# MichaelWoodhams/IQ-TREE

Hardware: AMD Instinct MI355X
Metric: million pattern-node partial-likelihood updates/sec (higher is better)
Workload: dtype f64; 1 GPU; DNA 50 taxa x 100000 patterns/GPU, GTR+G4, fixed tree: clearAllPartialLH + full traversal + root-branch lnL; ntaxa=50, patterns_per_gpu=100000, patterns_total=100000, nstates=4, ncat=4, parallelism=patterns sharded over 1 GPU(s), 1 RCCL all-reduce/step

## Files before the change

### include/iqhip.h

```cpp
#ifndef IQHIP_H_
#define IQHIP_H_

#include <stddef.h>
#include <stdint.h>

#ifdef __cplusplus
extern "C" {
#endif

#define IQHIP_ABI_VERSION 2

enum {
    IQHIP_OK = 0,
    IQHIP_ERR_NO_DEVICE = 1,
    IQHIP_ERR_INVALID = 2,
    IQHIP_ERR_UNSUPPORTED = 3,
    IQHIP_ERR_HIP = 4,
    IQHIP_ERR_NOMEM = 5
};

typedef struct iqhip_engine iqhip_engine;

typedef struct iqhip_node_op {
    uint64_t dst_key;
// ... 185 lines not shown
int iqhip_debug_ufboot_timing(iqhip_engine *e, double *ms , int64_t *launches);

int iqhip_pair_counts(iqhip_engine *e, const int32_t *pairs , int npairs, double *counts);
int iqhip_pair_distances(iqhip_engine *e, const double *init, double x1, double x2, double xacc, int max_steps,
                         double *dist, double *d2l, int32_t *nsteps);
int iqhip_debug_pair_timing(iqhip_engine *e, double *counts_ms, double *solve_ms);

typedef struct iqhip_quartet_result {
    double  logl[3];
    double  len[3][5];
    int32_t nsweeps[3], neval[3], status[3], _pad;
} iqhip_quartet_result;
int iqhip_quartet_cells(iqhip_engine *e, const int32_t *quartets , int nq,
                        double *cells , int32_t *nother );
int iqhip_quartet_likelihoods(iqhip_engine *e, const int32_t *quartets, int nq,
                              const double *const_invar ,
                              double x1, double x2, double xacc, int max_steps, double diverge_frac,
                              int iterations, double tolerance, iqhip_quartet_result *results);
int iqhip_debug_quartet_timing(iqhip_engine *e, double *cells_ms, double *solve_ms);

typedef struct iqhip_bionj_step { int32_t a, b; double la, lb, lambda; } iqhip_bionj_step;
int iqhip_bionj(iqhip_engine *e, int n, const double *dist , const double *var ,
                iqhip_bionj_step *steps , int32_t *last , double *last_len );
int iqhip_debug_bionj_timing(iqhip_engine *e, double *ms, int64_t *launches);

typedef struct iqhip_pars_op { int32_t dst, left, right, _pad; } iqhip_pars_op;
int iqhip_pars_init(iqhip_engine *e, const uint8_t *informative , int nvectors, int64_t *nsites);
int iqhip_pars_update(iqhip_engine *e, const iqhip_pars_op *ops, int nops);
int iqhip_pars_branch_scores(iqhip_engine *e, const int32_t *ends , int nbranch, int32_t *score,
                             int32_t *subst );
int iqhip_pars_insert_scores(iqhip_engine *e, const int32_t *ends, int nbranch, int32_t taxon,
                             int32_t *score , int32_t *best, int32_t *best_score);
int iqhip_pars_shape(iqhip_engine *e, int64_t *nsites, int64_t *nwords, int *nvectors);
int iqhip_pars_fetch(iqhip_engine *e, int32_t slot, uint32_t *out );
int iqhip_debug_pars_levels(int ntaxa, int nvectors, const uint8_t *valid , const iqhip_pars_op *ops,
                            int nops, int32_t *level);
int iqhip_debug_pars_timing(iqhip_engine *e, double *ms , int64_t *counts , int reset);
int iqhip_pars_insert_scores_batch(iqhip_engine *e, const int32_t *ends ,
                                   const int32_t *seg_start , int nseg,
                                   const int32_t *taxon , int32_t *score ,
                                   int32_t *best , int32_t *best_score );
int iqhip_debug_pars_batch_timing(iqhip_engine *e, double *ms , int64_t *counts ,
                                  int reset);

enum { IQHIP_PARS_SPR_NO_SCORE = 1 };
#define IQHIP_PARS_SPR_MAX_RADIUS 10
typedef struct iqhip_pars_spr_step { int32_t parent, side, target, flags; } iqhip_pars_spr_step;
typedef struct iqhip_pars_spr_job { int32_t subtree, first_step, nsteps, _pad; } iqhip_pars_spr_job;
int iqhip_pars_spr_scan(iqhip_engine *e, const iqhip_pars_spr_job *jobs, int njobs, const iqhip_pars_spr_step *steps,
                        int nsteps, int32_t *score , int32_t *best_step ,
                        int32_t *best_score , int32_t *best_job);
int iqhip_debug_pars_spr_check(int ntaxa, int nvectors, const uint8_t *valid ,
                               const iqhip_pars_spr_job *jobs, int njobs, const iqhip_pars_spr_step *steps, int nsteps,
                               int32_t *depth );
int iqhip_debug_pars_spr_timing(iqhip_engine *e, double *ms , int64_t *counts , int reset);

int iqhip_upload_partial(iqhip_engine *e, uint64_t key, const double *partial_lh,
                         const int16_t *scale_num);

int iqhip_timing_enable(iqhip_engine *e, int on);
int iqhip_timing_read(iqhip_engine *e, double *avg_ms, int64_t *launches, int reset);
int iqhip_timing_plan_bytes(iqhip_engine *e, double *stored, double *loaded);
int iqhip_timing_collective_read(iqhip_engine *e, double *avg_us, int64_t *count, int reset);

int iqhip_debug_cherry_tables(iqhip_engine *e, int64_t *tables_built, int64_t *ops_from_tables);

#define IQHIP_PATH_NEWTON_ONE_LAUNCH 0
#define IQHIP_PATH_NEWTON_CHAIN 1
#define IQHIP_PATH_SWEEP_PERSISTENT 2
#define IQHIP_PATH_SWEEP_PER_STEP 3
#define IQHIP_PATH_SWEEP_SEQUENTIAL 4
#define IQHIP_PATH_NEWTON_FALLBACK 5
#define IQHIP_PATH_NSLOTS 6
int iqhip_debug_path_counts(iqhip_engine *e, int64_t *out, int n);

int iqhip_debug_create_planner(iqhip_engine **out, int nstates , int ncat, int64_t nptn, int ntaxa,
                               int num_cus, int state_unknown, int nclass);
int iqhip_debug_plan(iqhip_engine *e, const iqhip_node_op *ops, int nops);
#define IQHIP_PLAN_SHAPE_NSLOTS 28
int iqhip_debug_plan_shape(iqhip_engine *e, int64_t *out, int n);
#define IQHIP_PLAN_LAYOUT_NSLOTS 8
int iqhip_debug_plan_layout(iqhip_engine *e, int32_t *out, int nops);

void iqhip_debug_memory(int64_t *device_bytes, int64_t *host_bytes);
void iqhip_debug_fail_alloc(int nth);

typedef struct iqhip_partition iqhip_partition;
int iqhip_partition_create(iqhip_partition **out, iqhip_engine *const *members, int nparts);
void iqhip_partition_destroy(iqhip_partition *g);
int iqhip_partition_set_rates(iqhip_partition *g, const double *rate );
int iqhip_partition_newton_branch(iqhip_partition *g, double xguess, double x1, double x2, double xacc, int max_steps,
                                  double *optx, double *d2l, int *nsteps, double *part_lnl );
int iqhip_partition_lnl_from_theta(iqhip_partition *g, double x, double *part_lnl );
int iqhip_partition_traverse_lnl(iqhip_partition *g, const iqhip_node_op *ops, int nops, iqhip_branch_end a,
                                 iqhip_branch_end b, double len, const double *scale ,
                                 double *part_lnl );
int iqhip_partition_optimize_branch_batch(iqhip_partition *g, const iqhip_branch_task *tasks, int ntasks,
                                          iqhip_branch_result *results,
                                          double *part_lnl );
int iqhip_debug_partition_timing(iqhip_partition *g, double *ms ,
                                 int64_t *launches);

int iqhip_partition_ptnlh_reserve(iqhip_partition *g, int nrows);
int iqhip_partition_optimize_branch_batch_rows(iqhip_partition *g, const iqhip_branch_task *tasks, int ntasks,
                                               iqhip_branch_result *results,
                                               double *part_lnl ,
                                               const int32_t *rows );
int iqhip_partition_ptnlh_rell(iqhip_partition *g, const int32_t *rows, int nrows, int nsamples,
                               double *out );
int iqhip_partition_ufboot_init(iqhip_partition *g, int nsamples);
int iqhip_partition_ufboot_update(iqhip_partition *g, const iqhip_ufboot_tree *trees, int ntrees, double epsilon,
                                  double logl_cutoff, int64_t *counts , double *min_orig_logl );
int iqhip_partition_ufboot_fetch(iqhip_partition *g, double *boot_logl, double *boot_orig_logl, int32_t *boot_counts,
                                 int64_t *boot_tree);
int iqhip_debug_partition_ufboot_timing(iqhip_partition *g, double *ms , int64_t *launches);

int iqhip_partition_pair_distances(iqhip_partition *g, const double *init, double x1, double x2, double xacc, int max_steps,
                                   double *dist, double *d2l, int32_t *nsteps);
int iqhip_debug_partition_pair_timing(iqhip_partition *g, double *counts_ms, double *solve_ms);

#ifdef __cplusplus
}
#endif
#endif
```

### iq-tree_amd/__init__.py

```python
import ctypes as C
import os

import numpy as np

_HERE = os.path.dirname(os.path.abspath(__file__))
LIB_DIR = os.environ.get("IQHIP_LIB_DIR") or os.path.join(_HERE, "lib")
REPO_ROOT = os.path.dirname(_HERE)

IQHIP_SYMBOLS = [
    "iqhip_last_error", "iqhip_abi_version", "iqhip_device_count", "iqhip_create", "iqhip_destroy",
    "iqhip_set_stream", "iqhip_reserve", "iqhip_release", "iqhip_rekey", "iqhip_set_alignment",
    "iqhip_set_ptn_freq", "iqhip_set_ptn_invar", "iqhip_set_ascertainment", "iqhip_set_model", "iqhip_update_partials",
    "iqhip_branch_lnl", "iqhip_traverse_lnl", "iqhip_compute_theta", "iqhip_derv",
    "iqhip_lnl_from_theta", "iqhip_newton_branch", "iqhip_optimize_branch", "iqhip_bind_result_buffer", "iqhip_result_device_ptr",
    "iqhip_result_capacity", "iqhip_traverse_lnl_async", "iqhip_derv_async", "iqhip_result_read",
    "iqhip_synchronize", "iqhip_fetch_scale_num", "iqhip_fetch_pattern_lh", "iqhip_fetch_partial",
    "iqhip_fetch_theta", "iqhip_upload_partial", "iqhip_timing_enable", "iqhip_timing_read",
    "iqhip_fetch_pattern_lh_scaled", "iqhip_set_boot_samples", "iqhip_rell", "iqhip_rell_async",
    "iqhip_set_mixture_model", "iqhip_pattern_lh_cat", "iqhip_optimize_branch_batch",
    "iqhip_em_posteriors", "iqhip_em_fetch_posteriors", "iqhip_em_site_rates", "iqhip_em_objective", "iqhip_debug_em_timing",
    "iqhip_mix_class_lh", "iqhip_mix_weights_em", "iqhip_mix_posteriors", "iqhip_debug_mix_timing",
    "iqhip_class_lnl", "iqhip_debug_class_lnl_timing",
    "iqhip_create_sharded", "iqhip_num_shards", "iqhip_shard_range", "iqhip_comm_unique_id", "iqhip_comm_init_rank",
    "iqhip_comm_size", "iqhip_update_partials_async", "iqhip_lnl_from_theta_async",
    "iqhip_newton_host_init", "iqhip_newton_host_update", "iqhip_newton_host_result",
    "iqhip_debug_create_planner", "iqhip_debug_plan", "iqhip_timing_plan_bytes", "iqhip_timing_collective_read", "iqhip_optimize_sweep", "iqhip_debug_cherry_tables",
    "iqhip_debug_path_counts", "iqhip_debug_plan_shape", "iqhip_debug_plan_layout", "iqhip_debug_memory", "iqhip_debug_fail_alloc",
    "iqhip_ptnlh_reserve", "iqhip_ptnlh_put_current", "iqhip_ptnlh_fetch", "iqhip_optimize_branch_batch_rows",
    "iqhip_branch_tests", "iqhip_ptnlh_rell",
    "iqhip_ptnlh_upload", "iqhip_gen_boot_samples", "iqhip_ptnlh_diff_variance", "iqhip_tree_tests", "iqhip_multiscale_bp",
    "iqhip_pair_counts", "iqhip_pair_distances", "iqhip_debug_pair_timing",
    "iqhip_quartet_cells", "iqhip_quartet_likelihoods", "iqhip_debug_quartet_timing",
    "iqhip_pars_init", "iqhip_pars_update", "iqhip_pars_branch_scores", "iqhip_pars_insert_scores", "iqhip_pars_fetch", "iqhip_pars_shape",
    "iqhip_debug_pars_levels", "iqhip_debug_pars_timing",
    "iqhip_pars_insert_scores_batch", "iqhip_debug_pars_batch_timing",
    "iqhip_pars_spr_scan", "iqhip_debug_pars_spr_check", "iqhip_debug_pars_spr_timing",
    "iqhip_bionj", "iqhip_debug_bionj_timing",
    "iqhip_ufboot_init", "iqhip_ufboot_update", "iqhip_ufboot_fetch", "iqhip_debug_ufboot_timing",
    "iqhip_partition_create", "iqhip_partition_destroy", "iqhip_partition_set_rates", "iqhip_partition_newton_branch",
    "iqhip_partition_lnl_from_theta", "iqhip_partition_traverse_lnl", "iqhip_debug_partition_timing",
    "iqhip_partition_optimize_branch_batch",
    "iqhip_partition_ptnlh_reserve", "iqhip_partition_optimize_branch_batch_rows", "iqhip_partition_ptnlh_rell",
    "iqhip_partition_ufboot_init", "iqhip_partition_ufboot_update", "iqhip_partition_ufboot_fetch",
    "iqhip_partition_pair_distances", "iqhip_debug_partition_pair_timing",
    "iqhip_debug_partition_ufboot_timing",
]

_LAUNCH_SLOTS = ("variant", "tab", "nfull", "ngroups", "grid", "lds_bytes", "hold_off")
PLAN_SHAPE_SLOTS = (("lds_budget", "lds_doubles", "state_slots", "nhold", "chunks", "stages") +
                    tuple("stage_units_%d" % s for s in range(8)) +
                    tuple("top_" + f for f in _LAUNCH_SLOTS) + tuple("unit_" + f for f in _LAUNCH_SLOTS))
PATH_SLOTS = ("newton_one_launch", "newton_chain", "sweep_persistent", "sweep_per_step", "sweep_sequential",
              "newton_fallback")


class NodeOp(C.Structure):
    _fields_ = [("dst_key", C.c_uint64), ("left_key", C.c_uint64), ("right_key", C.c_uint64),
                ("left_leaf", C.c_int32), ("right_leaf", C.c_int32),
                ("left_len", C.c_double), ("right_len", C.c_double), ("flags", C.c_uint32), ("_pad", C.c_uint32)]


class BranchEnd(C.Structure):
    _fields_ = [("key", C.c_uint64), ("leaf", C.c_int32), ("_pad", C.c_int32)]


class ParsOp(C.Structure):
    _fields_ = [("dst", C.c_int32), ("left", C.c_int32), ("right", C.c_int32), ("_pad", C.c_int32)]


class BranchSupport(C.Structure):
    _fields_ = [("sh_alrt", C.c_double), ("lbp", C.c_double), ("abayes", C.c_double), ("alrt_stat", C.c_double)]


class TreeTest(C.Structure):
    _fields_ = [("rell_bp", C.c_double), ("kh_pvalue", C.c_double), ("sh_pvalue", C.c_double), ("wkh_pvalue", C.c_double),
                ("wsh_pvalue", C.c_double), ("elw_value", C.c_double), ("rell_confident", C.c_int32),
                ("elw_confident", C.c_int32)]


class UFBootTree(C.Structure):
    _fields_ = [("row", C.c_int32), ("_pad", C.c_int32), ("tree_id", C.c_int64), ("logl", C.c_double), ("rand", C.c_double)]


class BranchTask(C.Structure):
    _fields_ = [("ops", C.c_void_p), ("nops", C.c_int32), ("max_steps", C.c_int32), ("a", BranchEnd), ("b", BranchEnd),
                ("xguess", C.c_double), ("x1", C.c_double), ("x2", C.c_double), ("xacc", C.c_double)]


class BranchResult(C.Structure):
    _fields_ = [("optx", C.c_double), ("d2l", C.c_double), ("lnl", C.c_double), ("nsteps", C.c_int32), ("status", C.c_int32)]


TREE_TEST_DTYPE = np.dtype([("logl", np.float64), ("rell_bp", np.float64), ("kh_pvalue", np.float64),
                            ("sh_pvalue", np.float64), ("wkh_pvalue", np.float64), ("wsh_pvalue", np.float64),
                            ("elw_value", np.float64), ("rell_confident", np.bool_), ("elw_confident", np.bool_)])
AU_SCALES = (0.5, 0.6, 0.7, 0.8, 0.9, 1.0, 1.1, 1.2, 1.3, 1.4)
BIONJ_STEP_DTYPE = np.dtype([("a", np.int32), ("b", np.int32), ("la", np.float64), ("lb", np.float64), ("lambda", np.float64)])
SUPPORT_DTYPE = np.dtype([("node1", np.int32), ("node2", np.int32), ("lh", np.float64, (3,)), ("sh_alrt", np.float64),
                          ("lbp", np.float64), ("abayes", np.float64), ("alrt_stat", np.float64)])


def leaf_end(leaf):
    return BranchEnd(0, int(leaf), 0)


def key_end(key):
    return BranchEnd(int(key), -1, 0)


ALLREDUCE_HOOK = C.CFUNCTYPE(None, C.c_void_p, C.c_int, C.c_void_p)
# ... 2713 lines not shown
```

### iq-tree_amd/csrc/engine.hip

```cpp
#include <math.h>
#include <stdio.h>
#include <stdlib.h>
#include <string.h>

#include <algorithm>
#include <cmath>
#include <atomic>

#include "iqhip_internal.h"

using namespace iqhip;

static thread_local std::string g_err;
namespace iqhip {
int set_error(int code, const std::string &msg) {
    g_err = msg;
    return code;
}
double debug_build_us = 0.0;
}

extern "C" void iqhip_debug_memory(int64_t *device_bytes, int64_t *host_bytes) {
    if (device_bytes) *device_bytes = g_mem_bytes[0].load();
    if (host_bytes) *host_bytes = g_mem_bytes[1].load();
// ... 138 lines not shown
                    hipHostGetDevicePointer((void **)&e->d_done, (void *)e->h_done.p, 0) == hipSuccess &&
                    hipEventCreateWithFlags(&e->staging_free, hipEventDisableTiming) == hipSuccess &&
                    e->dummy.plh.ensure(e, P * e->block) == hipSuccess && e->dummy.sc.ensure(e, P) == hipSuccess &&
                    e->d_newton_partials.ensure(e, (size_t)4 * e->num_cus) == hipSuccess &&
                    e->d_newton_barrier.ensure(e, 2) == hipSuccess && e->d_fold_ticket.ensure(e, 4) == hipSuccess &&
                    e->d_newton_posts.ensure(e, nposts) == hipSuccess &&
                    e->d_fold_flags.ensure(e, (size_t)e->result_cap) == hipSuccess;
    if (!ok) {
        iqhip_destroy(e);
        return fail(IQHIP_ERR_NOMEM, "iqhip_create: device allocation failed");
    }
    hipMemsetAsync(e->dummy.plh.p, 0, P * e->block * sizeof(double), e->stream);
    hipMemsetAsync(e->dummy.sc.p, 0, P * sizeof(int16_t), e->stream);
    hipMemsetAsync(e->d_newton_barrier.p, 0, 2 * sizeof(unsigned int), e->stream);
    hipMemsetAsync(e->d_newton_posts.p, 0xFF, nposts * sizeof(double), e->stream);
    hipMemsetAsync(e->d_fold_ticket.p, 0, 4 * sizeof(unsigned int), e->stream);
    hipMemsetAsync(e->d_fold_flags.p, 0, (size_t)e->result_cap * sizeof(int), e->stream);
    e->d_result = e->d_result_own;
    hipMemsetAsync(e->d_theta.p, 0, P * e->block * sizeof(double), e->stream);
    hipMemsetAsync(e->d_pattern_lh.p, 0, P * sizeof(double), e->stream);
    memset(e->h_result.p, 0, e->result_cap * sizeof(double));
    *e->h_done.p = 0;
    hipStreamSynchronize(e->stream);
    *out = e;
    return IQHIP_OK;
}

extern "C" void iqhip_destroy(iqhip_engine *e) {
    if (!e) return;
    if (!e->shards.empty()) sharded::destroy(e);
    use_device(e);
    if (e->stream) hipStreamSynchronize(e->stream);
    if (e->pair) iqhip_destroy(e->pair);
    e->pair = nullptr;
    comm_destroy(e);
    if (e->stream) hipStreamSynchronize(e->stream);
    if (e->staging_free) hipEventDestroy(e->staging_free);
    for (auto &p : e->tev) {
        hipEventDestroy(p.first);
        hipEventDestroy(p.second);
    }
    for (auto &p : e->cev) {
        hipEventDestroy(p.first);
        hipEventDestroy(p.second);
    }
    if (e->own_stream && e->stream) hipStreamDestroy(e->stream);
    delete e;
}

extern "C" int iqhip_set_stream(iqhip_engine *e, void *hip_stream) {
    if (!e) return fail(IQHIP_ERR_INVALID, "null engine");
    if (!e->shards.empty()) return fail(IQHIP_ERR_UNSUPPORTED, "a sharded engine runs on its shards' own streams");
    HIPCHK(use_device(e));
    HIPCHK(hipStreamSynchronize(e->stream));
    if (e->own_stream) hipStreamDestroy(e->stream);
    e->stream = (hipStream_t)hip_stream;
    e->own_stream = false;
    if (e->pair) return iqhip_set_stream(e->pair, hip_stream);
    return IQHIP_OK;
}

static int new_slab(iqhip_engine *e, int *idx) {
    if (!e->free_slabs.empty()) {
        *idx = e->free_slabs.back();
        e->free_slabs.pop_back();
        return IQHIP_OK;
    }
    Slab s;
    const size_t P = (size_t)e->nptn_pad;
    if (s.plh.ensure(e, P * e->block) != hipSuccess || s.sc.ensure(e, P) != hipSuccess) return fail(IQHIP_ERR_NOMEM, "slab alloc");
    if (!e->planner) {
        hipMemsetAsync(s.plh.p, 0, P * e->block * sizeof(double), e->stream);
        hipMemsetAsync(s.sc.p, 0, P * sizeof(int16_t), e->stream);
    }
    e->slabs.push_back(std::move(s));
    *idx = (int)e->slabs.size() - 1;
    return IQHIP_OK;
}

int iqhip::slab_for_key(iqhip_engine *e, uint64_t key, bool create, int *idx) {
    auto it = e->key2slab.find(key);
    if (it != e->key2slab.end()) {
        *idx = it->second;
        return IQHIP_OK;
    }
    if (!create) return fail(IQHIP_ERR_INVALID, "unknown partial_lh key (vector never computed)");
    int rc = new_slab(e, idx);
    if (rc) return rc;
    e->key2slab[key] = *idx;
    e->keymap_version++;
    return IQHIP_OK;
}

extern "C" int iqhip_reserve(iqhip_engine *e, int nvectors) {
    if (!e) return fail(IQHIP_ERR_INVALID, "null engine");
    if (!e->shards.empty()) return sharded::reserve(e, nvectors);
    HIPCHK(use_device(e));
    int have = (int)e->slabs.size();
    for (int i = have; i < nvectors; i++) {
        int idx;
        std::vector<int> keep;
        keep.swap(e->free_slabs);
        int rc = new_slab(e, &idx);
        keep.swap(e->free_slabs);
        if (rc) return rc;
        e->free_slabs.push_back(idx);
    }
    return IQHIP_OK;
}

extern "C" int iqhip_release(iqhip_engine *e, uint64_t key) {
    if (!e) return fail(IQHIP_ERR_INVALID, "null engine");
    if (!e->shards.empty()) return sharded::release(e, key);
    auto it = e->key2slab.find(key);
    if (it == e->key2slab.end()) return IQHIP_OK;
    e->free_slabs.push_back(it->second);
    e->key2slab.erase(it);
    e->keymap_version++;
    return IQHIP_OK;
}

extern "C" int iqhip_rekey(iqhip_engine *e, uint64_t old_key, uint64_t new_key) {
    if (!e) return fail(IQHIP_ERR_INVALID, "null engine");
    if (!e->shards.empty()) return sharded::rekey(e, old_key, new_key);
    auto it = e->key2slab.find(old_key);
    if (it == e->key2slab.end()) return fail(IQHIP_ERR_INVALID, "iqhip_rekey: unknown key");
    if (old_key == new_key) return IQHIP_OK;
    if (e->key2slab.count(new_key)) iqhip_release(e, new_key);
    int idx = it->second;
    e->key2slab.erase(it);
    e->key2slab[new_key] = idx;
    e->keymap_version++;
    return IQHIP_OK;
}

extern "C" int iqhip_set_ptn_freq(iqhip_engine *e, const double *ptn_freq) {
    if (!e || !ptn_freq) return fail(IQHIP_ERR_INVALID, "null argument");
    if (!e->shards.empty()) return sharded::set_ptn_array(e, ptn_freq, false);
    HIPCHK(use_device(e));
    std::vector<double> tmp((size_t)e->nptn_pad, 0.0);
    memcpy(tmp.data(), ptn_freq, sizeof(double) * (size_t)e->nptn);
    HIPCHK(hipMemcpyAsync(e->d_freq.p, tmp.data(), tmp.size() * sizeof(double), hipMemcpyHostToDevice,
                          e->stream));
    HIPCHK(hipStreamSynchronize(e->stream));
    e->freq_prefix_valid = false;
    e->h_freq.assign(ptn_freq, ptn_freq + e->nptn);
    e->pars_ready = false;
    return IQHIP_OK;
}

extern "C" int iqhip_set_ptn_invar(iqhip_engine *e, const double *ptn_invar) {
    if (!e || !ptn_invar) return fail(IQHIP_ERR_INVALID, "null argument");
    if (!e->shards.empty()) return sharded::set_ptn_array(e, ptn_invar, true);
    HIPCHK(use_device(e));
    std::vector<double> tmp((size_t)e->nptn_pad, 0.0);
    memcpy(tmp.data(), ptn_invar, sizeof(double) * (size_t)e->nptn);
    HIPCHK(hipMemcpyAsync(e->d_invar.p, tmp.data(), tmp.size() * sizeof(double),
                          hipMemcpyHostToDevice, e->stream));
    HIPCHK(hipStreamSynchronize(e->stream));
    return IQHIP_OK;
}

extern "C" int iqhip_set_alignment(iqhip_engine *e, const uint8_t *states, const double *ptn_freq,
                                   const double *ptn_invar) {
    if (!e || !states || !ptn_freq || !ptn_invar) return fail(IQHIP_ERR_INVALID, "null argument");
    if (!e->shards.empty()) return sharded::set_alignment(e, states, ptn_freq, ptn_invar);
    if (!e->model_set)
        return fail(IQHIP_ERR_INVALID,
                    "iqhip_set_alignment: call iqhip_set_model first (needs state_unknown)");
    HIPCHK(use_device(e));
    const size_t P = (size_t)e->nptn_pad, N = (size_t)e->nptn;
    std::vector<uint8_t> tmp((size_t)e->ntaxa * P, (uint8_t)(e->embed2 ? e->n : e->state_unknown));
    for (int t = 0; t < e->ntaxa; t++) {
        const uint8_t *src = states + (size_t)t * N;
        if (e->embed2) {
            uint8_t *dst = tmp.data() + (size_t)t * P;
            for (size_t p = 0; p < N; p++) {
                if (src[p] > e->n_user) return fail(IQHIP_ERR_INVALID, "iqhip_set_alignment: state > STATE_UNKNOWN");
                dst[p] = src[p] == e->n_user ? (uint8_t)e->n : src[p];
            }
            continue;
        }
        for (size_t p = 0; p < N; p++)
            if (src[p] > e->state_unknown)
                return fail(IQHIP_ERR_INVALID, "iqhip_set_alignment: state > STATE_UNKNOWN");
        memcpy(tmp.data() + (size_t)t * P, src, N);
    }
    HIPCHK(hipMemcpyAsync(e->d_states.p, tmp.data(), tmp.size(), hipMemcpyHostToDevice, e->stream));
    HIPCHK(hipStreamSynchronize(e->stream));
    e->pars_ready = false;
    int rc = iqhip_set_ptn_freq(e, ptn_freq);
    if (rc) return rc;
    rc = iqhip_set_ptn_invar(e, ptn_invar);
    if (rc) return rc;
    e->aln_set = true;
    return IQHIP_OK;
}

extern "C" int iqhip_set_ascertainment(iqhip_engine *e, int64_t n_unobserved, double nsites) {
    if (!e) return fail(IQHIP_ERR_INVALID, "null engine");
    if (n_unobserved < 0 || n_unobserved >= e->nptn || (n_unobserved > 0 && !(nsites > 0.0)))
        return fail(IQHIP_ERR_INVALID, "iqhip_set_ascertainment: bad pattern count / site count");
    if (!e->shards.empty()) return sharded::set_ascertainment(e, n_unobserved, nsites);
    e->n_unobs = n_unobserved;
    e->asc_nsites = nsites;
    e->asc_active = n_unobserved > 0 || (e->comm && nsites > 0.0);
    e->pattern_lh_shift = 0.0;
    return IQHIP_OK;
}

static int set_model_common(iqhip_engine *e, int nclass, const int32_t *cat_class, const double *eval,
                            const double *evec, const double *inv_evec, const double *rates, const double *props,
                            int state_unknown, const double *tip ) {
    if (!e || !eval || !evec || !inv_evec || !rates || !props || !tip)
        return fail(IQHIP_ERR_INVALID, "null argument");
    if (!e->shards.empty())
        return sharded::set_model(e, nclass, cat_class, eval, evec, inv_evec, rates, props, state_unknown, tip);
    if (state_unknown < e->n || state_unknown > (e->mfma ? 255 : 31))
        return fail(IQHIP_ERR_INVALID, "iqhip_set_model: state_unknown out of range");
    if (e->aln_set && state_unknown != e->state_unknown)
        return fail(IQHIP_ERR_INVALID, "iqhip_set_model: state_unknown changed after set_alignment");
    if (nclass < 1 || nclass > e->ncat) return fail(IQHIP_ERR_INVALID, "bad number of mixture classes");
    if (e->n == 4 && !e->wide4) {
        const bool want_mfma = nclass > 1;
        if (want_mfma != e->mfma) {
            HIPCHK(use_device(e));
            HIPCHK(hipStreamSynchronize(e->stream));
            e->mfma = want_mfma;
            if (want_mfma) { e->lane_split_valu = e->lane_split; e->lane_split = 1; }
            else e->lane_split = e->lane_split_valu;
            e->tile = want_mfma ? 16 : 64;
            e->ntiles = e->nptn_pad / e->tile;
            e->plan_cache.invalidate();
            e->theta_valid = false;
            HIPCHK(hipMemsetAsync(e->d_newton_posts.p, 0xFF, (size_t)2 * kNewtonPostEpochs * (2 * e->num_cus) * 2 * sizeof(double), e->stream));
            e->newton_post_launches = 0;
        }
    }
    std::vector<int> cls(e->ncat, 0);
    if (nclass > 1) {
        if (!cat_class) return fail(IQHIP_ERR_INVALID, "null argument");
        for (int c = 0; c < e->ncat; c++) {
            if (cat_class[c] < 0 || cat_class[c] >= nclass) return fail(IQHIP_ERR_INVALID, "category class out of range");
            cls[c] = cat_class[c];
        }
    }
    HIPCHK(use_device(e));
    const int n = e->n, C = e->ncat;
    HIPCHK(hipStreamSynchronize(e->stream));
    const size_t nst = (size_t)state_unknown + 1;
    const size_t o_eval = 0, o_evec = o_eval + n, o_ievec = o_evec + (size_t)n * n, o_rates = o_ievec + (size_t)n * n,
                 o_props = o_rates + C, o_tip = o_props + C, o_evalc = o_tip + nst * n, o_tipc = o_evalc + (size_t)C * n,
                 o_cls = o_tipc + nst * C * n;
    const int a_mt = n / 16, a_ks = n / 4;
    const bool a_tail = (n % 16) == 4;
    const size_t aimg_doubles = (n == 20 || n == 64) ? (size_t)2 * a_mt * a_ks * 64 + (a_tail ? (size_t)2 * a_ks * 64 : 0) : 0;
    const size_t o_aimg = (o_cls + ((size_t)C + 1) / 2 + 1) / 2 * 2;
    const size_t total = o_aimg + aimg_doubles;
    std::vector<double> blk(total, 0.0);
    memcpy(&blk[o_eval], eval, sizeof(double) * n);
    memcpy(&blk[o_evec], evec, sizeof(double) * n * n);
    memcpy(&blk[o_ievec], inv_evec, sizeof(double) * n * n);
    memcpy(&blk[o_rates], rates, sizeof(double) * C);
    memcpy(&blk[o_props], props, sizeof(double) * C);
    for (size_t s = 0; s < nst; s++) memcpy(&blk[o_tip + s * n], &tip[(s * nclass) * n], sizeof(double) * n);
    for (int c = 0; c < C; c++) memcpy(&blk[o_evalc + (size_t)c * n], &eval[(size_t)cls[c] * n], sizeof(double) * n);
    for (size_t s = 0; s < nst; s++)
        for (int c = 0; c < C; c++)
            memcpy(&blk[o_tipc + (s * C + c) * n], &tip[(s * nclass + cls[c]) * n], sizeof(double) * n);
    memcpy(&blk[o_cls], cls.data(), sizeof(int) * C);
    e->h_evec0.assign(evec, evec + (size_t)n * n);
    e->h_tip0.assign(&blk[o_tip], &blk[o_tip] + nst * n);
    if (aimg_doubles) {
        double *U = &blk[o_aimg], *Ui = U + (size_t)a_mt * a_ks * 64, *U4 = Ui + (size_t)a_mt * a_ks * 64, *Ui4 = U4 + (size_t)a_ks * 64;
        for (int m = 0; m < a_mt; m++)
            for (int ks = 0; ks < a_ks; ks++)
                for (int l = 0; l < 64; l++) {
                    const int row = 16 * m + (l & 15), k = 4 * ks + (l >> 4);
                    U[((size_t)m * a_ks + ks) * 64 + l] = evec[(size_t)row * n + k];
                    Ui[((size_t)m * a_ks + ks) * 64 + l] = inv_evec[(size_t)row * n + k];
                }
        if (a_tail)
            for (int ks = 0; ks < a_ks; ks++)
                for (int l = 0; l < 64; l++) {
                    const int row = 16 * a_mt + (l & 3), k = 4 * ks + (l >> 4);
                    U4[(size_t)ks * 64 + l] = evec[(size_t)row * n + k];
                    Ui4[(size_t)ks * 64 + l] = inv_evec[(size_t)row * n + k];
                }
    }
    HIPCHK(e->d_model.ensure(e, total));
    double *const d_model = e->d_model.p;
    HIPCHK(hipMemcpy(d_model, blk.data(), sizeof(double) * total, hipMemcpyHostToDevice));
    e->d_eval = d_model + o_eval;
    e->d_evec = d_model + o_evec;
    e->d_inv_evec = d_model + o_ievec;
    e->d_rates = d_model + o_rates;
    e->d_props = d_model + o_props;
    e->d_tip = d_model + o_tip;
    e->d_evalc = d_model + o_evalc;
    e->d_tipc = d_model + o_tipc;
    e->d_cls = reinterpret_cast<int *>(d_model + o_cls);
    e->d_aimg = aimg_doubles ? d_model + o_aimg : nullptr;
    e->aimg_doubles = (int)aimg_doubles;
    if (nclass > 1 || (e->n == 20 && !e->mfma_pipelined_ok) || e->wide4) {
        const int MT = (n + 15) / 16, KS = n / 4;
// ... 151 lines not shown

int iqhip::require(iqhip_engine *e, const char *what, unsigned needs) {
    const auto no = [what](int code, const char *why) { return fail(code, std::string(what) + ": " + why); };
    if (!e) return no(IQHIP_ERR_INVALID, "null engine");
    if (e->planner) return no(IQHIP_ERR_INVALID, "not available on a planning-only engine");
    if ((needs & REQ_SINGLE_DEVICE) && (!e->shards.empty() || e->comm))
        return no(IQHIP_ERR_UNSUPPORTED, "not available on pattern-sharded engines");
    if ((needs & REQ_NO_ASC) && (e->asc_active || e->n_unobs > 0))
        return no(IQHIP_ERR_UNSUPPORTED, "not available with ascertainment bias correction (+ASC)");
    const bool only4 = needs & REQ_STATES_4;
    if ((needs & REQ_PLAIN_STATES) && (e->embed2 || e->n_user != e->n))
        return no(IQHIP_ERR_UNSUPPORTED, only4 ? "not available for embedded state counts (4 states only)"
                                               : "not available for embedded state counts (4, 20 or 64 states only)");
    if ((needs & REQ_STATES_4_20_64) && e->n != 4 && e->n != 20 && e->n != 64) return no(IQHIP_ERR_UNSUPPORTED, "4, 20 or 64 states only");
    if (only4 && e->n != 4) return no(IQHIP_ERR_UNSUPPORTED, "4 states only");
    if ((needs & REQ_NO_MIXTURE) && e->nclass > 1) return no(IQHIP_ERR_UNSUPPORTED, "not available for mixture models");
    if ((needs & REQ_MIXTURE) && e->nclass < 2) return no(IQHIP_ERR_UNSUPPORTED, "the model is no mixture (one class)");
    if ((needs & REQ_MODEL_ALN) && (!e->model_set || !e->aln_set))
        return no(IQHIP_ERR_INVALID, "needs iqhip_set_model and iqhip_set_alignment first");
    if ((needs & REQ_THETA) && !e->theta_valid) return no(IQHIP_ERR_INVALID, "needs iqhip_compute_theta first");
    return IQHIP_OK;
}

static void timing_begin(iqhip_engine *e) {
    if (!e->timing) return;
    if (e->tev_used == e->tev.size()) {
        hipEvent_t a, b;
        hipEventCreate(&a);
        hipEventCreate(&b);
        e->tev.emplace_back(a, b);
    }
    hipEventRecord(e->tev[e->tev_used].first, e->stream);
}
static void timing_end(iqhip_engine *e) {
    if (!e->timing) return;
    hipEventRecord(e->tev[e->tev_used].second, e->stream);
    e->tev_used++;
}

static int build_cherry_tables(iqhip_engine *e) {
    iqhip_engine *p = e->pair;
    const int n = (int)e->plan.cherry_jobs.size();
    std::vector<iqhip_node_op> ops((size_t)n);
    const std::vector<int> segs((size_t)n, 1);
    for (int i = 0; i < n; i++) {
        const iqhip_engine::CherrySlot &cs = e->cherry_slots[e->plan.cherry_jobs[i]];
        iqhip_node_op &o = ops[i];
        memset(&o, 0, sizeof o);
        o.dst_key = (uint64_t)e->plan.cherry_jobs[i] + 1;
        o.left_leaf = 0;
        o.right_leaf = 1;
        o.left_len = cs.len_l;
        o.right_len = cs.len_r;
    }
    iqhip_branch_end none = {0, -1, 0};
    int rc = submit_traverse(p, ops.data(), n, false, none, none, 0.0, true, &segs, nullptr);
    if (rc) return rc;
    std::vector<const double *> src((size_t)n);
    std::vector<double *> dst((size_t)n);
    const size_t per = (size_t)e->cherry_npairs * e->block;
    for (int i = 0; i < n; i++) {
        int idx;
        rc = slab_for_key(p, ops[i].dst_key, false, &idx);
        if (rc) return rc;
        src[i] = p->slabs[idx].plh.p;
        dst[i] = e->d_cherry_tab.p + (size_t)e->plan.cherry_jobs[i] * per;
    }
    HIPCHK(launch_cherry_transpose(e, src.data(), dst.data(), n, e->cherry_npairs));
    for (int i = 0; i < n; i++) e->cherry_slots[e->plan.cherry_jobs[i]].model_version = e->model_version;
    e->cherry_built_total += n;
    e->plan.cherry_jobs.clear();
    return IQHIP_OK;
}

int iqhip::submit_traverse(iqhip_engine *e, const iqhip_node_op *ops, int nops, bool has_root,
                           iqhip_branch_end a, iqhip_branch_end b, double len, bool skip_reduce,
                           const std::vector<int> *explicit_segs, const double *const *len_ptrs) {
    int rc = check_ready(e);
    if (rc) return rc;
    if (nops < 0 || (nops > 0 && !ops)) return fail(IQHIP_ERR_INVALID, "bad ops array");
    int last_dst = -1;
    Stopwatch watch;
    if (e->debug_sweep) watch.start();
    rc = build_plan(e, ops, nops, &last_dst, explicit_segs, len_ptrs);
    if (rc) return rc;
    if (e->debug_sweep) debug_build_us += watch.us();
    DevBranch br;
    if (has_root) {
        rc = build_branch(e, a, b, len, last_dst, &br);
        if (rc) return rc;
    }
    rc = ensure_slab_rows(e, 2 + nops);
    if (rc) return rc;
    const int nwaves = (int)e->ntiles * e->lane_split;
    if (e->plan.nleaf_tabs > 0) {
        const int njobs = leaf_tables_follow_model(e) ? e->plan.nleaf_tabs : e->plan.tab_dirty;
        if (njobs > 0)
            HIPCHK(launch_leaf_tables(e, reinterpret_cast<const TabJob *>(e->d_ops.p + e->plan.jobs_off), njobs));
        e->plan.tab_dirty = 0;
    }
    if (!e->plan.cherry_jobs.empty()) {
        rc = build_cherry_tables(e);
        if (rc) return rc;
    }
    if (e->plan.uses_cherry)
        for (int k = 0; k < nops; k++) e->cherry_ops_total += e->h_ops.p[k].cherry != nullptr;
    timing_begin(e);
    const int *table = reinterpret_cast<const int *>(e->d_ops.p + e->plan.table_off);
    {
        int off = 2;
        for (int n : e->plan.stage_units) {
            if (e->mfma) HIPCHK(launch_traverse_mfma(e, table + off, n, nwaves));
            else HIPCHK(launch_traverse4(e, table + off, n, e->plan.units_have_load, nullptr, nwaves));
            off += 2 * n;
        }
    }
    const bool empty_top = e->plan.nunits > 0 && !has_root && e->plan.top_nops == 0;
    const bool fold4 = e->fold_reduce && !e->mfma && !empty_top && !skip_reduce;
    const bool foldm = e->fold_reduce && e->mfma && has_root && e->n_unobs == 0;
    if (empty_top) {
    } else if (e->mfma) HIPCHK(launch_traverse_mfma(e, table, nops > 0 ? 1 : 0, nwaves, true));
    else HIPCHK(launch_traverse4(e, table, 1, e->plan.has_load, has_root ? &br : nullptr, nwaves, fold4 ? nops : -1));
    timing_end(e);
    if (e->timing) e->tev_launches += (int)e->plan.stage_units.size() + (empty_top ? 0 : 1);
    if (e->mfma && has_root) HIPCHK(launch_stream_mfma(e, 0, &br, br.len, nwaves, nullptr, foldm ? nops : -1));
    if (fold4 || foldm) {
    } else if (has_root) HIPCHK(launch_reduce(e, 0, 2 + nops, nwaves));
    else if (!skip_reduce) HIPCHK(launch_reduce(e, 2, nops, nwaves));
    e->last_nops = nops;
    e->last_has_root = has_root;
    e->last_root_loads_b = has_root && br.b_kind != CHILD_PREV;
    return IQHIP_OK;
}

int iqhip::read_result(iqhip_engine *e, int ndoubles) {
    if (e->d_result != e->d_result_own)
        HIPCHK(hipMemcpyAsync(e->h_result.p, e->d_result, sizeof(double) * ndoubles, hipMemcpyDeviceToHost,
                              e->stream));
    else if (e->poll_pending) {
        e->poll_pending = false;
        const unsigned long long want = e->result_seq;
        for (int spin = 0; spin < 200000; spin++) {
            if (*e->h_done.p == want) {
                std::atomic_thread_fence(std::memory_order_acquire);
                e->staging_busy = false;
                if (e->folded_rows >= 0) {
                    if (e->h_result.p[2 + e->folded_rows] == 0.0)
                        for (int k = 0; k < e->folded_rows; k++) e->h_result.p[2 + k] = 0.0;
                    e->folded_rows = -1;
                }
                return IQHIP_OK;
            }
            __builtin_ia32_pause();
        }
    }
    e->poll_pending = false;
    HIPCHK(hipStreamSynchronize(e->stream));
    e->staging_busy = false;
    if (e->folded_rows >= 0) {
        if (e->h_result.p[2 + e->folded_rows] == 0.0)
            for (int k = 0; k < e->folded_rows; k++) e->h_result.p[2 + k] = 0.0;
        e->folded_rows = -1;
    }
    return IQHIP_OK;
}

void iqhip::result_arrived(iqhip_engine *e) {
// ... 95 lines not shown
    return iqhip_traverse_lnl(e, nullptr, 0, a, b, len, nullptr, lnl);
}

extern "C" int iqhip_traverse_lnl_async(iqhip_engine *e, const iqhip_node_op *ops, int nops,
                                        iqhip_branch_end a, iqhip_branch_end b, double len) {
    if (e && !e->shards.empty())
        return fail(IQHIP_ERR_UNSUPPORTED, "a sharded engine reduces its results itself: use the synchronous calls");
    return submit_traverse(e, ops, nops, true, a, b, len);
}

extern "C" int iqhip_update_partials_async(iqhip_engine *e, const iqhip_node_op *ops, int nops) {
    if (e && !e->shards.empty())
        return fail(IQHIP_ERR_UNSUPPORTED, "a sharded engine reduces its results itself: use the synchronous calls");
    iqhip_branch_end none = {0, -1, 0};
    return submit_traverse(e, ops, nops, false, none, none, 0.0);
}

void iqhip::set_theta_branch(iqhip_engine *e, const DevBranch &br, iqhip_branch_end a, iqhip_branch_end b) {
    e->theta_valid = true;
    e->theta_a_sc = br.a_sc;
    e->theta_b_sc = br.b_sc;
    if (b.leaf >= 0) std::swap(a, b);
    e->theta_end[0] = a;
    e->theta_end[1] = b;
}

extern "C" int iqhip_compute_theta(iqhip_engine *e, iqhip_branch_end a, iqhip_branch_end b) {
    if (e && !e->shards.empty()) return sharded::compute_theta(e, a, b);
    int rc = check_ready(e);
    if (rc) return rc;
    DevBranch br;
    rc = build_branch(e, a, b, 0.0, -1, &br);
    if (rc) return rc;
    if (e->mfma) HIPCHK(launch_stream_mfma(e, 1, &br, 0.0, (int)e->ntiles));
    else HIPCHK(launch_theta4(e, br));
    set_theta_branch(e, br, a, b);
    return IQHIP_OK;
}

extern "C" int iqhip_derv_async(iqhip_engine *e, double len) {
    if (e && !e->shards.empty())
        return fail(IQHIP_ERR_UNSUPPORTED, "a sharded engine reduces its results itself: use the synchronous calls");
    int rc = check_ready(e);
    if (rc) return rc;
    if (!e->theta_valid) return fail(IQHIP_ERR_INVALID, "iqhip_derv: theta not computed");
    if (!(len >= 0.0)) return fail(IQHIP_ERR_INVALID, "negative or NaN branch length");
    const int nrows = e->n_unobs > 0 ? 5 : 2;
    if (e->asc_active && e->n_unobs == 0) {
        if (e->d_result == e->d_result_own) e->h_result.p[2] = e->h_result.p[3] = e->h_result.p[4] = 0.0;
        else HIPCHK(hipMemsetAsync(e->d_result + 2, 0, 3 * sizeof(double), e->stream));
    }
    rc = ensure_slab_rows(e, nrows);
    if (rc) return rc;
    const int nwaves = (int)e->ntiles;
    if (e->mfma) HIPCHK(launch_stream_mfma(e, 2, nullptr, len, nwaves));
    else HIPCHK(launch_derv4(e, len, nwaves));
    HIPCHK(launch_reduce(e, 0, nrows, nwaves));
    return IQHIP_OK;
}

extern "C" int iqhip_derv(iqhip_engine *e, double len, double *df, double *ddf) {
    if (e && !e->shards.empty()) return sharded::derv(e, len, df, ddf);
    int rc = iqhip_derv_async(e, len);
    if (rc) return rc;
    rc = comm_allreduce(e, e->asc_active ? 5 : 2);
    if (rc) return rc;
    rc = read_result(e, e->asc_active ? 5 : 2);
    if (rc) return rc;
    double a = e->h_result.p[0], b = e->h_result.p[1];
    newton_repair(a, b);
    if (e->asc_active) asc_derv_correct(e->h_result.p + 2, e->asc_nsites, a, b);
    if (df) *df = a;
    if (ddf) *ddf = b;
    return IQHIP_OK;
}

extern "C" int iqhip_debug_cherry_tables(iqhip_engine *e, int64_t *tables_built, int64_t *ops_from_tables) {
    if (!e) return fail(IQHIP_ERR_INVALID, "null engine");
    if (tables_built) *tables_built = e->cherry_built_total;
    if (ops_from_tables) *ops_from_tables = e->cherry_ops_total;
    return IQHIP_OK;
}

extern "C" int iqhip_debug_path_counts(iqhip_engine *e, int64_t *out, int n) {
    if (!e) return fail(IQHIP_ERR_INVALID, "null engine");
    if (!out && n > 0) return fail(IQHIP_ERR_INVALID, "null argument");
    for (int k = 0; k < n && k < IQHIP_PATH_NSLOTS; k++) out[k] = e->path_counts[k];
    return IQHIP_OK;
}

extern "C" int iqhip_lnl_from_theta_async(iqhip_engine *e, double len) {
    if (e && !e->shards.empty())
        return fail(IQHIP_ERR_UNSUPPORTED, "a sharded engine reduces its results itself: use the synchronous calls");
    int rc = check_ready(e);
    if (rc) return rc;
    if (!e->theta_valid) return fail(IQHIP_ERR_INVALID, "iqhip_lnl_from_theta: theta not computed");
    if (!(len >= 0.0)) return fail(IQHIP_ERR_INVALID, "negative or NaN branch length");
    rc = ensure_slab_rows(e, 2);
    if (rc) return rc;
    const int nwaves = (int)e->ntiles;
    if (e->mfma) HIPCHK(launch_stream_mfma(e, 3, nullptr, len, nwaves));
    else HIPCHK(launch_lnl_theta4(e, len, nwaves));
    HIPCHK(launch_reduce(e, 0, 2, nwaves));
    return IQHIP_OK;
}

extern "C" int iqhip_lnl_from_theta(iqhip_engine *e, double len, double *lnl) {
    if (e && !e->shards.empty()) return sharded::lnl_from_theta(e, len, lnl);
    int rc = iqhip_lnl_from_theta_async(e, len);
    if (rc) return rc;
    rc = comm_allreduce(e, e->asc_active ? 2 : 1);
    if (rc) return rc;
    rc = read_result(e, 2);
    if (rc) return rc;
    double v = e->h_result.p[0];
    if (isnan(v) || isinf(v)) {
        rc = repair_lnl_comm(e, &v);
        if (rc) return rc;
    }
    rc = asc_finish_lnl(e, &v);
    if (rc) return rc;
    if (lnl) *lnl = v;
    return IQHIP_OK;
}

extern "C" int iqhip_bind_result_buffer(iqhip_engine *e, void *device_ptr, int capacity_doubles) {
    if (!e) return fail(IQHIP_ERR_INVALID, "null engine");
    if (!e->shards.empty() || e->comm)
        return fail(IQHIP_ERR_UNSUPPORTED, "an engine with a communicator reduces in its own device result vector");
    HIPCHK(use_device(e));
    HIPCHK(hipStreamSynchronize(e->stream));
    if (!device_ptr) {
        e->d_result = e->d_result_own;
        e->result_cap = 8 + 16384;
        return IQHIP_OK;
    }
    if (capacity_doubles < 2) return fail(IQHIP_ERR_INVALID, "result buffer too small");
    e->d_result = (double *)device_ptr;
    e->result_cap = std::min(capacity_doubles, 8 + 16384);
    return IQHIP_OK;
}
extern "C" void *iqhip_result_device_ptr(iqhip_engine *e) { return (e && e->shards.empty()) ? (void *)e->d_result : nullptr; }
extern "C" int iqhip_result_capacity(iqhip_engine *e) { return e ? e->result_cap : 0; }

extern "C" int iqhip_result_read(iqhip_engine *e, double *out, int ndoubles) {
    if (e && !e->shards.empty())
        return fail(IQHIP_ERR_UNSUPPORTED, "a sharded engine reduces its results itself: use the synchronous calls");
    if (!e || !out || ndoubles < 0 || ndoubles > e->result_cap)
        return fail(IQHIP_ERR_INVALID, "iqhip_result_read: bad arguments");
    HIPCHK(use_device(e));
    int rc = read_result(e, ndoubles);
    if (rc) return rc;
    memcpy(out, e->h_result.p, sizeof(double) * ndoubles);
    return IQHIP_OK;
}

extern "C" int iqhip_synchronize(iqhip_engine *e) {
    if (!e) return fail(IQHIP_ERR_INVALID, "null engine");
    if (!e->shards.empty()) return sharded::synchronize(e);
    HIPCHK(use_device(e));
    HIPCHK(hipStreamSynchronize(e->stream));
    e->staging_busy = false;
    return IQHIP_OK;
}

static inline size_t dev_index(const iqhip_engine *e, int64_t p, int k) {
// ... 54 lines not shown
    HIPCHK(hipMemcpy(e->slabs[idx].sc.p, sc.data(), sc.size() * sizeof(int16_t), hipMemcpyHostToDevice));
    return IQHIP_OK;
}

extern "C" int iqhip_fetch_theta(iqhip_engine *e, double *out) {
    if (!e || !out) return fail(IQHIP_ERR_INVALID, "null argument");
    if (!e->shards.empty()) return sharded::fetch_vec(e, 0, true, out);
    HIPCHK(use_device(e));
    return fetch_vec(e, e->d_theta.p, out);
}

extern "C" int iqhip_fetch_scale_num(iqhip_engine *e, uint64_t key, int16_t *out) {
    if (!e || !out) return fail(IQHIP_ERR_INVALID, "null argument");
    if (!e->shards.empty()) return sharded::fetch_scale_num(e, key, out);
    HIPCHK(use_device(e));
    int idx;
    int rc = slab_for_key(e, key, false, &idx);
    if (rc) return rc;
    HIPCHK(hipStreamSynchronize(e->stream));
    HIPCHK(hipMemcpy(out, e->slabs[idx].sc.p, sizeof(int16_t) * (size_t)e->nptn, hipMemcpyDeviceToHost));
    return IQHIP_OK;
}

extern "C" int iqhip_fetch_pattern_lh(iqhip_engine *e, double *out) {
    if (!e || !out) return fail(IQHIP_ERR_INVALID, "null argument");
    if (!e->shards.empty()) return sharded::fetch_pattern_lh(e, out, 0, iqhip_branch_end{0, -1, 0}, iqhip_branch_end{0, -1, 0});
    HIPCHK(use_device(e));
    HIPCHK(hipStreamSynchronize(e->stream));
    HIPCHK(hipMemcpy(out, e->d_pattern_lh.p, sizeof(double) * (size_t)e->nptn, hipMemcpyDeviceToHost));
    if (e->asc_active) {
        const int64_t nobs = e->nptn - e->n_unobs;
        for (int64_t p = 0; p < nobs; p++) out[p] -= e->pattern_lh_shift;
        for (int64_t p = nobs; p < e->nptn; p++) out[p] = 0.0;
    }
    return IQHIP_OK;
}

extern "C" int iqhip_timing_enable(iqhip_engine *e, int on) {
    if (!e) return fail(IQHIP_ERR_INVALID, "null engine");
    if (!e->shards.empty()) {
        for (iqhip_engine *c : e->shards) c->timing = on != 0;
        return IQHIP_OK;
    }
    e->timing = on != 0;
    return IQHIP_OK;
}

extern "C" int iqhip_timing_collective_read(iqhip_engine *e, double *avg_us, int64_t *count, int reset) {
    if (!e) return fail(IQHIP_ERR_INVALID, "null engine");
    if (!e->shards.empty()) e = e->shards[0];
    HIPCHK(use_device(e));
    HIPCHK(hipStreamSynchronize(e->stream));
    double total = 0.0;
    for (size_t i = 0; i < e->cev_used; i++) {
        float ms = 0.f;
        HIPCHK(hipEventElapsedTime(&ms, e->cev[i].first, e->cev[i].second));
        total += ms;
    }
    if (avg_us) *avg_us = e->cev_used ? total * 1e3 / (double)e->cev_used : 0.0;
    if (count) *count = (int64_t)e->cev_used;
    if (reset) e->cev_used = 0;
    return IQHIP_OK;
}

extern "C" int iqhip_timing_plan_bytes(iqhip_engine *e, double *stored, double *loaded) {
    if (!e) return fail(IQHIP_ERR_INVALID, "null engine");
    double st = 0.0, ld = 0.0;
    if (!e->shards.empty()) {
        for (iqhip_engine *c : e->shards) {
            double a = 0.0, b = 0.0;
            int rc = iqhip_timing_plan_bytes(c, &a, &b);
            if (rc) return rc;
            st += a; ld += b;
        }
    } else {
        const double P = (double)e->nptn_pad, V = (double)e->block * 8.0;
        const bool hands_over = e->wide4 && !e->wide4_generic && e->h_ops.p && e->last_nops > 0;
        std::vector<char> seg_first(hands_over ? (size_t)e->last_nops : 0, 0);
        if (hands_over) {
            const int *tab = reinterpret_cast<const int *>(e->h_ops.p + e->plan.table_off);
            for (int u = 0; u <= e->plan.nunits; u++)
                if (tab[2 * u + 1] > 0 && tab[2 * u] >= 0 && tab[2 * u] < e->last_nops) seg_first[tab[2 * u]] = 1;
        }
        for (int k = 0; k < e->last_nops && e->h_ops.p; k++) {
            const DevOp &d = e->h_ops.p[k];
            st += P * (V + 2.0);
            const double *held = (hands_over && k > 0 && !seg_first[k]) ? e->h_ops.p[k - 1].dst : nullptr;
            if (d.left_kind == CHILD_LEAF) ld += P;
            else if ((d.left_kind == CHILD_PF || d.left_kind == CHILD_LOAD) && d.pf != held) ld += P * (V + 2.0);
            if (d.right_kind == CHILD_LEAF) ld += P; else if (d.right_kind == CHILD_LOAD && d.ld != held) ld += P * (V + 2.0);
        }
        if (e->last_has_root) {
            st += P * 8.0;
            ld += P * 16.0 + (e->last_root_loads_b ? P * V : 0.0) + P;
        }
    }
    if (stored) *stored = st;
    if (loaded) *loaded = ld;
    return IQHIP_OK;
}

extern "C" int iqhip_timing_read(iqhip_engine *e, double *avg_ms, int64_t *launches, int reset) {
    if (!e) return fail(IQHIP_ERR_INVALID, "null engine");
    if (!e->shards.empty()) {
        double worst = 0.0;
        int64_t n0 = 0;
        for (size_t g = 0; g < e->shards.size(); g++) {
            double a = 0.0;
            int64_t n = 0;
            int rc = iqhip_timing_read(e->shards[g], &a, &n, reset);
            if (rc) return rc;
            if (a > worst) worst = a;
            if (g == 0) n0 = n;
        }
        if (avg_ms) *avg_ms = worst;
        if (launches) *launches = n0;
        return IQHIP_OK;
    }
    HIPCHK(use_device(e));
    HIPCHK(hipStreamSynchronize(e->stream));
    double total = 0.0;
    for (size_t i = 0; i < e->tev_used; i++) {
        float ms = 0.f;
        HIPCHK(hipEventElapsedTime(&ms, e->tev[i].first, e->tev[i].second));
        total += ms;
    }
    if (avg_ms) *avg_ms = e->tev_launches ? total / (double)e->tev_launches : 0.0;
    if (launches) *launches = e->tev_launches;
    if (reset) { e->tev_used = 0; e->tev_launches = 0; }
    return IQHIP_OK;
}

extern "C" int iqhip_debug_create_planner(iqhip_engine **out, int nstates, int ncat, int64_t nptn, int ntaxa, int num_cus,
                                          int state_unknown, int nclass) {
    if (!out) return fail(IQHIP_ERR_INVALID, "iqhip_debug_create_planner: out == NULL");
    *out = nullptr;
    if (nptn <= 0 || ntaxa < 2 || ncat < 1 || num_cus < 1 || nclass < 1 || nclass > ncat)
        return fail(IQHIP_ERR_INVALID, "iqhip_debug_create_planner: bad shape");
    if (nstates != 4 && nstates != 20 && nstates != 64)
        return fail(IQHIP_ERR_UNSUPPORTED, "iqhip_debug_create_planner: nstates must be 4, 20 or 64");
    if (state_unknown < nstates || state_unknown > 255) return fail(IQHIP_ERR_INVALID, "state_unknown out of range");
    {
        const int rc = check_shape4("iqhip_debug_create_planner", nstates, nstates, ncat);
        if (rc) return rc;
    }
    iqhip_engine *e = new iqhip_engine();
    e->planner = true;
    e->check_plans = true;
    e->num_cus = num_cus;
    configure_engine(e, -1, nstates, nstates, ncat, nptn, ntaxa);
    const size_t P = (size_t)e->nptn_pad;
    e->d_states.ensure(e, (size_t)ntaxa * P);
    e->dummy.plh.ensure(e, P * e->block);
    e->dummy.sc.ensure(e, P);
    e->result_cap = 8 + 16384;
    e->state_unknown = state_unknown;
    e->nclass = nclass;
    if (nclass > 1 && nstates == 4 && !e->wide4) {
        e->mfma = true;
        e->lane_split = 1;
        e->tile = 16;
        e->ntiles = e->nptn_pad / 16;
    }
    e->mfma_pipelined = e->mfma_pipelined_ok && nclass == 1;
    e->model_set = e->aln_set = true;
    {
        const int s2 = state_unknown + 1;
        if (cherry_candidate(e) && nclass == 1 && s2 * s2 <= 4356 && (int64_t)4 * s2 * s2 <= e->nptn_pad) {
            e->cherry_s2 = s2;
// ... 61 lines not shown
```

### iq-tree_amd/csrc/iqhip_internal.h

```cpp
#pragma once
#include <hip/hip_runtime.h>
#include <stdint.h>
#include <stdlib.h>
#include <time.h>
#include <algorithm>
#include <atomic>
#include <string>
#include <type_traits>
#include <unordered_map>
#include <vector>
#include "../../include/iqhip.h"
#include "trav_lds.h"

namespace iqhip {

constexpr int kSmallPlanOps = 4;
constexpr int kNewtonPostEpochs = 128;
constexpr int kMixEmTile = 256;
constexpr int kMixEmRegClasses = 8;
constexpr int kMixEmBatch = 16;
constexpr int kMixEmUpdateThreads = 1024;
constexpr double kScalingThreshold = 0x1p-256;
constexpr double kScalingThresholdInv = 0x1p256;
constexpr double kLogScalingThreshold = -177.44567822334599;

enum ChildKind : int32_t { CHILD_LEAF = 0, CHILD_LOAD = 1, CHILD_PREV = 2, CHILD_PF = 3, CHILD_HOLD = 4 };

struct __attribute__((aligned(16))) DevOp {
    double *dst;
    int16_t *dst_sc;
    const double *pf;
    const int16_t *pf_sc;
    const uint8_t *sl;
    const uint8_t *sr;
    const double *ld;
    const int16_t *ld_sc;
    int32_t left_kind;
    int32_t right_kind;
    double left_len;
    double right_len;
    int32_t lds_left;
    int32_t lds_right;
    int32_t chunk_nops;
    int32_t real_mask;
    int32_t sl_slot;
    int32_t sr_slot;
    int32_t push_hold;
    int32_t out_row;
    int32_t no_scale;
    const double *tabL;
    const double *tabR;
    const double *left_len_p;
    const double *right_len_p;
    const double *cherry;
    int32_t chunk_slots;
    int32_t _pad_slots;
};

#if defined(__HIPCC__)
__device__ __forceinline__ double wave_sum64(double v) {
    unsigned lo = __double2loint(v), hi = __double2hiint(v);
    auto a = __builtin_amdgcn_permlane32_swap(lo, lo, false, false);
    auto b = __builtin_amdgcn_permlane32_swap(hi, hi, false, false);
    v = __hiloint2double(b[0], a[0]) + __hiloint2double(b[1], a[1]);
    lo = __double2loint(v);
    hi = __double2hiint(v);
    auto c = __builtin_amdgcn_permlane16_swap(lo, lo, false, false);
    auto d = __builtin_amdgcn_permlane16_swap(hi, hi, false, false);
    v = __hiloint2double(d[0], c[0]) + __hiloint2double(d[1], c[1]);
#define IQHIP_DPP_STEP(ctrl)                                                                                  \
    v += __hiloint2double(__builtin_amdgcn_mov_dpp(__double2hiint(v), ctrl, 0xF, 0xF, true),                  \
                          __builtin_amdgcn_mov_dpp(__double2loint(v), ctrl, 0xF, 0xF, true));
    IQHIP_DPP_STEP(0x128)
    IQHIP_DPP_STEP(0x124)
    IQHIP_DPP_STEP(0x4E)
    IQHIP_DPP_STEP(0xB1)
#undef IQHIP_DPP_STEP
    return v;
}

__device__ __forceinline__ double group_sum(double v) {
    unsigned lo = __double2loint(v), hi = __double2hiint(v);
    auto a = __builtin_amdgcn_permlane16_swap(lo, lo, false, false);
    auto b = __builtin_amdgcn_permlane16_swap(hi, hi, false, false);
    v = __hiloint2double(b[0], a[0]) + __hiloint2double(b[1], a[1]);
    lo = __double2loint(v);
    hi = __double2hiint(v);
    auto c = __builtin_amdgcn_permlane32_swap(lo, lo, false, false);
    auto d = __builtin_amdgcn_permlane32_swap(hi, hi, false, false);
    return __hiloint2double(d[0], c[0]) + __hiloint2double(d[1], c[1]);
}

constexpr unsigned kScalingThresholdHi = 0x2FF00000u;
__device__ __forceinline__ unsigned amax_hi(unsigned m, double v) {
    const unsigned h = (unsigned)__double2hiint(v) & 0x7fffffffu;
    return m > h ? m : h;
}
__device__ __forceinline__ unsigned nonzero_bits(double v) {
    return ((unsigned)__double2hiint(v) & 0x7fffffffu) | (unsigned)__double2loint(v);
}
__device__ __forceinline__ unsigned group_max_u(unsigned v) {
    auto a = __builtin_amdgcn_permlane32_swap(v, v, false, false);
    v = a[0] > a[1] ? a[0] : a[1];
    auto b = __builtin_amdgcn_permlane16_swap(v, v, false, false);
    return b[0] > b[1] ? b[0] : b[1];
}

template <typename OpRef>
__device__ __forceinline__ double op_child_len(const OpRef &d, int child) {
    const double *p = child ? d.right_len_p : d.left_len_p;
    return p ? *p : (child ? d.right_len : d.left_len);
}
#endif

struct __attribute__((aligned(16))) DevBranch {
    const double *a;
    const uint8_t *a_states;
    const double *b;
    const int16_t *a_sc;
    const int16_t *b_sc;
    int32_t a_kind;
    int32_t b_kind;
    double len;
};

struct __attribute__((aligned(16))) SweepOp {
    double *dst;
    int16_t *dst_sc;
    const double *lv, *rv;
    const int16_t *lsc, *rsc;
    const uint8_t *ls, *rs;
    double llen, rlen;
    int32_t llen_step, rlen_step;
    int32_t no_scale;
    int32_t row;
};
struct __attribute__((aligned(16))) SweepStep {
    DevBranch br;
    double xguess;
    int32_t op_begin, nops;
};

struct __attribute__((aligned(16))) PairTile {
    int32_t ra[4], rb[4];
    int32_t out[16];
};

struct __attribute__((aligned(16))) TabJob {
    double len;
    double *tab;
    const double *len_p;
    double _pad;
};

struct Plan {
    int lds_doubles = 0;
    int state_slots = 1;
    bool has_load = false;
    bool units_have_load = false;
    bool small = false;
    int small_nops = 0;
    int nunits = 0, top_nops = 0;
    std::vector<int> stage_units;
    int table_off = 0, jobs_off = 0;
    int nhold = 0;
    int nleaf_tabs = 0;
    std::vector<TabJob> tab_jobs;
    int tab_dirty = 0;
    std::vector<int> cherry_jobs;
    bool uses_cherry = false;
    uint64_t cherry_model = 0;
};

struct PlanCache {
    std::vector<char> ops_in;
    std::vector<int> segs;
    uint64_t version = 0;
    int dst = -1;
    std::vector<char> uploaded;
    void invalidate() { version = 0; uploaded.clear(); }
};

struct __attribute__((aligned(16))) NewtonState {
    double x1, x2, xacc;
    double rts, rts_old, xl, xh, dx, f, df, d2l, result;
    int32_t max_steps, j, neval, status;
    int32_t done, _pad[3];
};

__host__ __device__ inline void newton_init(NewtonState &s, double xguess, double x1, double x2, double xacc,
                                            int max_steps) {
    s.x1 = x1; s.x2 = x2; s.xacc = xacc;
    s.rts = xguess;
    if (s.rts < x1) s.rts = x1;
    if (s.rts > x2) s.rts = x2;
    s.rts_old = s.rts; s.xl = x1; s.xh = x2; s.dx = 0.0; s.f = s.df = s.d2l = 0.0;
    s.result = s.rts;
    s.max_steps = max_steps; s.j = 0; s.neval = 0; s.status = 0; s.done = 0;
    s._pad[0] = s._pad[1] = s._pad[2] = 0;
}

__host__ __device__ inline bool newton_finite(double v) { return v == v && v - v == 0.0; }

__host__ __device__ inline void newton_repair(double &pdf, double &pddf) {
    if (!newton_finite(pdf)) { pdf = 0.0; pddf = 0.0; }
}

__host__ __device__ inline void asc_derv_correct(const double *c, double asc_nsites, double &df, double &ddf) {
    const double prob_const = 1.0 - c[0];
    const double df_frac = c[1] / prob_const, ddf_frac = c[2] / prob_const;
    df += asc_nsites * df_frac;
    ddf += asc_nsites * (ddf_frac + df_frac * df_frac);
}

__host__ __device__ inline void newton_advance(NewtonState &s, double f, double df) {
    if (s.done) return;
    s.f = f; s.df = df;
    s.neval++;
    if (s.neval == 1) {
        s.d2l = df;
        if (!newton_finite(f) || !newton_finite(df)) { s.status = 2; s.result = s.rts; s.done = 1; return; }
        if (df >= 0.0 && fabs(f) < s.xacc) { s.result = s.rts; s.done = 1; return; }
        if (f < 0.0) { s.xl = s.rts; s.xh = s.x2; } else { s.xh = s.rts; s.xl = s.x1; }
        s.dx = fabs(s.xh - s.xl);
        s.j = 1;
    } else {
        if (!newton_finite(f) || !newton_finite(df)) { s.status = 2; s.result = s.rts_old; s.done = 1; return; }
        if (df > 0.0 && fabs(f) < s.xacc) { s.d2l = df; s.result = s.rts; s.done = 1; return; }
        if (f < 0.0) s.xl = s.rts; else s.xh = s.rts;
        s.j++;
        if (s.j > s.max_steps) { s.status = 3; s.result = s.rts; s.done = 1; return; }
    }
    s.rts_old = s.rts;
    if ((df <= 0.0) || (((s.rts - s.xh) * df - f) * ((s.rts - s.xl) * df - f) >= 0.0)) {
        s.dx = 0.5 * (s.xh - s.xl);
        s.rts = s.xl + s.dx;
        s.d2l = df;
        if (s.xl == s.rts) { s.result = s.rts; s.done = 1; return; }
    } else {
        s.dx = f / df;
        const double temp = s.rts;
        s.rts -= s.dx;
        s.d2l = df;
        if (temp == s.rts) { s.result = s.rts; s.done = 1; return; }
    }
    if (fabs(s.dx) < s.xacc || s.j == s.max_steps) { s.result = s.rts_old; s.done = 1; return; }
}

__host__ __device__ inline void newton_update(NewtonState &s, double pdf, double pddf) {
    if (s.done) return;
    newton_repair(pdf, pddf);
    newton_advance(s, -pdf, -pddf);
}

enum MemKind : int { MEM_DEVICE = 0, MEM_PINNED, MEM_PINNED_MAPPED, MEM_HOST };
inline std::atomic<int64_t> g_mem_bytes[2];
inline std::atomic<int> g_fail_alloc_in{0};
inline hipError_t mem_alloc(void **p, size_t bytes, MemKind kind) {
    *p = nullptr;
    if (g_fail_alloc_in.load() > 0 && g_fail_alloc_in.fetch_sub(1) == 1) return hipErrorOutOfMemory;
    hipError_t s;
    if (kind == MEM_DEVICE) s = hipMalloc(p, bytes);
    else if (kind == MEM_HOST) s = (*p = calloc(1, bytes)) ? hipSuccess : hipErrorOutOfMemory;
    else s = hipHostMalloc(p, bytes, kind == MEM_PINNED_MAPPED ? hipHostMallocMapped : hipHostMallocDefault);
    if (s == hipSuccess) g_mem_bytes[kind != MEM_DEVICE] += (int64_t)bytes;
    return s;
}
inline void mem_free(void *p, size_t bytes, MemKind kind) {
    if (kind == MEM_DEVICE) hipFree(p);
    else if (kind == MEM_HOST) free(p);
    else hipHostFree(p);
    g_mem_bytes[kind != MEM_DEVICE] -= (int64_t)bytes;
}

template <typename T>
struct OwnedBuf {
    T *p = nullptr; size_t cap = 0;
    OwnedBuf() = default;
    OwnedBuf(OwnedBuf &&o) noexcept { swap(o); }
    OwnedBuf &operator=(OwnedBuf &&o) noexcept { swap(o); return *this; }
    ~OwnedBuf() { reset(); }
    void swap(OwnedBuf &o) { std::swap(p, o.p); std::swap(cap, o.cap); std::swap(bytes, o.bytes); std::swap(kind, o.kind); }
    void reset() {
        if (bytes) mem_free(const_cast<std::remove_cv_t<T> *>(p), bytes, kind);
        p = nullptr; cap = 0; bytes = 0;
    }
protected:
    hipError_t replace(hipStream_t s, size_t count, MemKind k) {
        if (k != MEM_HOST) {
            const hipError_t rc = hipStreamSynchronize(s);
            if (rc != hipSuccess) return rc;
        }
        reset();
        void *q = nullptr;
        const hipError_t rc = mem_alloc(&q, count * sizeof(T), k);
        if (rc != hipSuccess) return rc;
        p = static_cast<T *>(q); cap = count; bytes = count * sizeof(T); kind = k;
        return hipSuccess;
    }
    size_t bytes = 0;
    MemKind kind = MEM_DEVICE;
};

template <typename T>
struct DevBuf : OwnedBuf<T> {
    hipError_t ensure(hipStream_t s, size_t count) { return count <= this->cap ? hipSuccess : this->replace(s, count, MEM_DEVICE); }
    hipError_t ensure(iqhip_engine *e, size_t count);
};
template <typename T>
struct PinBuf : OwnedBuf<T> {
    hipError_t ensure(hipStream_t s, size_t count, bool mapped = false) {
        return count <= this->cap ? hipSuccess : this->replace(s, count, mapped ? MEM_PINNED_MAPPED : MEM_PINNED);
    }
    hipError_t ensure(iqhip_engine *e, size_t count, bool mapped = false);
};
template <typename T>
struct PairBuf {
    DevBuf<T> d; PinBuf<T> h;
    template <typename Where>
    hipError_t ensure(Where w, size_t count) {
        const hipError_t rc = d.ensure(w, count);
        return rc != hipSuccess ? rc : h.ensure(w, count);
    }
};

struct Slab {
    DevBuf<double> plh;
    DevBuf<int16_t> sc;
};

}

struct iqhip_engine {
    int device = 0;
    bool planner = false;
    uint64_t fake_next = 0x100000000000ull;
    bool check_plans = false;
    int n = 0, ncat = 0, ntaxa = 0;
    bool embed2 = false;
    bool scalar_rule_all = false;
    int n_user = 0;
    int64_t nptn = 0;
    int64_t nptn_pad = 0;
    int64_t ntiles = 0;
    int tile = 64;
    bool mfma = false;
    bool mfma_pipelined = false;
    bool row_split = false;
    bool cat_split = false;
    bool top_cs2 = false;
    int lane_split = 1;
    bool wide4 = false, wide4_generic = false;
    int lane_split_valu = 1;
    bool mix_split = false;
    bool mixed_top = true;
    bool hold_lds = true;
    int lds_budget_bytes = 64 * 1024;
    bool small_plans = true;
    int split_target = -1;
    int max_levels = 3;
    int mfma_lds_kb = -1;
    bool debug_plan = false;
    bool debug_sweep = false;
    std::string debug_break_plan;
    iqhip::Plan plan;
    iqhip::Slab dummy;
    int block = 0;
    int state_unknown = -1;
    bool model_set = false, aln_set = false, theta_valid = false;
    int64_t n_unobs = 0;
    bool asc_active = false;
    double asc_nsites = 0.0;
    double pattern_lh_shift = 0.0;
    const int16_t *theta_a_sc = nullptr;
    const int16_t *theta_b_sc = nullptr;
    iqhip_branch_end theta_end[2] = {{0, -1, 0}, {0, -1, 0}};

    hipStream_t stream = nullptr;
    bool own_stream = false;

    iqhip::DevBuf<uint8_t> d_states;
    iqhip::DevBuf<double> d_freq, d_invar;
    double *d_eval = nullptr, *d_evec = nullptr, *d_inv_evec = nullptr;
    double *d_rates = nullptr, *d_props = nullptr, *d_tip = nullptr;
    std::vector<double> h_eval, h_rates, h_props;
    std::vector<int> h_cls;
    iqhip::DevBuf<iqhip::DevOp> d_ops;
    iqhip::DevBuf<double> d_slab;
    iqhip::DevBuf<unsigned int> d_fold_ticket;
    iqhip::DevBuf<int> d_fold_flags;
    bool fold_reduce = false;
    bool poll_result = true, poll_pending = false;
    unsigned long long result_seq = 0;
    iqhip::PinBuf<volatile unsigned long long> h_done;
    unsigned long long *d_done = nullptr;
    iqhip::DevBuf<double> d_theta, d_pattern_lh;
    iqhip::DevBuf<double> d_leaf_tab;
    std::vector<double> tab_len;
    uint64_t model_version = 1, tab_model_version = 0;
    struct CherrySlot {
        double len_l = -1.0, len_r = -1.0;
        uint64_t model_version = 0;
        uint64_t stamp = 0;
    };
    bool cherry_on = true;
    iqhip_engine *pair = nullptr;
    int cherry_s2 = 0, cherry_npairs = 0;
    iqhip::DevBuf<double> d_cherry_tab;
    std::unordered_map<uint64_t, int> cherry_slot_of;
    std::vector<CherrySlot> cherry_slots;
    uint64_t cherry_stamp = 0;
// ... 58 lines not shown
    } mix;
    struct {
        iqhip::DevBuf<double> cw, inv, part, out;
        iqhip::DevBuf<int32_t> list;
        double ms = 0.0;
    } cl;
    bool mixture_api = false;
    struct {
        iqhip::DevBuf<iqhip::PairTile> tiles;
        iqhip::DevBuf<double> counts, coef, init, out;
        double ms[2] = {0.0, 0.0};
    } pd;
    struct {
        iqhip::DevBuf<int32_t> quartets, nother, other;
        iqhip::DevBuf<double> cells;
        iqhip::DevBuf<iqhip_quartet_result> out;
        double ms[2] = {0.0, 0.0};
    } qt;
    struct {
        double ms = 0.0;
        int64_t launches = 0;
    } bj;
    std::vector<double> h_freq, h_evec0, h_tip0;
    bool pars_ready = false;
    int pars_nvec = 0;
    int64_t pars_nsites = 0, pars_nwords = 0;
    std::vector<uint8_t> pars_valid;
    struct {
        iqhip::DevBuf<uint32_t> vec, score;
        iqhip::DevBuf<int32_t> ints;
        iqhip::DevBuf<int32_t> out;
        iqhip::DevBuf<uint64_t> masks;
    } pars;
    iqhip::PinBuf<int32_t> h_pars_ops, h_pars_ends, h_pars_out;
    double pars_ms[2] = {0.0, 0.0};
    int64_t pars_counts[4] = {0, 0, 0, 0};
    double pars_spr_ms = 0.0;
    int64_t pars_spr_counts[2] = {0, 0};
    double pars_batch_ms = 0.0;
    int64_t pars_batch_counts[3] = {0, 0, 0};
    iqhip::DevBuf<int32_t> d_batch_rows;
    double *d_result_own = nullptr, *d_result = nullptr;
    iqhip::DevBuf<double> d_newton_partials;
    iqhip::DevBuf<unsigned int> d_newton_barrier;
    unsigned int newton_launches = 0;
    iqhip::DevBuf<double> d_newton_posts;
    unsigned int newton_post_launches = 0;
    bool newton_posts = true;
    iqhip::DevBuf<double> d_batch_posts;
    size_t batch_posts_used[2] = {0, 0};
    unsigned int batch_post_launches = 0;
    iqhip::DevBuf<double> d_theta_batch, d_batch_partials, d_batch_out;
    iqhip::DevBuf<unsigned int> d_batch_barriers;
    iqhip::DevBuf<char> d_batch_tasks;
    int batch_cap = 0;
    unsigned int batch_launches = 0;
    iqhip::DevBuf<double> d_sweep_len;
    iqhip::PinBuf<char> h_sweep_desc;
    iqhip::DevBuf<char> d_sweep_desc;
    iqhip::DevBuf<unsigned long long> d_sweep_prof;
    iqhip::DevBuf<double> d_sweep_posts;
    int num_cus = 256;
    int result_cap = 0;
    void *comm = nullptr;
    int comm_nranks = 1, comm_rank = 0;
    iqhip::DevBuf<double> d_result_dev;
    iqhip::DevBuf<iqhip::NewtonState> d_nstate;
    iqhip::PinBuf<iqhip::NewtonState> h_nstate;
    iqhip::DevBuf<iqhip::NewtonState> d_bstates;
    iqhip::DevBuf<const int16_t *> d_bsc;
    std::vector<iqhip_engine *> shards;
    std::vector<int64_t> shard_first;
    int reduce_mode = 0;
    iqhip::PinBuf<iqhip::DevOp> h_ops;
    iqhip::PinBuf<double> h_result;
    iqhip::PlanCache plan_cache;
    iqhip::PinBuf<char> h_plan_arena;
    size_t plan_arena_used = 0;
    bool plan_arena_on = false;
    uint64_t keymap_version = 1;
    hipEvent_t staging_free = nullptr;
    bool staging_busy = false;

    std::unordered_map<uint64_t, int> key2slab;
    std::vector<iqhip::Slab> slabs;
    std::vector<int> free_slabs;

    bool timing = false;
    std::vector<std::pair<hipEvent_t, hipEvent_t>> tev;
    size_t tev_used = 0;
    std::vector<std::pair<hipEvent_t, hipEvent_t>> cev;
    size_t cev_used = 0;
    int64_t tev_launches = 0;
    int last_nops = 0;
    bool last_has_root = false, last_root_loads_b = false;
    int folded_rows = -1;
};

namespace iqhip {

struct FoldArgs {
    double *slab;
    double *result;
    unsigned int *ticket;
    int *flags;
    int nwaves;
    int nrows_scale;
    int root_rows;
    int enabled;
    volatile unsigned long long *done;
    unsigned long long seq;
};

#if defined(__HIPCC__)
__device__ __forceinline__ void fold_store(double *p, double v) {
    __hip_atomic_store(p, v, __ATOMIC_RELAXED, __HIP_MEMORY_SCOPE_AGENT);
}
__device__ __forceinline__ void fold_flag(const FoldArgs &F, int row) {
    __hip_atomic_fetch_or(&F.flags[row], 1, __ATOMIC_RELAXED, __HIP_MEMORY_SCOPE_AGENT);
}

__device__ inline void fold_tail(const FoldArgs &F) {
    __shared__ double s_f[256];
    __shared__ int s_last;
    asm volatile("s_waitcnt vmcnt(0)" ::: "memory");
    __syncthreads();
    if (threadIdx.x == 0) {
        const unsigned int t = __hip_atomic_fetch_add(F.ticket, 1u, __ATOMIC_RELAXED, __HIP_MEMORY_SCOPE_AGENT);
        s_last = (t == gridDim.x - 1) ? 1 : 0;
    }
    __syncthreads();
    if (!s_last) return;
    __shared__ int s_rows[256];
    __shared__ int s_n;
    const int nrows = 2 + F.nrows_scale;
    auto sum_row = [&](int row) {
        const double *r = F.slab + (size_t)row * F.nwaves;
        if (threadIdx.x < 64) {
            double acc[4] = {0.0, 0.0, 0.0, 0.0};
            for (int base = 0; base < F.nwaves; base += 8 * 256) {
                double v[4][8];
#pragma unroll
                for (int j = 0; j < 4; j++)
#pragma unroll
                    for (int q = 0; q < 8; q++) {
                        const int i = base + q * 256 + (int)threadIdx.x + 64 * j;
                        v[j][q] = i < F.nwaves ? __hip_atomic_load(&r[i], __ATOMIC_RELAXED, __HIP_MEMORY_SCOPE_AGENT) : 0.0;
                    }
#pragma unroll
                for (int j = 0; j < 4; j++)
#pragma unroll
                    for (int q = 0; q < 8; q++) {
                        const int i = base + q * 256 + (int)threadIdx.x + 64 * j;
                        if (i < F.nwaves) acc[j] += v[j][q];
                    }
            }
#pragma unroll
            for (int j = 0; j < 4; j++) s_f[(int)threadIdx.x + 64 * j] = acc[j];
        }
        __syncthreads();
#pragma unroll
        for (int o = 128; o > 0; o >>= 1) {
            if (threadIdx.x < 64)
                for (int v = (int)threadIdx.x; v < o; v += 64) s_f[v] += s_f[v + o];
            __syncthreads();
        }
// ... 38 lines not shown
                }
        }
        for (int q = 0; q < n; q++) sum_row(s_rows[q]);
    }
    if (F.done && threadIdx.x == 0) F.result[nrows] = (double)nflagged;
    if (threadIdx.x == 0) {
        __hip_atomic_store(F.ticket, 0u, __ATOMIC_RELAXED, __HIP_MEMORY_SCOPE_AGENT);
        if (F.done) {
            __threadfence_system();
            *F.done = F.seq;
        }
    }
}
#endif

int set_error(int code, const std::string &msg);
inline int fail(int code, const std::string &msg) { return set_error(code, msg); }
#define HIPCHK(call)                                                                                           \
    do {                                                                                                       \
        hipError_t _s = (call);                                                                                \
        if (_s != hipSuccess)                                                                                  \
            return iqhip::set_error(IQHIP_ERR_HIP, std::string(#call) + ": " + hipGetErrorString(_s));        \
    } while (0)

template <typename T>
T *fake_alloc(iqhip_engine *e, size_t count) {
    const uint64_t a = e->fake_next;
    e->fake_next += (count * sizeof(T) + 255) / 256 * 256 + 256;
    return reinterpret_cast<T *>(a);
}
template <typename T>
hipError_t DevBuf<T>::ensure(iqhip_engine *e, size_t count) {
    if (!e->planner) return ensure(e->stream, count);
    if (count > this->cap) {
        this->p = fake_alloc<T>(e, count);
        this->cap = count;
    }
    return hipSuccess;
}
template <typename T>
hipError_t PinBuf<T>::ensure(iqhip_engine *e, size_t count, bool mapped) {
    if (!e->planner) return ensure(e->stream, count, mapped);
    return count <= this->cap ? hipSuccess : this->replace(nullptr, count, MEM_HOST);
}
constexpr unsigned kLdsCeilingDevices = 64;
template <auto Kernel>
hipError_t raise_lds_ceiling(const iqhip_engine *e, int bytes) {
    static std::atomic<bool> raised[kLdsCeilingDevices];
    const unsigned dev = (unsigned)e->device;
    if (dev < kLdsCeilingDevices && raised[dev].load(std::memory_order_relaxed)) return hipSuccess;
    const hipError_t s = hipFuncSetAttribute(reinterpret_cast<const void *>(Kernel), hipFuncAttributeMaxDynamicSharedMemorySize, bytes);
    if (s == hipSuccess && dev < kLdsCeilingDevices) raised[dev].store(true, std::memory_order_relaxed);
    return s;
}
struct PhaseTimer {
    PhaseTimer(iqhip_engine *e_, int nphases_) : e(e_), nphases(nphases_), ok(e_->timing) {}
    PhaseTimer(const PhaseTimer &) = delete; PhaseTimer &operator=(const PhaseTimer &) = delete;
    void mark() {
        hipEvent_t x = nullptr;
        if (!ok || !(ok = hipEventCreate(&x) == hipSuccess)) return;
        ev.push_back(x);
        ok = hipEventRecord(x, e->stream) == hipSuccess;
    }
    bool read(double *ms) {
        const size_t round = (size_t)nphases + 1;
        if (!ok || ev.empty() || ev.size() % round || hipEventSynchronize(ev.back()) != hipSuccess) return false;
        std::vector<double> sum((size_t)nphases, 0.0);
        for (size_t k = 0; k < ev.size(); k += round)
            for (int h = 0; h < nphases; h++) {
                float t = 0.0f;
                if (hipEventElapsedTime(&t, ev[k + h], ev[k + h + 1]) != hipSuccess) return false;
                sum[(size_t)h] += t;
            }
        std::copy(sum.begin(), sum.end(), ms);
        return true;
    }
    ~PhaseTimer() { for (hipEvent_t x : ev) hipEventDestroy(x); }
    iqhip_engine *e;
    int nphases;
    bool ok;
    std::vector<hipEvent_t> ev;
};
int slab_for_key(iqhip_engine *e, uint64_t key, bool create, int *idx);
bool cherry_candidate(const iqhip_engine *e);

int build_plan(iqhip_engine *e, const iqhip_node_op *ops, int nops, int *last_dst,
               const std::vector<int> *explicit_segs = nullptr, const double *const *len_ptrs = nullptr);
int build_branch(iqhip_engine *e, iqhip_branch_end a, iqhip_branch_end b, double len, int prev_dst, DevBranch *br);
int resolve_child(iqhip_engine *e, uint64_t key, int32_t leaf, int prev_dst, const double **plh, const int16_t **sc,
                  const uint8_t **states, int32_t *kind);
bool leaf_tables_follow_model(iqhip_engine *e);
int lds_budget(const iqhip_engine *e);

enum TravVariant : int {
    TRAV_NONE = 0,
    TRAV_GENERIC,
    TRAV_MIX20,
    TRAV_MIX20_SPLIT,
    TRAV_M2,
    TRAV_M2_CAT_SPLIT,
    TRAV_M2_TOP_CS2,
    TRAV_TOP20,
    TRAV_ROWS64,
    TRAV_TOP64,
    TRAV_WIDE4,
};
struct TravLaunch {
    TravVariant variant;
    bool tab;
    int nfull;
    int ngroups;
    int grid;
    size_t lds_bytes;
    int hold_off;
};
TravLaunch choose_traverse_mfma(const iqhip_engine *e, bool top_stage, int nsegs);
inline bool top_stage_may_share_tiles(const iqhip_engine *e) { return e->top_cs2; }
inline bool top_stage_may_mix_roles64(const iqhip_engine *e) { return e->n == 64 && e->mixed_top; }
inline int trav4_ngroups(const iqhip_engine *e) {
    const int wpb = kTravWg / 64;
    return (int)((e->ntiles * e->lane_split + wpb - 1) / wpb);
}
inline bool kernel_takes_small_plan(const iqhip_engine *e) {
    return !e->mfma || (e->mfma_pipelined && e->n == 20 && !e->leaf_tables && e->plan.nleaf_tabs == 0);
}

int comm_allreduce(iqhip_engine *e, int n);
int comm_group_allreduce(const std::vector<iqhip_engine *> &shards, int n);
int comm_init_all(const std::vector<iqhip_engine *> &shards);
void comm_destroy(iqhip_engine *e);
int comm_use_device_result(iqhip_engine *e);

hipError_t use_device(const iqhip_engine *e);
enum : unsigned {
    REQ_SINGLE_DEVICE = 1u << 0,
    REQ_NO_ASC = 1u << 1,
    REQ_PLAIN_STATES = 1u << 2,
    REQ_STATES_4_20_64 = 1u << 3,
    REQ_STATES_4 = 1u << 4,
    REQ_NO_MIXTURE = 1u << 5,
    REQ_MIXTURE = 1u << 6,
    REQ_MODEL_ALN = 1u << 7,
    REQ_THETA = 1u << 8,
};
int require(iqhip_engine *e, const char *what, unsigned needs);
int check_ready(iqhip_engine *e);
int branch_scale_counters(iqhip_engine *e, iqhip_branch_end a, iqhip_branch_end b, const int16_t *sc[2]);
int ensure_slab_rows(iqhip_engine *e, int nrows);
int submit_traverse(iqhip_engine *e, const iqhip_node_op *ops, int nops, bool has_root, iqhip_branch_end a,
                    iqhip_branch_end b, double len, bool skip_reduce = false, const std::vector<int> *explicit_segs = nullptr,
                    const double *const *len_ptrs = nullptr);
int read_result(iqhip_engine *e, int ndoubles);
void set_theta_branch(iqhip_engine *e, const DevBranch &br, iqhip_branch_end a, iqhip_branch_end b);
void result_arrived(iqhip_engine *e);
int eng_repair_lnl(iqhip_engine *e, double *lnl);
extern double debug_build_us;

struct Stopwatch {
    timespec t0;
    void start() { clock_gettime(CLOCK_MONOTONIC, &t0); }
    double us() const {
        timespec t1;
        clock_gettime(CLOCK_MONOTONIC, &t1);
        return (t1.tv_sec - t0.tv_sec) * 1e6 + (t1.tv_nsec - t0.tv_nsec) * 1e-3;
    }
};
// ... 310 lines not shown
```

### iq-tree_amd/csrc/kernels_valu4.hip

```cpp
#include "iqhip_internal.h"
#include "trav_phases.h"

namespace iqhip {

#define CONST_AS __attribute__((address_space(4)))
template <typename T>
__device__ __forceinline__ const CONST_AS T *as_const(const T *p) {
    return (const CONST_AS T *)(p);
}

__device__ __forceinline__ double wave_sum(double v) { return wave_sum64(v); }

template <int C>
__device__ __forceinline__ void load_vec4(const double *__restrict__ base, int64_t tile, int lane,
                                          double (&v)[4 * C]) {
    const double2 *p = reinterpret_cast<const double2 *>(base + tile * (64 * 4 * C)) + lane;
#pragma unroll
    for (int j = 0; j < 2 * C; j++) {
        double2 t = p[j * 64];
        v[2 * j] = t.x;
        v[2 * j + 1] = t.y;
    }
}
template <int C>
__device__ __forceinline__ void store_vec4(double *__restrict__ base, int64_t tile, int lane,
                                           const double (&v)[4 * C]) {
    double2 *p = reinterpret_cast<double2 *>(base + tile * (64 * 4 * C)) + lane;
#pragma unroll
    for (int j = 0; j < 2 * C; j++) p[j * 64] = make_double2(v[2 * j], v[2 * j + 1]);
}

struct Trav4Args {
    const DevOp *ops;
    const double *evec;
    const double *inv_evec;
    const double *tip;
    const double *freq;
    const double *invar;
    const double *eval;
    const double *rates;
    const double *props;
    double *pattern_lh;
    double *slab;
    int64_t ntiles;
    int64_t nptn;
    int64_t nobs;
    const int *segs;
    int ngroups;
    int nwaves;
    int state_unknown;
    int has_root;
    int lds_reg_doubles;
    int state_slots;
    int nsegs_launch;
    int has_load;
    FoldArgs fold;
    DevBranch root;
    int small_plan;
    int small_segs[2];
    DevOp small_ops[kSmallPlanOps];
};

template <int CF>
__device__ __forceinline__ void leaf_cat4(const double *reg , const double *s_tip,
                                          const CONST_AS double *U, int s, int row, bool slow,
                                          int state_unknown, int c, double (&a)[4]) {
    constexpr int B = 4 * CF;
    if (__builtin_expect(slow, 0)) {
        double l[4];
#pragma unroll
        for (int i = 0; i < 4; i++) l[i] = reg[c * 4 + i] * s_tip[s * 4 + i];
#pragma unroll
        for (int x = 0; x < 4; x++) {
            double v = U[x * 4] * l[0];
            v = fma(U[x * 4 + 1], l[1], v);
            v = fma(U[x * 4 + 2], l[2], v);
            v = fma(U[x * 4 + 3], l[3], v);
            a[x] = (s == state_unknown) ? 1.0 : v;
        }
    } else {
        const double2 *tab = reinterpret_cast<const double2 *>(reg + B + row * B + c * 4);
        const double2 v0 = tab[0], v1 = tab[1];
        a[0] = v0.x; a[1] = v0.y; a[2] = v1.x; a[3] = v1.y;
    }
}

template <int C, int CF>
__device__ __forceinline__ double node_update4(bool leafL, bool holdL, bool leafR, const double *regL,
                                               const double *regR, const double *s_tip,
                                               const CONST_AS double *U, const CONST_AS double *uinv,
                                               int sL, int sR, int state_unknown, const char *nx_pf,
                                               char *dst, int coff, double (&PF)[4 * C],
                                               const double (&HOLD)[4 * C], double (&prev)[4 * C]) {
    bool slowL = false, slowR = false;
    int rowL = 0, rowR = 0;
    if (leafL) {
        slowL = __any((sL >= 4) && (sL != state_unknown));
        rowL = sL < 4 ? sL : 4;
    }
    if (leafR) {
        slowR = __any((sR >= 4) && (sR != state_unknown));
        rowR = sR < 4 ? sR : 4;
    }
    double lh_max = 0.0;
#pragma unroll
    for (int c = 0; c < C; c++) {
        double a[4], b[4], tmp[4];
        if (leafL) {
            leaf_cat4<CF>(regL, s_tip, U, sL, rowL, slowL, state_unknown, coff + c, a);
        } else {
            double l[4];
            if (holdL) {
#pragma unroll
                for (int i = 0; i < 4; i++) l[i] = regL[(coff + c) * 4 + i] * HOLD[c * 4 + i];
            } else {
#pragma unroll
                for (int i = 0; i < 4; i++) l[i] = regL[(coff + c) * 4 + i] * PF[c * 4 + i];
            }
#pragma unroll
            for (int x = 0; x < 4; x++) {
                double v = U[x * 4] * l[0];
                v = fma(U[x * 4 + 1], l[1], v);
                v = fma(U[x * 4 + 2], l[2], v);
                a[x] = fma(U[x * 4 + 3], l[3], v);
            }
        }
        if (nx_pf != nullptr) {
            const double2 t0 = *reinterpret_cast<const double2 *>(nx_pf + (2 * c) * 1024);
            const double2 t1 = *reinterpret_cast<const double2 *>(nx_pf + (2 * c + 1) * 1024);
            PF[c * 4] = t0.x; PF[c * 4 + 1] = t0.y; PF[c * 4 + 2] = t1.x; PF[c * 4 + 3] = t1.y;
        }
        if (leafR) {
            leaf_cat4<CF>(regR, s_tip, U, sR, rowR, slowR, state_unknown, coff + c, b);
        } else {
            double r[4];
#pragma unroll
            for (int i = 0; i < 4; i++) r[i] = regR[(coff + c) * 4 + i] * prev[c * 4 + i];
#pragma unroll
            for (int x = 0; x < 4; x++) {
                double v = U[x * 4] * r[0];
                v = fma(U[x * 4 + 1], r[1], v);
                v = fma(U[x * 4 + 2], r[2], v);
                b[x] = fma(U[x * 4 + 3], r[3], v);
            }
        }
#pragma unroll
        for (int x = 0; x < 4; x++) tmp[x] = a[x] * b[x];
#pragma unroll
        for (int i = 0; i < 4; i++) {
            double o = uinv[i * 4] * tmp[0];
            o = fma(uinv[i * 4 + 1], tmp[1], o);
            o = fma(uinv[i * 4 + 2], tmp[2], o);
            o = fma(uinv[i * 4 + 3], tmp[3], o);
            prev[c * 4 + i] = o;
            lh_max = fmax(lh_max, fabs(o));
        }
#ifndef IQHIP_ABLATE_NOSTORE
        *reinterpret_cast<double2 *>(dst + (2 * c) * 1024) = make_double2(prev[c * 4], prev[c * 4 + 1]);
        *reinterpret_cast<double2 *>(dst + (2 * c + 1) * 1024) = make_double2(prev[c * 4 + 2], prev[c * 4 + 3]);
#endif
    }
    return (leafL && leafR) ? 0.0 : lh_max;
}

template <int C>
__device__ __forceinline__ void load_vec4_off(const double *base, uint32_t voff, double (&v)[4 * C]) {
    const char *p = reinterpret_cast<const char *>(base) + voff;
#pragma unroll
    for (int j = 0; j < 2 * C; j++) {
        const double2 t = *reinterpret_cast<const double2 *>(p + j * 1024);
        v[2 * j] = t.x;
        v[2 * j + 1] = t.y;
    }
}
template <int C>
__device__ __forceinline__ void store_vec4_off(double *base, uint32_t voff, const double (&v)[4 * C]) {
    char *p = reinterpret_cast<char *>(base) + voff;
#pragma unroll
    for (int j = 0; j < 2 * C; j++)
        *reinterpret_cast<double2 *>(p + j * 1024) = make_double2(v[2 * j], v[2 * j + 1]);
}

__device__ __forceinline__ void lds_barrier() { asm volatile("s_waitcnt lgkmcnt(0)\n\ts_barrier" ::: "memory"); }
#ifdef IQHIP_T4_TRACE
__device__ unsigned long long g_t4[8];
#define T4_CLK() (t4_on ? (unsigned long long)clock64() : 0ull)
#else
#define T4_CLK() 0ull
#endif
template <int C, bool HAS_LOAD, int SP>
__global__ __launch_bounds__(kTravWg, 2) void k_traverse4(const Trav4Args A) {
    static_assert(SP == 1 || (SP == 2 && C % 2 == 0), "SP = 2 needs an even category count");
    constexpr int B = 4 * C;
    constexpr int CL = C / SP, BL = 4 * CL;
    constexpr int WPB = kTravWg / 64;
    extern __shared__ __attribute__((aligned(16))) double smem[];
    constexpr Trav4Lds L = trav4_lds(B);
    double *s_tip = smem + L.s_tip;
    double *s_val = smem + L.s_val;
    double *s_reg = smem + L.s_reg;
    uint8_t *s_states = reinterpret_cast<uint8_t *>(s_reg + A.lds_reg_doubles);

    __shared__ double s_model[32];
    __shared__ int s_opi[64][4];
    __shared__ double s_opl[64][2];
    __shared__ const uint8_t *s_row[kTrav4RowSlots];
    const int nst = A.state_unknown + 1;
    for (int t = threadIdx.x; t < nst * 4; t += kTravWg) s_tip[t] = A.tip[t];
    for (int t = threadIdx.x; t < 20 + C; t += kTravWg) s_model[t] = t < 16 ? A.evec[t] : (t < 20 ? A.eval[t - 16] : A.rates[t - 20]);
    if (A.has_root && threadIdx.x < B) {
        const int c = threadIdx.x >> 2, i = threadIdx.x & 3;
        s_val[threadIdx.x] = exp(A.eval[i] * (A.rates[c] * A.root.len)) * A.props[c];
    }

    const int lane = threadIdx.x & 63;
    const int wave = __builtin_amdgcn_readfirstlane(threadIdx.x >> 6);
    uint8_t *const w_states = s_states + wave * (A.state_slots * 64);
    const int seg = (int)blockIdx.x / A.ngroups;
    const CONST_AS char *kargs = (const CONST_AS char *)__builtin_amdgcn_kernarg_segment_ptr();
    const CONST_AS int *segs = A.small_plan ? (const CONST_AS int *)(kargs + offsetof(Trav4Args, small_segs)) : as_const(A.segs);
    const int k_begin = segs[2 * seg], k_end = k_begin + segs[2 * seg + 1];
    const int64_t wtile = (int64_t)((int)blockIdx.x - seg * A.ngroups) * WPB + wave;
    const bool active = wtile < A.ntiles * SP;
    const int64_t wt = active ? wtile : 0;
    const int gw = (int)wt;
    const int64_t tl = wt / SP;
    const int pl = (SP == 1) ? lane : (int)(wt & 1) * 32 + (lane & 31);
    const int hl = (SP == 1) ? 0 : (lane >> 5);
    const int coff = hl * CL;
    const bool lead = (hl == 0);
    const int64_t ptn = tl * 64 + pl;
    const uint32_t voff = (uint32_t)(tl * (64 * B * 8) + pl * 16 + coff * 2048);
    const uint32_t doff = (uint32_t)(lane * 16);
    const uint32_t soff = (uint32_t)(ptn * 2);
    const uint32_t poff = (uint32_t)ptn;

    const double freq = A.freq[ptn];
    const double invar = A.invar[ptn];

    const CONST_AS double *U = as_const(A.evec);
    const CONST_AS double *uinv = as_const(A.inv_evec);
    const CONST_AS DevOp *ops = A.small_plan ? (const CONST_AS DevOp *)(kargs + offsetof(Trav4Args, small_ops)) : as_const(A.ops);

    double prev[BL], PF[BL], HOLD[BL];
    int hold_sc = 0;
    int pf_sc = 0, prev_sc = 0;
#pragma unroll
    for (int e = 0; e < BL; e++) { prev[e] = 0.0; PF[e] = 0.0; }
#pragma unroll
    for (int e = 0; e < BL; e++) HOLD[e] = 0.0;

    if (active) {
        const CONST_AS DevOp *nx = ops + k_begin;
        const int nreal = nx->real_mask;
        load_vec4_off<CL>(nx->pf, (nreal & 1) ? voff : doff, PF);
        pf_sc = *reinterpret_cast<const int16_t *>(reinterpret_cast<const char *>(nx->pf_sc) +
                                                   ((nreal & 1) ? soff : (uint32_t)(lane * 2)));
    }


#ifdef IQHIP_T4_TRACE
    const bool t4_on = (blockIdx.x % 97) == 5 && threadIdx.x == 0;
    unsigned long long t4_fill = 0, t4_head = 0, t4_upd = 0, t4_tail = 0, t4_n = 0, t4_f1 = 0, t4_f2 = 0;
#endif
    int k = k_begin;
    while (k < k_end) {
        const int kn = ops[k].chunk_nops;
        const int nslots = ops[k].chunk_slots;
        [[maybe_unused]] const unsigned long long c0 = T4_CLK();
        __syncthreads();
        for (int t = threadIdx.x; t < kn; t += kTravWg) {
            const CONST_AS DevOp &d = ops[k + t];
            const int slot_l = d.sl_slot, slot_r = d.sr_slot;
            const uint8_t *const row_l = d.sl, *const row_r = d.sr;
            s_row[slot_l] = row_l;
            s_row[slot_r] = row_r;
        }
        auto request_states = [&]() {
            if constexpr (SP == 1) {
                if (active) {
                    constexpr int RB = 4;
                    const int grp = lane >> 4;
                    const int64_t roff = tl * 64 + 4 * (lane & 15);
                    for (int s0 = 1; s0 < nslots; s0 += 4 * RB) {
                        const uint8_t *row[RB];
#pragma unroll
                        for (int r = 0; r < RB; r++) {
                            const int slot = s0 + 4 * r + grp;
                            row[r] = s_row[slot < nslots ? slot : 0];
                        }
#pragma unroll
                        for (int r = 0; r < RB; r++) {
                            if (s0 + 4 * r + grp < nslots)
                                __builtin_amdgcn_global_load_lds((const __attribute__((address_space(1))) void *)(row[r] + roff),
                                                                 (__attribute__((address_space(3))) void *)(w_states + (s0 + 4 * r) * 64), 4, 0, 0);
                        }
                    }
                }
            }
        };
        lds_barrier();
        request_states();
        {
            int touched = 0;
#pragma unroll 4
            for (int o = wave; o < kn; o += WPB) {
                const CONST_AS int *w = reinterpret_cast<const CONST_AS int *>(ops + (k + o));
                touched ^= w[0] ^ w[16] ^ w[32] ^ w[sizeof(DevOp) / 4 - 1];
            }
            asm volatile("" ::"s"(touched));
        }
        [[maybe_unused]] unsigned long long c0a = T4_CLK();
        for (int o0 = 0; o0 < kn; o0 += 64) {
            const int on = kn - o0 < 64 ? kn - o0 : 64;
            if (o0 > 0) lds_barrier();
            for (int t = threadIdx.x; t < on; t += kTravWg) {
                const CONST_AS DevOp &d = ops[k + o0 + t];
                s_opi[t][0] = d.lds_left;
                s_opi[t][1] = d.lds_right;
                s_opi[t][2] = d.left_kind == CHILD_LEAF;
                s_opi[t][3] = d.right_kind == CHILD_LEAF;
                s_opl[t][0] = op_child_len(d, 0);
                s_opl[t][1] = op_child_len(d, 1);
            }
            lds_barrier();
            for (int t = threadIdx.x; t < on * 2 * B; t += kTravWg) {
                const int o = t / (2 * B), r = t - o * (2 * B), child = r / B, e = r - child * B;
                s_reg[s_opi[o][child] + e] = exp(s_model[16 + (e & 3)] * (s_model[20 + (e >> 2)] * s_opl[o][child]));
            }
            lds_barrier();
            c0a = T4_CLK();
            for (int t = threadIdx.x; t < on * 2 * B; t += kTravWg) {
                const int o = t / (2 * B), r = t - o * (2 * B), child = r / B, e = r - child * B, c = e >> 2, x = e & 3;
                if (!s_opi[o][2 + child]) continue;
                double *reg = s_reg + s_opi[o][child];
                const LeafE4 E = leaf_e4(s_model + x * 4, reg + c * 4);
#pragma unroll
                for (int row = 0; row < 4; row++) reg[B + row * B + e] = E.entry(s_tip + row * 4);
                reg[B + 4 * B + e] = 1.0;
            }
        }
        [[maybe_unused]] const unsigned long long c0b = T4_CLK();
        if constexpr (SP == 1) {
            asm volatile("s_waitcnt vmcnt(0)" ::: "memory");
        } else
        if (active) {
            for (int o0 = 0; o0 < kn; o0 += 16) {
                uint8_t vl[16], vr[16];
#pragma unroll
                for (int j = 0; j < 16; j++) {
                    const CONST_AS DevOp *d = ops + (k + (o0 + j < kn ? o0 + j : kn - 1));
                    vl[j] = *(d->sl + poff);
                    vr[j] = *(d->sr + poff);
                }
#pragma unroll
                for (int j = 0; j < 16; j++) {
                    if (o0 + j < kn) {
                        const CONST_AS DevOp *d = ops + (k + o0 + j);
                        w_states[d->sl_slot * 64 + lane] = vl[j];
                        w_states[d->sr_slot * 64 + lane] = vr[j];
                    }
                }
            }
        }
        __syncthreads();
        if (!active) { k += kn; continue; }
#ifdef IQHIP_T4_TRACE
        { const unsigned long long cz = T4_CLK(); t4_fill += cz - c0; t4_f1 += c0a - c0; t4_f2 += c0b - c0a; }
#endif

        for (int kk = 0; kk < kn; kk++, k++) {
            [[maybe_unused]] const unsigned long long c1 = T4_CLK();
            const CONST_AS DevOp *op = ops + k;
            const bool leafL = op->left_kind == CHILD_LEAF;
            const bool holdL = op->left_kind == CHILD_HOLD;
            const bool leafR = op->right_kind == CHILD_LEAF;
            int16_t *const dst_sc_p = op->dst_sc;
            const int out_row = op->out_row, rule = op->no_scale, push_hold = op->push_hold;
            int sc = 0;
            const int sL = w_states[op->sl_slot * 64 + lane];
            const int sR = w_states[op->sr_slot * 64 + lane];
            if (!leafL) sc += holdL ? hold_sc : pf_sc;
            if (HAS_LOAD && op->right_kind == CHILD_LOAD) {
                load_vec4_off<CL>(op->ld, voff, prev);
                prev_sc = *reinterpret_cast<const int16_t *>(reinterpret_cast<const char *>(op->ld_sc) + soff);
            }
            if (!leafR) sc += prev_sc;
            const CONST_AS DevOp *nx = ops + (k + 1);
            const int nreal = nx->real_mask;
            const char *nx_pf = (nreal & 1) ? reinterpret_cast<const char *>(nx->pf) + voff : nullptr;
            if (nreal & 1) pf_sc = *reinterpret_cast<const int16_t *>(reinterpret_cast<const char *>(nx->pf_sc) + soff);
            char *dstp = reinterpret_cast<char *>(op->dst) + voff;
            [[maybe_unused]] const unsigned long long c2 = T4_CLK();
            double lh_max = node_update4<CL, C>(leafL, holdL, leafR, s_reg + op->lds_left, s_reg + op->lds_right,
                                                s_tip, U, uinv, sL, sR, A.state_unknown, nx_pf, dstp, coff, PF, HOLD, prev);
            if (SP == 2) lh_max = fmax(lh_max, __shfl_xor(lh_max, 32, 64));
            [[maybe_unused]] const unsigned long long c3 = T4_CLK() + (lh_max == -1.0 ? 1 : 0);
            const ScaleChoice ch = scale_choice(rule, leafL && leafR, lh_max, invar);
            double my_scale = 0.0;
            const unsigned long long any = __ballot(ch.scale);
            if (__builtin_expect(any != 0, 0)) {
                if (ch.scale) {
                    if (ch.zero) {
#pragma unroll
                        for (int e = 0; e < BL; e++) prev[e] = s_tip[A.state_unknown * 4 + (e & 3)];
                    } else {
#pragma unroll
                        for (int e = 0; e < BL; e++) prev[e] *= kScalingThresholdInv;
                    }
                    sc += ch.events();
                    my_scale = (lead && ptn < A.nptn) ? ch.events() * (kLogScalingThreshold * freq) : 0.0;
#ifndef IQHIP_ABLATE_NOSTORE
                    store_vec4_off<CL>(op->dst, voff, prev);
#endif
                }
            }
            prev_sc = sc;
            if (push_hold) {
#pragma unroll
                for (int e = 0; e < BL; e++) HOLD[e] = prev[e];
                hold_sc = sc;
            }
#ifndef IQHIP_ABLATE_NOSTORE
            if (SP == 1 || lead) *reinterpret_cast<int16_t *>(reinterpret_cast<char *>(dst_sc_p) + soff) = (int16_t)sc;
#endif
            double ws = 0.0;
            if (any) ws = wave_sum(my_scale);
            if (lane == 0) {
                fold_store(&A.slab[(size_t)(2 + out_row) * A.nwaves + gw], ws);
                if (any) fold_flag(A.fold, 2 + out_row);
            }
#ifdef IQHIP_T4_TRACE
            { const unsigned long long c4 = T4_CLK(); t4_head += c2 - c1; t4_upd += c3 - c2; t4_tail += c4 - c3; t4_n++; }
#endif
        }
    }
#ifdef IQHIP_T4_TRACE
    if (t4_on) {
        atomicAdd(&g_t4[0], t4_fill); atomicAdd(&g_t4[1], t4_head); atomicAdd(&g_t4[2], t4_upd); atomicAdd(&g_t4[3], t4_tail);
        atomicAdd(&g_t4[4], t4_n); atomicAdd(&g_t4[5], 1ull); atomicAdd(&g_t4[6], t4_f1); atomicAdd(&g_t4[7], t4_f2);
    }
#endif
    if (k_end == k_begin) __syncthreads();
    if (!active) return;

    if (A.has_root) {
        double Bv[BL];
        const double *sv = s_val + coff * 4;
        if (A.root.b_kind == CHILD_PREV) {
#pragma unroll
            for (int e = 0; e < BL; e++) Bv[e] = prev[e];
        } else {
            load_vec4_off<CL>(A.root.b, voff, Bv);
        }
        double lh = 0.0;
        if (A.root.a_kind == CHILD_LEAF) {
            const int s = A.root.a_states[ptn];
#pragma unroll
            for (int e = 0; e < BL; e++) lh = fma(sv[e] * s_tip[s * 4 + (e & 3)], Bv[e], lh);
        } else {
            double Av[BL];
            if (A.root.a_kind == CHILD_PREV) {
#pragma unroll
                for (int e = 0; e < BL; e++) Av[e] = prev[e];
            } else {
                load_vec4_off<CL>(A.root.a, voff, Av);
            }
#pragma unroll
            for (int e = 0; e < BL; e++) lh = fma(sv[e] * Av[e], Bv[e], lh);
        }
        if (SP == 2) lh += __shfl_xor(lh, 32, 64);
        double pc = 0.0;
        if (A.nobs < A.nptn) {
            if (lead && ptn >= A.nobs && ptn < A.nptn) {
                int ssc = (A.root.b_kind == CHILD_PREV) ? prev_sc : (int)A.root.b_sc[ptn];
                if (A.root.a_kind != CHILD_LEAF) ssc += (A.root.a_kind == CHILD_PREV) ? prev_sc : (int)A.root.a_sc[ptn];
                pc = (ssc >= 1 ? lh * kScalingThreshold : lh) + invar;
            }
        }
        lh += invar;
        const double plh = log(fabs(lh));
        if (SP == 1 || lead) A.pattern_lh[ptn] = plh;
        const double acc = (lead && ptn < A.nobs) ? plh * freq : 0.0;
        const double ws = wave_sum(acc);
        const double wpc = (A.nobs < A.nptn) ? wave_sum(pc) : 0.0;
        if (lane == 0) {
            fold_store(&A.slab[gw], ws);
            fold_store(&A.slab[(size_t)A.nwaves + gw], wpc);
        }
    }
    if (A.fold.enabled) fold_tail(A.fold);
}

template <int C, bool HAS_LOAD, int SP>
static hipError_t launch_trav(iqhip_engine *e, Trav4Args &A) {
    const size_t lds = trav4_lds_bytes(4 * C, e->plan.lds_doubles, e->plan.state_slots);
    (void)raise_lds_ceiling<&k_traverse4<C, HAS_LOAD, SP>>(e, kTrav4MaxLdsBytes);
    A.ngroups = trav4_ngroups(e);
    hipLaunchKernelGGL((k_traverse4<C, HAS_LOAD, SP>), dim3((unsigned)(A.ngroups * A.nsegs_launch)), dim3(kTravWg), lds, e->stream, A);
    return hipGetLastError();
}

template <int C>
static hipError_t launch_trav_c(iqhip_engine *e, Trav4Args &A) {
    if constexpr (C % 2 == 0) {
        if (e->lane_split == 2) return A.has_load ? launch_trav<C, true, 2>(e, A) : launch_trav<C, false, 2>(e, A);
    }
    return A.has_load ? launch_trav<C, true, 1>(e, A) : launch_trav<C, false, 1>(e, A);
}

hipError_t launch_traverse4(iqhip_engine *e, const int *seg_table, int nsegs, bool has_load, const DevBranch *root, int nwaves,
                            int fold_rows) {
#ifdef IQHIP_T4_TRACE
// ... 203 lines not shown
        const double wpc = (nobs < nptn) ? wave_sum(pc) : 0.0;
        if (lane == 0) {
            slab[gw] = wa;
            slab[(size_t)nwaves + gw] = wpc;
        }
    }
}

template <int MODE>
static hipError_t launch_theta_reduce(iqhip_engine *e, double len, int nwaves, const NewtonState *st = nullptr,
                                      const BatchChain *bc = nullptr) {
    const int grid = (int)((e->ntiles + 3) / 4);
    const double *theta = bc ? bc->theta : e->d_theta.p;
    double *plh = bc ? nullptr : e->d_pattern_lh.p;
    const size_t stride = bc ? bc->theta_stride : 0;
    const int ny = bc ? bc->ntasks : 1;
    const int task_rows = (bc && MODE == 0) ? bc->derv_rows : 2;
    const int16_t *const *task_sc = bc ? bc->sc : nullptr;
#define IQ_TR(Cv)                                                                              \
    case Cv:                                                                                   \
        hipLaunchKernelGGL((k_theta_reduce4<Cv, MODE>), dim3(grid, ny), dim3(256), 0, e->stream, \
                           theta, e->d_eval, e->d_rates, e->d_props, len, e->d_freq.p,           \
                           e->d_invar.p, plh, e->d_slab.p, e->ntiles, e->nptn, nwaves,             \
                           e->nptn - e->n_unobs, e->theta_a_sc, e->theta_b_sc, st, stride,     \
                           task_rows, task_sc);                                                \
        break;
    switch (e->ncat) {
        IQ_TR(1) IQ_TR(2) IQ_TR(3) IQ_TR(4) IQ_TR(5) IQ_TR(6) IQ_TR(7) IQ_TR(8)
        default: return hipErrorInvalidValue;
    }
#undef IQ_TR
    return hipGetLastError();
}

hipError_t launch_derv4(iqhip_engine *e, double len, int nwaves, const NewtonState *st, const BatchChain *bc) {
    return launch_theta_reduce<0>(e, len, nwaves, bc ? bc->states : st, bc);
}
hipError_t launch_lnl_theta4(iqhip_engine *e, double len, int nwaves, const BatchChain *bc) {
    return launch_theta_reduce<1>(e, len, nwaves, bc ? bc->states : nullptr, bc);
}

__global__ __launch_bounds__(256) void k_reduce(const double *__restrict__ slab, int nwaves,
                                                int first_row, double *__restrict__ result, unsigned int *ticket,
                                                volatile unsigned long long *done, unsigned long long seq) {
    __shared__ double s[256];
    const double *row = slab + (size_t)(first_row + blockIdx.x) * nwaves;
    double acc = 0.0;
    for (int i = threadIdx.x; i < nwaves; i += 256) acc += row[i];
    s[threadIdx.x] = acc;
    __syncthreads();
#pragma unroll
    for (int o = 128; o > 0; o >>= 1) {
        if ((int)threadIdx.x < o) s[threadIdx.x] += s[threadIdx.x + o];
        __syncthreads();
    }
    if (threadIdx.x == 0) {
        result[first_row + blockIdx.x] = s[0];
        if (done) {
            __threadfence_system();
            const unsigned int t = __hip_atomic_fetch_add(ticket, 1u, __ATOMIC_RELAXED, __HIP_MEMORY_SCOPE_AGENT);
            if (t == gridDim.x - 1) {
                __hip_atomic_store(ticket, 0u, __ATOMIC_RELAXED, __HIP_MEMORY_SCOPE_AGENT);
                __threadfence_system();
                *done = seq;
            }
        }
    }
}

hipError_t launch_reduce(iqhip_engine *e, int first_row, int nrows, int nwaves) {
    if (nrows <= 0) return hipSuccess;
    unsigned long long *done = nullptr;
    unsigned long long seq = 0;
    if (e->poll_result && e->d_result == e->d_result_own) {
        seq = ++e->result_seq;
        done = e->d_done;
        e->poll_pending = true;
    }
    hipLaunchKernelGGL(k_reduce, dim3(nrows), dim3(256), 0, e->stream, e->d_slab.p, nwaves,
                       first_row, e->d_result, e->d_fold_ticket.p + 1, done, seq);
    return hipGetLastError();
}

}
```

### iq-tree_amd/csrc/plan.hip

```cpp
#include <math.h>
#include <stdio.h>
#include <stdlib.h>
#include <string.h>

#include <algorithm>
#include <unordered_set>

#include "iqhip_internal.h"

using namespace iqhip;

namespace {

int fail(int code, const std::string &msg) { return set_error(code, msg); }
constexpr int kSentinels = 2;

int devops_for(size_t bytes) { return (int)((bytes + sizeof(DevOp) - 1) / sizeof(DevOp)); }

struct Units {
    std::vector<int> order;
    std::vector<int> seg_of;
    std::vector<std::pair<int, int>> units;
    std::vector<int> stage_units;
    int top_begin = 0;
};

int segment_table_ops(const Units &u) { return devops_for(sizeof(int) * 2 * (1 + u.units.size())); }

int ensure_plan_capacity(iqhip_engine *e, int nops) {
    if ((size_t)nops <= std::min(e->d_ops.cap, e->h_ops.cap)) return IQHIP_OK;
    const size_t cap = (size_t)std::max(64, nops * 2);
    e->plan_cache.uploaded.clear();
    HIPCHK(e->d_ops.ensure(e, cap));
    if (e->h_ops.ensure(e, cap) != hipSuccess) return fail(IQHIP_ERR_NOMEM, "plan staging");
    return IQHIP_OK;
}

void dummy_op(const iqhip_engine *e, DevOp &d) {
    memset(&d, 0, sizeof(d));
    d.dst = e->dummy.plh.p;
    d.dst_sc = e->dummy.sc.p;
    d.pf = d.ld = e->dummy.plh.p;
    d.pf_sc = d.ld_sc = e->dummy.sc.p;
    d.sl = d.sr = e->d_states.p;
    d.tabL = d.tabR = e->d_leaf_tab.p;
}

bool plan_is_cached(const iqhip_engine *e, const iqhip_node_op *ops, int nops, const std::vector<int> *explicit_segs,
                    const double *const *len_ptrs) {
    const PlanCache &c = e->plan_cache;
    const size_t in_bytes = sizeof(iqhip_node_op) * (size_t)nops;
    return !len_ptrs && nops > 0 && c.version == e->keymap_version && c.ops_in.size() == in_bytes &&
           memcmp(c.ops_in.data(), ops, in_bytes) == 0 && !c.uploaded.empty() &&
           (explicit_segs ? c.segs == *explicit_segs : c.segs.empty()) &&
           (!e->plan.uses_cherry || e->plan.cherry_model == e->model_version);
}

int cut_explicit(const iqhip_node_op *ops, int nops, const std::vector<int> &segs, Units &u) {
    std::unordered_set<uint64_t> dsts;
    for (int k = 0; k < nops; k++)
        if (!dsts.insert(ops[k].dst_key).second)
            return fail(IQHIP_ERR_INVALID, "batched node updates must write distinct vectors");
    int pos = 0;
    for (const int n : segs) {
        if (n <= 0) continue;
        if (pos + n > nops) break;
        u.units.push_back({pos, n});
        for (int q = 0; q < n; q++) u.seg_of[pos + q] = (int)u.units.size();
        pos += n;
    }
    if (pos != nops) return fail(IQHIP_ERR_INVALID, "segment sizes do not add up to the op count");
    u.stage_units.push_back((int)u.units.size());
    u.top_begin = nops;
    return IQHIP_OK;
}

int unit_target(const iqhip_engine *e, int nops) {
    if (e->split_target >= 0) return e->split_target;
    const int64_t simds = (int64_t)e->num_cus * 4;
    int target = 0;
    if (e->mfma && e->ntiles < 6 * simds && nops >= 12)
        target = (int)std::min<int64_t>(nops / 2, std::max<int64_t>(3, ((int64_t)nops * e->ntiles + 4 * simds - 1) / (4 * simds)));
    if (!e->mfma && e->ntiles * e->lane_split <= simds && nops >= 12) target = std::max(6, nops / 4);
    return target;
}

bool producer_links(const iqhip_node_op *ops, int nops, std::vector<int> &lc, std::vector<int> &rc) {
    std::unordered_map<uint64_t, int> prod;
    std::unordered_set<uint64_t> ext_in;
    std::vector<char> consumed(nops, 0);
    lc.assign(nops, -1);
    rc.assign(nops, -1);
    for (int k = 0; k < nops; k++) {
        const iqhip_node_op &o = ops[k];
        for (int side = 0; side < 2; side++) {
            if ((side ? o.right_leaf : o.left_leaf) >= 0) continue;
            const uint64_t key = side ? o.right_key : o.left_key;
            auto it = prod.find(key);
            if (it == prod.end()) { ext_in.insert(key); continue; }
            if (consumed[it->second]++) return false;
            (side ? rc : lc)[k] = it->second;
        }
        if (!prod.emplace(o.dst_key, k).second) return false;
    }
    for (int k = 0; k < nops; k++)
        if (ext_in.count(ops[k].dst_key)) return false;
    return true;
}

void cut_subtrees(int nops, int target, int max_levels, const std::vector<int> &lc, const std::vector<int> &rc, Units &u) {
    std::vector<char> placed(nops, 0);
    std::vector<int> new_order;
    new_order.reserve(nops);
    const int min_top = std::max(2, std::min(target, 6));
    for (int level = 0; level < max_levels && nops - (int)new_order.size() > min_top; level++) {
        std::vector<int> rem;
        for (int k = 0; k < nops; k++)
            if (!placed[k]) rem.push_back(k);
        const int R = (int)rem.size();
        std::vector<int> pos_of(nops, -1), l2(R, -1), r2(R, -1), sz(R, 1);
        std::vector<char> cont(R, 1), cons(R, 0);
        for (int q = 0; q < R; q++) pos_of[rem[q]] = q;
        for (int q = 0; q < R; q++) {
            const int k = rem[q];
            if (lc[k] >= 0 && !placed[lc[k]]) { l2[q] = pos_of[lc[k]]; cons[l2[q]] = 1; sz[q] += sz[l2[q]]; }
            if (rc[k] >= 0 && !placed[rc[k]]) { r2[q] = pos_of[rc[k]]; cons[r2[q]] = 1; sz[q] += sz[r2[q]]; }
            const int a = std::max(l2[q], r2[q]), b2 = std::min(l2[q], r2[q]);
            bool c2 = true;
            if (a >= 0) c2 = (a == q - 1) && cont[a];
            if (b2 >= 0) c2 = c2 && (b2 == a - sz[a]) && cont[b2];
            cont[q] = c2;
        }
        std::vector<int> stack;
        for (int q = R - 1; q >= 0; q--)
            if (!cons[q]) stack.push_back(q);
        std::vector<std::pair<int, int>> found;
        while (!stack.empty()) {
            const int q = stack.back();
            stack.pop_back();
            if (sz[q] <= target && sz[q] >= 2 && cont[q]) {
                found.push_back({q, sz[q]});
            } else {
                if (l2[q] >= 0) stack.push_back(l2[q]);
                if (r2[q] >= 0) stack.push_back(r2[q]);
            }
        }
        if (found.size() < 2) break;
        std::stable_sort(found.begin(), found.end(),
                         [](const std::pair<int, int> &x, const std::pair<int, int> &y2) { return x.second > y2.second; });
        for (const std::pair<int, int> &f : found) {
            u.units.push_back({(int)new_order.size(), f.second});
            for (int q = f.first - f.second + 1; q <= f.first; q++) {
                u.seg_of[new_order.size()] = (int)u.units.size();
                placed[rem[q]] = 1;
                new_order.push_back(rem[q]);
            }
        }
        u.stage_units.push_back((int)found.size());
    }
    if (u.units.empty()) return;
    u.top_begin = (int)new_order.size();
    for (int k = 0; k < nops; k++)
        if (!placed[k]) { u.seg_of[new_order.size()] = 0; new_order.push_back(k); }
    u.order = std::move(new_order);
}

int cut_units(const iqhip_engine *e, const iqhip_node_op *ops, int nops, const std::vector<int> *explicit_segs, Units &u) {
    u.order.resize(nops);
    for (int k = 0; k < nops; k++) u.order[k] = k;
    u.seg_of.assign(nops, 0);
    if (explicit_segs) {
        const int rc = cut_explicit(ops, nops, *explicit_segs, u);
        if (rc) return rc;
    } else {
        const int target = unit_target(e, nops);
        std::vector<int> lc, rc;
        if (target > 0 && target < nops && nops >= 4 && producer_links(ops, nops, lc, rc))
            cut_subtrees(nops, target, e->max_levels, lc, rc, u);
    }
    if (e->debug_plan) {
        fprintf(stderr, "[iqhip] plan: %d ops, %zu stages of units (", nops, u.stage_units.size());
        size_t ui = 0;
        for (int n : u.stage_units) {
            for (int q = 0; q < n; q++) fprintf(stderr, "%d ", u.units[ui++].second);
            fprintf(stderr, "| ");
        }
        fprintf(stderr, ") top %d ops\n", nops - u.top_begin);
    }
    return IQHIP_OK;
}

int fill_descriptors(iqhip_engine *e, const iqhip_node_op *ops, int nops, const Units &u, const double *const *len_ptrs,
                     int *last_dst) {
    int prev_dst = -1;
    for (int k = 0; k < nops; k++) {
        const iqhip_node_op &o = ops[u.order[k]];
        DevOp &d = e->h_ops.p[k];
        dummy_op(e, d);
        d.out_row = u.order[k];
        d.no_scale = (o.flags & IQHIP_OP_NO_SCALE) ? 1 : (((o.flags & IQHIP_OP_SCALAR_RULE) || e->scalar_rule_all) ? 2 : 0);
        if (k > 0 && u.seg_of[k] != u.seg_of[k - 1]) prev_dst = -1;
        if (!(o.left_len >= 0.0) || !(o.right_len >= 0.0))
            return fail(IQHIP_ERR_INVALID, "negative or NaN branch length");
        const double *lp, *rp; const int16_t *lsc, *rsc;
        const uint8_t *lst, *rst; int32_t lkind, rkind;
        int rc = resolve_child(e, o.left_key, o.left_leaf, prev_dst, &lp, &lsc, &lst, &lkind);
        if (rc) return rc;
        rc = resolve_child(e, o.right_key, o.right_leaf, prev_dst, &rp, &rsc, &rst, &rkind);
        if (rc) return rc;
        int didx;
        rc = slab_for_key(e, o.dst_key, true, &didx);
        if (rc) return rc;
        if ((lkind != CHILD_LEAF && lp == e->slabs[didx].plh.p) || (rkind != CHILD_LEAF && rp == e->slabs[didx].plh.p))
            return fail(IQHIP_ERR_INVALID, "node update writes onto one of its own children");
        if (lkind == CHILD_PREV && rkind == CHILD_PREV)
            return fail(IQHIP_ERR_INVALID, "node update uses the same vector for both children");
        double llen = o.left_len, rlen = o.right_len;
        const double *llen_p = len_ptrs ? len_ptrs[2 * u.order[k]] : nullptr, *rlen_p = len_ptrs ? len_ptrs[2 * u.order[k] + 1] : nullptr;
        d.dst = e->slabs[didx].plh.p;
        d.dst_sc = e->slabs[didx].sc.p;
        if (e->mfma && !e->mfma_pipelined) {
            if (lkind != CHILD_LEAF) { lkind = CHILD_LOAD; d.pf = lp; d.pf_sc = lsc; } else d.sl = lst;
            if (rkind != CHILD_LEAF) { rkind = CHILD_LOAD; d.ld = rp; d.ld_sc = rsc; } else d.sr = rst;
        } else {
            auto swap_children = [&]() {
                std::swap(lp, rp); std::swap(lsc, rsc); std::swap(lst, rst);
                std::swap(lkind, rkind); std::swap(llen, rlen); std::swap(llen_p, rlen_p);
            };
            if (lkind == CHILD_PREV) swap_children();
            else if (lkind == CHILD_LEAF && rkind == CHILD_LOAD) swap_children();
            if (lkind == CHILD_LOAD) lkind = CHILD_PF;
            if (rkind == CHILD_LOAD) (u.seg_of[k] ? e->plan.units_have_load : e->plan.has_load) = true;
            if (lkind == CHILD_PF) { d.pf = lp; d.pf_sc = lsc; d.real_mask |= 1; }
            if (rkind == CHILD_LOAD) { d.ld = rp; d.ld_sc = rsc; }
            if (lkind == CHILD_LEAF) d.sl = lst;
            if (rkind == CHILD_LEAF) d.sr = rst;
        }
        d.left_kind = lkind; d.right_kind = rkind;
        d.left_len = llen; d.right_len = rlen;
        d.left_len_p = llen_p; d.right_len_p = rlen_p;
        prev_dst = didx;
    }
    *last_dst = prev_dst;
    return IQHIP_OK;
}

void park_operands(iqhip_engine *e, int nops, const std::vector<int> &seg_of) {
    const bool hold_regs = !e->mfma;
    const bool hold_in_lds = e->mfma && e->mfma_pipelined && e->hold_lds && e->n == 20 && !e->cat_split;
    std::unordered_map<const double *, int> producer;
    for (int k = 0; k < nops && (hold_regs || hold_in_lds); k++) {
        DevOp &d = e->h_ops.p[k];
        const auto it = d.left_kind == CHILD_PF ? producer.find(d.pf) : producer.end();
        const int j = it == producer.end() ? -1 : it->second;
        producer[d.dst] = k;
        if (j < 0) continue;
        bool ok = !e->h_ops.p[j].push_hold && seg_of[j] == seg_of[k];
        if (hold_in_lds && top_stage_may_share_tiles(e) && seg_of[k] == 0) ok = false;
        for (int q = j + 1; q < k && ok; q++) {
            const DevOp &m = e->h_ops.p[q];
            ok = m.left_kind != CHILD_PF && m.left_kind != CHILD_HOLD && m.right_kind != CHILD_LOAD && !m.push_hold;
        }
        if (!ok) continue;
        e->h_ops.p[j].push_hold = 1;
        d.left_kind = CHILD_HOLD;
        d.pf = e->dummy.plh.p;
        d.pf_sc = e->dummy.sc.p;
        d.real_mask &= ~1;
        e->plan.nhold++;
    }
    if (e->debug_plan) {
        int npf = 0;
        for (int k = 0; k < nops; k++) npf += (e->h_ops.p[k].left_kind == CHILD_PF) + (e->h_ops.p[k].right_kind == CHILD_LOAD);
        fprintf(stderr, "[iqhip] plan: %d children read back from memory, %d parked\n", npf, e->plan.nhold);
    }
}

int assign_leaf_tables(iqhip_engine *e, int nops) {
    if (!(e->mfma && e->mfma_pipelined && e->leaf_tables)) return IQHIP_OK;
    const size_t per = leaf_table_doubles(e);
    leaf_tables_follow_model(e);
    struct Use { double len; const double *len_p; int slot; };
    std::unordered_map<int, std::vector<Use>> seen;
    int noverflow = 0;
    std::vector<TabJob> dirty, clean;
    std::vector<std::pair<int, int>> uses;
    std::vector<int> use_slot;
    for (int k = 0; k < nops; k++) {
        const DevOp &d = e->h_ops.p[k];
        for (int side = 0; side < 2; side++) {
            if ((side ? d.right_kind : d.left_kind) != CHILD_LEAF) continue;
            const uint8_t *row = side ? d.sr : d.sl;
            const int taxon = (int)((row - e->d_states.p) / e->nptn_pad);
            const double *len_p = side ? d.right_len_p : d.left_len_p;
            const double len = len_p ? NAN : (side ? d.right_len : d.left_len);
            std::vector<Use> &u = seen[taxon];
            int slot = -1;
            for (const Use &x : u)
                if (x.len_p == len_p && (len_p || x.len == len)) slot = x.slot;
            if (slot < 0) {
                slot = u.empty() ? taxon : e->ntaxa + noverflow++;
                u.push_back({len, len_p, slot});
                const TabJob j = {len, reinterpret_cast<double *>((size_t)slot), len_p, 0.0};
                const bool cached = !len_p && slot < e->ntaxa && (size_t)slot < e->tab_len.size() && e->tab_len[slot] == len;
                (cached ? clean : dirty).push_back(j);
            }
            uses.push_back({k, side});
            use_slot.push_back(slot);
        }
    }
    const size_t need = (size_t)e->ntaxa + (size_t)noverflow;
    if (need > e->d_leaf_tab.cap / per) {
        HIPCHK(e->d_leaf_tab.ensure(e, (need + 16) * per));
        e->plan_cache.uploaded.clear();
        dirty.insert(dirty.end(), clean.begin(), clean.end());
        clean.clear();
        e->tab_len.assign(e->d_leaf_tab.cap / per, NAN);
    }
    if (e->tab_len.size() < e->d_leaf_tab.cap / per) e->tab_len.resize(e->d_leaf_tab.cap / per, NAN);
    for (int k = 0; k < nops; k++) e->h_ops.p[k].tabL = e->h_ops.p[k].tabR = e->d_leaf_tab.p;
    for (size_t q = 0; q < uses.size(); q++) {
        DevOp &d = e->h_ops.p[uses[q].first];
        (uses[q].second ? d.tabR : d.tabL) = e->d_leaf_tab.p + (size_t)use_slot[q] * per;
    }
    for (std::vector<TabJob> *v : {&dirty, &clean})
        for (TabJob &j : *v) {
            const size_t slot = (size_t)j.tab;
            j.tab = e->d_leaf_tab.p + slot * per;
            e->tab_len[slot] = slot < (size_t)e->ntaxa ? j.len : NAN;
            e->plan.tab_jobs.push_back(j);
        }
    e->plan.tab_dirty = (int)dirty.size();
    e->plan.nleaf_tabs = (int)e->plan.tab_jobs.size();
    return IQHIP_OK;
}

int assign_cherry_tables(iqhip_engine *e, int nops, const std::vector<int> &seg_of) {
    const bool have_pair = e->planner ? e->cherry_s2 > 0 : (e->pair && e->cherry_model_synced);
    if (!(cherry_candidate(e) && e->mfma_pipelined && have_pair && nops >= 8)) return IQHIP_OK;
    const size_t per = (size_t)e->cherry_npairs * e->block;
    const size_t want = (size_t)2 * e->ntaxa + 16;
    const bool fresh = e->d_cherry_tab.cap < want * per;
    if (fresh) HIPCHK(e->d_cherry_tab.ensure(e, want * per));
    const size_t cherry_cap = e->d_cherry_tab.cap / per;
    if (fresh || e->cherry_slots.size() + (size_t)e->ntaxa / 2 + 1 > cherry_cap) {
        e->cherry_slot_of.clear();
        e->cherry_slots.clear();
    }
    const uint64_t stamp = ++e->cherry_stamp;
    for (int k = 0; k < nops; k++) {
        DevOp &d = e->h_ops.p[k];
        if (d.left_kind != CHILD_LEAF || d.right_kind != CHILD_LEAF || d.left_len_p || d.right_len_p) continue;
        if ((top_stage_may_share_tiles(e) || top_stage_may_mix_roles64(e)) && seg_of[k] == 0) continue;
        const uint64_t tl = (uint64_t)((d.sl - e->d_states.p) / e->nptn_pad), tr = (uint64_t)((d.sr - e->d_states.p) / e->nptn_pad);
        const uint64_t key = (tl << 32) | tr;
        auto it = e->cherry_slot_of.find(key);
        int slot;
        if (it == e->cherry_slot_of.end()) {
            if (e->cherry_slots.size() >= cherry_cap) continue;
            slot = (int)e->cherry_slots.size();
            e->cherry_slots.emplace_back();
            e->cherry_slot_of[key] = slot;
        } else {
            slot = it->second;
        }
        iqhip_engine::CherrySlot &cs = e->cherry_slots[slot];
        const bool same = cs.len_l == d.left_len && cs.len_r == d.right_len;
        if (cs.stamp == stamp && !same) continue;
        if (!same || cs.model_version != e->model_version) {
            cs.len_l = d.left_len;
            cs.len_r = d.right_len;
            cs.model_version = 0;
            if (cs.stamp != stamp) e->plan.cherry_jobs.push_back(slot);
        }
        cs.stamp = stamp;
        d.cherry = e->d_cherry_tab.p + (size_t)slot * per;
        e->plan.uses_cherry = true;
    }
    return IQHIP_OK;
}

int lay_out_lds(iqhip_engine *e, int nops, const std::vector<int> &seg_of) {
    const int B = e->block, budget = lds_budget(e);
    const bool tables_in_lds = e->mfma && e->mfma_pipelined && e->n == 20 && e->plan.nleaf_tabs > 0;
    const int leaf_sz = (!e->mfma || e->wide4) ? 6 * B : (tables_in_lds ? (int)leaf_table_doubles(e) : B);
    const int slot_sz = e->mfma ? 0 : trav4_lds(B).slot_doubles;
    int chunk_start = 0, used = slot_sz, regs = 0, max_used = 0, slots = 1, max_slots = 1;
    for (int k = 0; k < nops; k++) {
        DevOp &d = e->h_ops.p[k];
        const int szl = d.left_kind == CHILD_LEAF ? leaf_sz : B;
        const int szr = d.right_kind == CHILD_LEAF ? leaf_sz : B;
        const int nleaf = (d.left_kind == CHILD_LEAF) + (d.right_kind == CHILD_LEAF);
        const int need = szl + szr + nleaf * slot_sz;
        if (need > budget) return fail(IQHIP_ERR_UNSUPPORTED, "nstates*ncat too large for the LDS plan regions");
        const bool rows_full = !e->mfma && slots + nleaf > kTrav4RowSlots;
        if ((used + need > budget || rows_full || seg_of[k] != seg_of[k - (k > 0)]) && k > chunk_start) {
            e->h_ops.p[chunk_start].chunk_nops = k - chunk_start;
            e->h_ops.p[chunk_start].chunk_slots = slots;
            chunk_start = k; used = slot_sz; regs = 0; slots = 1;
        }
        d.lds_left = regs; d.lds_right = regs + szl;
        regs += szl + szr;
        used += need;
        if (regs > max_used) max_used = regs;
        d.sl_slot = d.left_kind == CHILD_LEAF ? slots++ : 0;
        d.sr_slot = d.right_kind == CHILD_LEAF ? slots++ : 0;
        if (slots > max_slots) max_slots = slots;
    }
    if (nops > 0) {
        e->h_ops.p[chunk_start].chunk_nops = nops - chunk_start;
        e->h_ops.p[chunk_start].chunk_slots = slots;
    }
    e->plan.state_slots = max_slots;
    e->plan.lds_doubles = max_used;
    return IQHIP_OK;
}

int check_plan(iqhip_engine *e, int nops, int nsentinels) {
    std::unordered_set<const void *> vecs, scs;
    for (const Slab &sl : e->slabs) { vecs.insert(sl.plh.p); scs.insert(sl.sc.p); }
    vecs.insert(e->dummy.plh.p);
    scs.insert(e->dummy.sc.p);
    const size_t per = (e->mfma && e->mfma_pipelined) ? leaf_table_doubles(e) : 0;
    char msg[256];
    auto bad = [&](int k, const char *what) {
        snprintf(msg, sizeof msg, "plan check: op %d of %d (+%d sentinels): %s", k, nops, nsentinels, what);
        return fail(IQHIP_ERR_INVALID, msg);
    };
    auto state_row = [&](const uint8_t *p) {
        if (!p || !e->d_states.p || p < e->d_states.p) return false;
        const size_t off = (size_t)(p - e->d_states.p);
        return off % (size_t)e->nptn_pad == 0 && off / (size_t)e->nptn_pad < (size_t)e->ntaxa;
    };
    auto table = [&](const double *p) {
        if (e->plan.nleaf_tabs == 0 && !e->d_leaf_tab.p) return p == nullptr;
        if (!p || !e->d_leaf_tab.p || p < e->d_leaf_tab.p || per == 0) return false;
        const size_t off = (size_t)(p - e->d_leaf_tab.p);
        return off % per == 0 && off / per < e->d_leaf_tab.cap / per;
    };
    for (int k = 0; k < nops + nsentinels; k++) {
        const DevOp &d = e->h_ops.p[k];
        if (!vecs.count(d.dst) || d.dst == nullptr) return bad(k, "dst is not a vector slab");
        if (!scs.count(d.dst_sc)) return bad(k, "dst_sc is not a counter slab");
        if (!vecs.count(d.pf)) return bad(k, "pf (streamed child) is not a vector slab / the dummy slab");
        if (!scs.count(d.pf_sc)) return bad(k, "pf_sc is not a counter slab / the dummy");
        if (!vecs.count(d.ld)) return bad(k, "ld (second memory child) is not a vector slab / the dummy slab");
        if (!scs.count(d.ld_sc)) return bad(k, "ld_sc is not a counter slab / the dummy");
        if (!state_row(d.sl) || !state_row(d.sr)) return bad(k, "sl / sr is not a row of the state matrix");
        if (!table(d.tabL) || !table(d.tabR)) return bad(k, "tabL / tabR is not a K2 table slot");
        if (d.cherry) {
            const size_t cper = (size_t)e->cherry_npairs * e->block;
            if (!e->d_cherry_tab.p || cper == 0 || d.cherry < e->d_cherry_tab.p || (size_t)(d.cherry - e->d_cherry_tab.p) % cper != 0 ||
                (size_t)(d.cherry - e->d_cherry_tab.p) / cper >= e->d_cherry_tab.cap / cper || k >= nops || d.left_kind != CHILD_LEAF ||
                d.right_kind != CHILD_LEAF)
                return bad(k, "cherry is not a cherry-table slot of an op with two leaf children");
        }
        if (k >= nops) continue;
        if (d.dst == e->dummy.plh.p || d.dst_sc == e->dummy.sc.p) return bad(k, "a real op writes the dummy slab");
        const bool lk = d.left_kind == CHILD_LEAF || d.left_kind == CHILD_PF || d.left_kind == CHILD_HOLD ||
                        (d.left_kind == CHILD_LOAD && e->mfma && !e->mfma_pipelined);
        const bool rk = d.right_kind == CHILD_LEAF || d.right_kind == CHILD_PREV || d.right_kind == CHILD_LOAD;
        if (!lk || !rk) return bad(k, "child kinds are not in canonical form");
        if (d.left_kind == CHILD_PF && (d.pf == e->dummy.plh.p || !(d.real_mask & 1))) return bad(k, "streamed child without a real vector");
        if (d.left_kind != CHILD_PF && !(e->mfma && !e->mfma_pipelined) && (d.real_mask & 1)) return bad(k, "real_mask set without a streamed child");
        if (d.right_kind == CHILD_LOAD && d.ld == e->dummy.plh.p) return bad(k, "second memory child without a real vector");
        if (d.dst == d.pf || d.dst == d.ld) return bad(k, "op writes one of its own children");
        if (!(d.left_len >= 0.0) || !(d.right_len >= 0.0)) return bad(k, "negative or NaN branch length");
        if (d.out_row < 0 || d.out_row >= nops) return bad(k, "out_row outside the caller's op list");
        if (d.lds_left < 0 || d.lds_right < 0 || d.lds_left > e->plan.lds_doubles || d.lds_right > e->plan.lds_doubles)
            return bad(k, "LDS region outside the launch's allocation");
        if (d.sl_slot < 0 || d.sr_slot < 0 || d.sl_slot >= e->plan.state_slots || d.sr_slot >= e->plan.state_slots)
            return bad(k, "leaf-state slot outside the launch's allocation");
        if (d.chunk_nops < 0 || k + d.chunk_nops > nops) return bad(k, "LDS chunk runs past the plan");
        if (e->wide4) {
            if ((d.left_kind != CHILD_LEAF && d.left_kind != CHILD_LOAD) || (d.right_kind != CHILD_LEAF && d.right_kind != CHILD_LOAD))
                return bad(k, "wide 4-state op is not in the (memory, memory) form");
            if ((d.left_kind == CHILD_LOAD && d.pf == e->dummy.plh.p) || (d.right_kind == CHILD_LOAD && d.ld == e->dummy.plh.p))
                return bad(k, "memory child without a real vector");
            const int szl = (d.left_kind == CHILD_LEAF ? 6 : 1) * e->block, szr = (d.right_kind == CHILD_LEAF ? 6 : 1) * e->block;
            if (d.lds_left + szl > e->plan.lds_doubles || d.lds_right + szr > e->plan.lds_doubles ||
                (d.lds_left < d.lds_right + szr && d.lds_right < d.lds_left + szl))
                return bad(k, "LDS regions of the two children overlap or leave the launch's allocation");
            if (d.no_scale < 0 || d.no_scale > 2) return bad(k, "unknown scaling rule");
        }
    }
    for (int k = 0; k < nops;) {
        const DevOp &c = e->h_ops.p[k];
        if (c.chunk_nops <= 0) return bad(k, "op is not covered by an LDS chunk");
        if (!e->mfma) {
            int next = 1, regs = 0;
            for (int q = k; q < k + c.chunk_nops; q++) {
                const DevOp &d = e->h_ops.p[q];
                if (d.sl_slot != (d.left_kind == CHILD_LEAF ? next : 0)) return bad(q, "leaf-state slots of the chunk are not 1 .. n in op order");
                next += d.left_kind == CHILD_LEAF;
                if (d.sr_slot != (d.right_kind == CHILD_LEAF ? next : 0)) return bad(q, "leaf-state slots of the chunk are not 1 .. n in op order");
                next += d.right_kind == CHILD_LEAF;
                const int szl = (d.left_kind == CHILD_LEAF ? 6 : 1) * e->block, szr = (d.right_kind == CHILD_LEAF ? 6 : 1) * e->block;
                regs = std::max(regs, std::max(d.lds_left + szl, d.lds_right + szr));
            }
            if (c.chunk_slots != next) return bad(k, "chunk_slots is not the chunk's slot count");
            if (next > kTrav4RowSlots) return bad(k, "more leaf-state slots than the kernel's row-pointer list holds");
            if (next > e->plan.state_slots || regs > e->plan.lds_doubles ||
                regs + next * trav4_lds(e->block).slot_doubles > lds_budget(e))
                return bad(k, "LDS chunk outside the launch's allocation or over the budget");
        }
        k += c.chunk_nops;
    }
    const int *tab = reinterpret_cast<const int *>(e->h_ops.p + e->plan.table_off);
    int covered = 0;
    for (int u = 0; u <= e->plan.nunits; u++) {
        const int b = tab[2 * u], n = tab[2 * u + 1];
        if (b < 0 || n < 0 || b + n > nops) return bad(b, "segment outside the plan");
        covered += n;
    }
    if (covered != nops) return bad(nops, "segments do not cover the plan exactly once");
    return IQHIP_OK;
}

int upload_plan(iqhip_engine *e, size_t nbytes) {
    if (e->planner) return IQHIP_OK;
    std::vector<char> &up = e->plan_cache.uploaded;
    const char *h = reinterpret_cast<const char *>(e->h_ops.p);
    if (e->plan.small) {
    } else if (up.size() == nbytes && memcmp(up.data(), h, nbytes) == 0) {
        return IQHIP_OK;
    } else if (e->plan_arena_on && e->plan_arena_used + nbytes <= e->h_plan_arena.cap) {
        char *slice = e->h_plan_arena.p + e->plan_arena_used;
        memcpy(slice, h, nbytes);
        e->plan_arena_used += (nbytes + 255) / 256 * 256;
        HIPCHK(hipMemcpyAsync(e->d_ops.p, slice, nbytes, hipMemcpyHostToDevice, e->stream));
    } else {
        HIPCHK(hipMemcpyAsync(e->d_ops.p, e->h_ops.p, nbytes, hipMemcpyHostToDevice, e->stream));
        HIPCHK(hipEventRecord(e->staging_free, e->stream));
        e->staging_busy = true;
    }
    up.assign(h, h + nbytes);
    return IQHIP_OK;
}

int finish_and_upload(iqhip_engine *e, const iqhip_node_op *ops, int nops, Units &u, const std::vector<int> *explicit_segs,
                      const double *const *len_ptrs, int last_dst) {
    Plan &p = e->plan;
    for (int q = 0; q < kSentinels; q++) dummy_op(e, e->h_ops.p[nops + q]);
    p.table_off = nops + kSentinels;
    const int table_ops = segment_table_ops(u);
    int *tab = reinterpret_cast<int *>(e->h_ops.p + p.table_off);
    memset(tab, 0, sizeof(DevOp) * (size_t)table_ops);
    tab[0] = u.top_begin; tab[1] = nops - u.top_begin;
    for (size_t i = 0; i < u.units.size(); i++) { tab[2 + 2 * i] = u.units[i].first; tab[3 + 2 * i] = u.units[i].second; }
    p.nunits = (int)u.units.size();
    p.stage_units = std::move(u.stage_units);
    p.top_nops = nops - u.top_begin;
    p.jobs_off = p.table_off + table_ops;
    const int jobs_ops = devops_for(sizeof(TabJob) * p.tab_jobs.size());
    if (jobs_ops > 0) {
        memset(e->h_ops.p + p.jobs_off, 0, sizeof(DevOp) * (size_t)jobs_ops);
        memcpy(e->h_ops.p + p.jobs_off, p.tab_jobs.data(), sizeof(TabJob) * p.tab_jobs.size());
    }
    PlanCache &c = e->plan_cache;
    c.ops_in.assign((const char *)ops, (const char *)(ops + nops));
    c.segs = explicit_segs ? *explicit_segs : std::vector<int>();
    c.version = len_ptrs ? 0 : e->keymap_version;
    c.dst = last_dst;
    p.small = e->small_plans && kernel_takes_small_plan(e) && !explicit_segs && u.units.empty() && nops > 0 && nops + kSentinels <= kSmallPlanOps;
    p.small_nops = nops;
    if (e->planner && nops > 0) {
        const std::string &br = e->debug_break_plan;
        if (br == "tab") e->h_ops.p[nops - 1].tabL = nullptr;
        else if (br == "sentinel") e->h_ops.p[nops + kSentinels - 1].pf = nullptr;
        else if (br == "states") e->h_ops.p[0].sr = nullptr;
        else if (br == "cherry")
            for (int k = 0; k < nops; k++)
                if (e->h_ops.p[k].cherry) { e->h_ops.p[k].cherry += 8; break; }
    }
    if (e->check_plans) {
        const int rc = check_plan(e, nops, kSentinels);
        if (rc) { c.invalidate(); return rc; }
    }
    return upload_plan(e, sizeof(DevOp) * (size_t)(p.jobs_off + jobs_ops));
}

}

namespace iqhip {

int resolve_child(iqhip_engine *e, uint64_t key, int32_t leaf, int prev_dst, const double **plh, const int16_t **sc,
                  const uint8_t **states, int32_t *kind) {
    *plh = nullptr; *sc = nullptr; *states = nullptr;
    if (leaf >= 0) {
        if (leaf >= e->ntaxa) return fail(IQHIP_ERR_INVALID, "leaf id out of range");
        *states = e->d_states.p + (size_t)leaf * e->nptn_pad;
        *kind = CHILD_LEAF;
        return IQHIP_OK;
    }
    int idx;
    int rc = slab_for_key(e, key, false, &idx);
    if (rc) return rc;
    *plh = e->slabs[idx].plh.p;
    *sc = e->slabs[idx].sc.p;
    *kind = (idx == prev_dst) ? CHILD_PREV : CHILD_LOAD;
    return IQHIP_OK;
}

int build_branch(iqhip_engine *e, iqhip_branch_end a, iqhip_branch_end b, double len, int prev_dst, DevBranch *br) {
    if (!(len >= 0.0)) return fail(IQHIP_ERR_INVALID, "negative or NaN branch length");
    if (a.leaf >= 0 && b.leaf >= 0)
        return fail(IQHIP_ERR_INVALID, "branch with two leaf ends (2-taxon tree) is not supported");
    if (b.leaf >= 0) std::swap(a, b);
    const uint8_t *st_unused;
    int rc = resolve_child(e, a.key, a.leaf, prev_dst, &br->a, &br->a_sc, &br->a_states, &br->a_kind);
    if (rc) return rc;
    rc = resolve_child(e, b.key, b.leaf, prev_dst, &br->b, &br->b_sc, &st_unused, &br->b_kind);
    if (rc) return rc;
    br->len = len;
    return IQHIP_OK;
}

bool leaf_tables_follow_model(iqhip_engine *e) {
    if (e->tab_model_version == e->model_version) return false;
    std::fill(e->tab_len.begin(), e->tab_len.end(), NAN);
    const size_t per = leaf_table_doubles(e);
    for (const TabJob &j : e->plan.tab_jobs) {
        const size_t slot = (size_t)(j.tab - e->d_leaf_tab.p) / per;
        if (slot < (size_t)e->ntaxa) e->tab_len[slot] = j.len;
    }
    e->tab_model_version = e->model_version;
    return true;
}

constexpr int kRows64BudgetSlack = 128;

int lds_budget(const iqhip_engine *e) {
    const int B = e->block, nx = e->state_unknown + 1 - e->n;
    if (!e->mfma) return e->lds_budget_bytes / 8 - trav4_lds(B).s_reg;
    if (e->wide4) {
        const int kb = e->mfma_lds_kb >= 0 ? e->mfma_lds_kb : kWide4LdsKb;
        return kb * 1024 / 8 - std::max(wide4_lds(e->nclass, B).sReg, generic_lds(4, nx).sReg);
    }
    int fixed = !e->mfma_pipelined ? generic_lds(e->n, nx).sReg
                : e->row_split     ? rows64_lds(nx).sReg + kRows64BudgetSlack
                                   : mfma2_lds(e->n, nx).sReg;
    if (e->mfma_pipelined && e->n == 64) fixed = std::max(fixed, rows64_lds(nx).sReg + kRows64BudgetSlack);
    const int total_kb = e->mfma_lds_kb >= 0 ? e->mfma_lds_kb : (e->n == 20 ? 75 : 78);
    if (e->plan.nhold > 0) fixed += mfma2_park_doubles(B);
    int budget = (total_kb * 1024) / 8 - fixed;
    if (e->mfma_lds_kb < 0 && !e->mfma_pipelined && budget < 2 * B) budget = kTravMaxLdsBytes / 8 - fixed;
    return budget;
}

TravLaunch choose_traverse_mfma(const iqhip_engine *e, bool top_stage, int nsegs) {
    const int n = e->n, C = e->ncat, nx = e->state_unknown + 1 - n, regs = e->plan.lds_doubles;
    const int64_t tiles = e->ntiles;
    TravLaunch L = {TRAV_NONE, false, 0, 0, 0, 0, -1};
    int fixed = 0, waves_per_tile = 1;
    if (!e->mfma_pipelined) {
        if (e->wide4 && !e->wide4_generic) {
            L.variant = TRAV_WIDE4;
            fixed = wide4_lds(e->nclass, e->block).sReg;
        } else if (n == 20) {
            L.variant = e->mix_split ? TRAV_MIX20_SPLIT : TRAV_MIX20;
            waves_per_tile = e->mix_split ? 4 : 1;
            fixed = mix20_lds().sReg;
        } else if (n == 64 || n == 4) {
            L.variant = TRAV_GENERIC;
            fixed = generic_lds(n, nx).sReg;
        }
    } else if ((n == 20 && (C == 4 || C == 1)) || (n == 64 && C == 1)) {
        L.tab = e->plan.nleaf_tabs > 0 || e->leaf_tables;
        L.variant = TRAV_M2;
        fixed = mfma2_lds(n, nx).sReg;
        if (n == 64) {
            const int64_t per_round = (int64_t)e->num_cus * 4, rounds = tiles / per_round, rest = tiles - rounds * per_round;
            if (e->row_split) {
                L.variant = TRAV_ROWS64;
                waves_per_tile = 4;
                fixed = rows64_lds(nx).sReg;
            } else if (top_stage && nsegs == 1 && top_stage_may_mix_roles64(e) && rounds >= 1 && rest > 0 && rest <= per_round / 2) {
                L.variant = TRAV_TOP64;
                L.nfull = (int)(rounds * e->num_cus);
                L.ngroups = (int)(tiles - (int64_t)L.nfull * 4);
                fixed = top64_fixed_doubles(nx);
            }
        } else if (C == 4 && e->cat_split) {
            L.variant = TRAV_M2_CAT_SPLIT;
            waves_per_tile = 4;
        } else if (C == 4 && !L.tab && top_stage && top_stage_may_share_tiles(e)) {
            const int64_t per_round = (int64_t)e->num_cus * 3 * 2, rounds = tiles / per_round, rest = tiles - rounds * per_round;
            L.variant = TRAV_M2_TOP_CS2;
            waves_per_tile = 2;
            if (e->mixed_top && nsegs == 1 && rounds >= 1 && rest > 0 && rest <= per_round / 4) {
                L.variant = TRAV_TOP20;
                L.nfull = (int)(rounds * e->num_cus * 3);
                L.ngroups = (int)(tiles - (int64_t)L.nfull * 2);
            }
        }
    }
    if (L.variant == TRAV_NONE) return L;
    if (L.nfull > 0) L.grid = L.nfull + L.ngroups;
    else {
        L.ngroups = (int)((tiles * waves_per_tile + kTravWg / 64 - 1) / (kTravWg / 64));
        L.grid = L.ngroups * nsegs;
    }
    L.lds_bytes = (size_t)(fixed + regs) * sizeof(double);
    if (L.variant == TRAV_M2 && n < 64 && e->plan.nhold > 0) {
        L.hold_off = fixed + regs;
        L.lds_bytes += (size_t)mfma2_park_doubles(e->block) * sizeof(double);
    }
    return L;
}

int build_plan(iqhip_engine *e, const iqhip_node_op *ops, int nops, int *last_dst, const std::vector<int> *explicit_segs,
               const double *const *len_ptrs) {
    if (nops + 2 > e->result_cap) return fail(IQHIP_ERR_INVALID, "too many node updates in one submission");
    if (plan_is_cached(e, ops, nops, explicit_segs, len_ptrs)) {
        *last_dst = e->plan_cache.dst;
        return IQHIP_OK;
    }
    e->plan_cache.version = 0;
    if (e->staging_busy) {
        HIPCHK(hipEventSynchronize(e->staging_free));
        e->staging_busy = false;
    }
    e->plan = Plan();
    e->plan.cherry_model = e->model_version;
    Units u;
    int rc = cut_units(e, ops, nops, explicit_segs, u);
    if (!rc) rc = ensure_plan_capacity(e, nops + kSentinels + segment_table_ops(u) + devops_for(sizeof(TabJob) * (size_t)(2 * nops + 1)));
    if (!rc) rc = fill_descriptors(e, ops, nops, u, len_ptrs, last_dst);
    if (!rc) park_operands(e, nops, u.seg_of);
    if (!rc) rc = assign_leaf_tables(e, nops);
    if (!rc) rc = assign_cherry_tables(e, nops, u.seg_of);
    if (!rc) rc = lay_out_lds(e, nops, u.seg_of);
    if (!rc) rc = finish_and_upload(e, ops, nops, u, explicit_segs, len_ptrs, *last_dst);
    return rc;
}

}
```

### iq-tree_amd/csrc/trav_lds.h

```cpp
#pragma once
#include <hip/hip_runtime.h>

namespace iqhip {

constexpr int kTravWg = 256;
constexpr int kTravMaxLdsBytes = 150 * 1024;
constexpr int kTravGenericMaxLdsBytes = 160 * 1024;
constexpr int kTrav4MaxLdsBytes = 152 * 1024;

__host__ __device__ constexpr int tipx_doubles(int n, int nx) { return nx * n; }

struct GenericLds { int sU, sUi, sTipx, sReg; };
__host__ __device__ constexpr GenericLds generic_lds(int n, int nx) {
    const int img = ((n + 15) / 16) * (n / 4) * 64;
    return {0, img, 2 * img, 2 * img + tipx_doubles(n, nx)};
}

struct Mfma2Lds { int sU, sUi, sU4, sUi4, sUiT, sTipx, sReg; bool tip_copy; };
__host__ __device__ constexpr Mfma2Lds mfma2_lds(int n, int nx) {
    const int ks = n / 4;
    const int img1 = n < 64 ? 0 : (n / 16) * ks * 64, img4 = (n < 64 || n % 16 != 4) ? 0 : ks * 64;
    const bool tip_copy = n * n * 8 <= 4096;
    const int tipx = 2 * img1 + 2 * img4 + (tip_copy ? n * n : 0);
    return {0, img1, 2 * img1, 2 * img1 + img4, 2 * img1 + 2 * img4, tipx, tipx + tipx_doubles(n, nx), tip_copy};
}
__host__ __device__ constexpr int mfma2_park_doubles(int block) { return (kTravWg / 64) * 16 * block; }

struct Rows64Lds { int sTip, sX, sT, sReg; };
__host__ __device__ constexpr Rows64Lds rows64_lds(int nx) {
    const int tip = (64 + nx) * 64, slices = 2 * 16 * 64;
    return {0, tip, tip + slices, tip + 2 * slices};
}

struct Mix20Lds { int sReg; };
__host__ __device__ constexpr Mix20Lds mix20_lds() { return {0}; }

__host__ __device__ constexpr int top64_fixed_doubles(int nx) {
    return mfma2_lds(64, nx).sReg > rows64_lds(nx).sReg ? mfma2_lds(64, nx).sReg : rows64_lds(nx).sReg;
}

struct Wide4Lds { int sW, sTipc, sReg; };
__host__ __device__ constexpr Wide4Lds wide4_lds(int nclass, int block) { return {0, 32 * nclass, 32 * nclass + 4 * block}; }
constexpr int kWide4LdsKb = 40;

constexpr int kTrav4RowSlots = 256;
struct Trav4Lds { int s_tip, s_val, s_reg, slot_doubles; };
__host__ __device__ constexpr Trav4Lds trav4_lds(int block) { return {0, 128, 128 + block, kTravWg / 8}; }
__host__ __device__ constexpr size_t trav4_lds_bytes(int block, int lds_doubles, int state_slots) {
    return ((size_t)trav4_lds(block).s_reg + (size_t)lds_doubles + (size_t)state_slots * trav4_lds(block).slot_doubles) * sizeof(double);
}

}
```

Measured before the change: 34330 M updates/s.

## Fold cherry nodes into pair-code tables and skip writing their partials

Adds a CHILD_PAIR child kind. Cherries whose two children are plain-state leaves are no longer computed as separate ops. Their parent instead looks up a 25-row table indexed by the combined pair code, built in LDS from the two leaf tables. The removed cherry slabs are marked virtual and only expanded on demand when a later call needs them. This is meant to cut the global memory stores and loads and the op count for cherry nodes. In exchange it adds per-chunk table construction, more LDS use, a bigger descriptor and lazy-expansion bookkeeping.

```diff
diff --git a/include/iqhip.h b/include/iqhip.h
--- a/include/iqhip.h
+++ b/include/iqhip.h
@@ -291,6 +291,10 @@
 #define IQHIP_PLAN_LAYOUT_NSLOTS 8
 int iqhip_debug_plan_layout(iqhip_engine *e, int32_t *out, int nops);
 
+int iqhip_debug_pair_children(iqhip_engine *e, int64_t *ops_removed, int64_t *slabs_expanded, int64_t *last_plan_removed);
+int iqhip_debug_planner_plain_taxa(iqhip_engine *e, const uint8_t *plain);
+int iqhip_debug_plan_removed(iqhip_engine *e, int32_t *out, int nrows);
+
 void iqhip_debug_memory(int64_t *device_bytes, int64_t *host_bytes);
 void iqhip_debug_fail_alloc(int nth);
 
diff --git a/iq-tree_amd/__init__.py b/iq-tree_amd/__init__.py
--- a/iq-tree_amd/__init__.py
+++ b/iq-tree_amd/__init__.py
@@ -25,7 +25,7 @@
     "iqhip_comm_size", "iqhip_update_partials_async", "iqhip_lnl_from_theta_async",
     "iqhip_newton_host_init", "iqhip_newton_host_update", "iqhip_newton_host_result",
     "iqhip_debug_create_planner", "iqhip_debug_plan", "iqhip_timing_plan_bytes", "iqhip_timing_collective_read", "iqhip_optimize_sweep", "iqhip_debug_cherry_tables",
-    "iqhip_debug_path_counts", "iqhip_debug_plan_shape", "iqhip_debug_plan_layout", "iqhip_debug_memory", "iqhip_debug_fail_alloc",
+    "iqhip_debug_path_counts", "iqhip_debug_plan_shape", "iqhip_debug_plan_layout", "iqhip_debug_pair_children", "iqhip_debug_planner_plain_taxa", "iqhip_debug_plan_removed", "iqhip_debug_memory", "iqhip_debug_fail_alloc",
     "iqhip_ptnlh_reserve", "iqhip_ptnlh_put_current", "iqhip_ptnlh_fetch", "iqhip_optimize_branch_batch_rows",
     "iqhip_branch_tests", "iqhip_ptnlh_rell",
     "iqhip_ptnlh_upload", "iqhip_gen_boot_samples", "iqhip_ptnlh_diff_variance", "iqhip_tree_tests", "iqhip_multiscale_bp",
diff --git a/iq-tree_amd/csrc/engine.hip b/iq-tree_amd/csrc/engine.hip
--- a/iq-tree_amd/csrc/engine.hip
+++ b/iq-tree_amd/csrc/engine.hip
@@ -244,6 +244,12 @@
     auto it = e->key2slab.find(key);
     if (it != e->key2slab.end()) {
         *idx = it->second;
+        Slab &s = e->slabs[*idx];
+        if (s.virt && !create && !e->planner) {
+            HIPCHK(launch_pair_expand(e, s));
+            e->pair_slabs_expanded++;
+        }
+        s.virt = false;
         return IQHIP_OK;
     }
     if (!create) return fail(IQHIP_ERR_INVALID, "unknown partial_lh key (vector never computed)");
@@ -251,6 +257,18 @@
     if (rc) return rc;
     e->key2slab[key] = *idx;
     e->keymap_version++;
+    return IQHIP_OK;
+}
+
+int iqhip::expand_virtual_slabs(iqhip_engine *e) {
+    if (e->planner) return IQHIP_OK;
+    for (Slab &s : e->slabs) {
+        if (!s.virt) continue;
+        HIPCHK(use_device(e));
+        HIPCHK(launch_pair_expand(e, s));
+        e->pair_slabs_expanded++;
+        s.virt = false;
+    }
     return IQHIP_OK;
 }
 
@@ -276,6 +294,7 @@
     if (!e->shards.empty()) return sharded::release(e, key);
     auto it = e->key2slab.find(key);
     if (it == e->key2slab.end()) return IQHIP_OK;
+    e->slabs[it->second].virt = false;
     e->free_slabs.push_back(it->second);
     e->key2slab.erase(it);
     e->keymap_version++;
@@ -331,6 +350,10 @@
         return fail(IQHIP_ERR_INVALID,
                     "iqhip_set_alignment: call iqhip_set_model first (needs state_unknown)");
     HIPCHK(use_device(e));
+    {
+        const int rc = expand_virtual_slabs(e);
+        if (rc) return rc;
+    }
     const size_t P = (size_t)e->nptn_pad, N = (size_t)e->nptn;
     std::vector<uint8_t> tmp((size_t)e->ntaxa * P, (uint8_t)(e->embed2 ? e->n : e->state_unknown));
     for (int t = 0; t < e->ntaxa; t++) {
@@ -350,6 +373,14 @@
     }
     HIPCHK(hipMemcpyAsync(e->d_states.p, tmp.data(), tmp.size(), hipMemcpyHostToDevice, e->stream));
     HIPCHK(hipStreamSynchronize(e->stream));
+    e->taxon_plain.assign((size_t)e->ntaxa, 1);
+    for (int t = 0; t < e->ntaxa; t++)
+        for (size_t p = 0; p < P; p++) {
+            const uint8_t st = tmp[(size_t)t * P + p];
+            if (st >= 4 && st != (uint8_t)e->state_unknown) { e->taxon_plain[t] = 0; break; }
+        }
+    e->pair_row_of.clear();
+    e->plan_cache.invalidate();
     e->pars_ready = false;
     int rc = iqhip_set_ptn_freq(e, ptn_freq);
     if (rc) return rc;
@@ -383,6 +414,11 @@
     if (e->aln_set && state_unknown != e->state_unknown)
         return fail(IQHIP_ERR_INVALID, "iqhip_set_model: state_unknown changed after set_alignment");
     if (nclass < 1 || nclass > e->ncat) return fail(IQHIP_ERR_INVALID, "bad number of mixture classes");
+    if (e->model_set) {
+        HIPCHK(use_device(e));
+        const int rc = expand_virtual_slabs(e);
+        if (rc) return rc;
+    }
     if (e->n == 4 && !e->wide4) {
         const bool want_mfma = nclass > 1;
         if (want_mfma != e->mfma) {
@@ -700,7 +736,13 @@
     int last_dst = -1;
     Stopwatch watch;
     if (e->debug_sweep) watch.start();
+    e->n_root_end_keys = 0;
+    if (has_root) {
+        if (a.leaf < 0) e->root_end_keys[e->n_root_end_keys++] = a.key;
+        if (b.leaf < 0) e->root_end_keys[e->n_root_end_keys++] = b.key;
+    }
     rc = build_plan(e, ops, nops, &last_dst, explicit_segs, len_ptrs);
+    e->n_root_end_keys = 0;
     if (rc) return rc;
     if (e->debug_sweep) debug_build_us += watch.us();
     DevBranch br;
@@ -962,6 +1004,31 @@
     return IQHIP_OK;
 }
 
+extern "C" int iqhip_debug_pair_children(iqhip_engine *e, int64_t *ops_removed, int64_t *slabs_expanded, int64_t *last_plan_removed) {
+    if (!e) return fail(IQHIP_ERR_INVALID, "null engine");
+    if (!e->shards.empty()) e = e->shards[0];
+    if (ops_removed) *ops_removed = e->pair_ops_removed;
+    if (slabs_expanded) *slabs_expanded = e->pair_slabs_expanded;
+    if (last_plan_removed) *last_plan_removed = (int64_t)e->plan.virt.size();
+    return IQHIP_OK;
+}
+
+extern "C" int iqhip_debug_planner_plain_taxa(iqhip_engine *e, const uint8_t *plain) {
+    if (!e || !e->planner) return fail(IQHIP_ERR_INVALID, "iqhip_debug_planner_plain_taxa needs a planning-only engine");
+    e->taxon_plain.clear();
+    if (plain) e->taxon_plain.assign(plain, plain + e->ntaxa);
+    e->plan_cache.invalidate();
+    return IQHIP_OK;
+}
+
+extern "C" int iqhip_debug_plan_removed(iqhip_engine *e, int32_t *out, int nrows) {
+    if (!e || !e->planner || !out || nrows != e->plan.nrows)
+        return fail(IQHIP_ERR_INVALID, "iqhip_debug_plan_removed needs a planning-only engine and the last plan's row count");
+    std::fill(out, out + nrows, 1);
+    for (int k = 0; k < e->plan.small_nops; k++) out[e->h_ops.p[k].out_row] = 0;
+    return IQHIP_OK;
+}
+
 extern "C" int iqhip_debug_path_counts(iqhip_engine *e, int64_t *out, int n) {
     if (!e) return fail(IQHIP_ERR_INVALID, "null engine");
     if (!out && n > 0) return fail(IQHIP_ERR_INVALID, "null argument");
@@ -1182,9 +1249,11 @@
             for (int u = 0; u <= e->plan.nunits; u++)
                 if (tab[2 * u + 1] > 0 && tab[2 * u] >= 0 && tab[2 * u] < e->last_nops) seg_first[tab[2 * u]] = 1;
         }
-        for (int k = 0; k < e->last_nops && e->h_ops.p; k++) {
+        const int ndev = (!e->mfma && e->last_nops > 0) ? e->plan.small_nops : e->last_nops;
+        for (int k = 0; k < ndev && e->h_ops.p; k++) {
             const DevOp &d = e->h_ops.p[k];
             st += P * (V + 2.0);
+            ld += P * ((d.left_kind == CHILD_PAIR) + (d.right_kind == CHILD_PAIR));
             const double *held = (hands_over && k > 0 && !seg_first[k]) ? e->h_ops.p[k - 1].dst : nullptr;
             if (d.left_kind == CHILD_LEAF) ld += P;
             else if ((d.left_kind == CHILD_PF || d.left_kind == CHILD_LOAD) && d.pf != held) ld += P * (V + 2.0);
diff --git a/iq-tree_amd/csrc/iqhip_internal.h b/iq-tree_amd/csrc/iqhip_internal.h
--- a/iq-tree_amd/csrc/iqhip_internal.h
+++ b/iq-tree_amd/csrc/iqhip_internal.h
@@ -24,7 +24,10 @@
 constexpr double kScalingThresholdInv = 0x1p256;
 constexpr double kLogScalingThreshold = -177.44567822334599;
 
-enum ChildKind : int32_t { CHILD_LEAF = 0, CHILD_LOAD = 1, CHILD_PREV = 2, CHILD_PF = 3, CHILD_HOLD = 4 };
+enum ChildKind : int32_t { CHILD_LEAF = 0, CHILD_LOAD = 1, CHILD_PREV = 2, CHILD_PF = 3, CHILD_HOLD = 4, CHILD_PAIR = 5 };
+constexpr bool child_is_table(int32_t kind) { return kind == CHILD_LEAF || kind == CHILD_PAIR; }
+constexpr int kPairRows = 25;
+constexpr int child_region_blocks(int32_t kind) { return kind == CHILD_LEAF ? 6 : (kind == CHILD_PAIR ? 1 + kPairRows + 12 : 1); }
 
 struct __attribute__((aligned(16))) DevOp {
     double *dst;
@@ -55,6 +58,8 @@
     const double *cherry;
     int32_t chunk_slots;
     int32_t _pad_slots;
+    double pair_len[4];
+    int32_t pair_row_l, pair_row_r;
 };
 
 #if defined(__HIPCC__)
@@ -170,6 +175,9 @@
     std::vector<int> cherry_jobs;
     bool uses_cherry = false;
     uint64_t cherry_model = 0;
+    struct Virtual { int slab; int32_t taxon_l, taxon_r; double len_l, len_r; };
+    std::vector<Virtual> virt;
+    int nrows = 0;
 };
 
 struct PlanCache {
@@ -327,6 +335,9 @@
 struct Slab {
     DevBuf<double> plh;
     DevBuf<int16_t> sc;
+    bool virt = false;
+    int32_t taxon_l = -1, taxon_r = -1;
+    double len_l = 0.0, len_r = 0.0;
 };
 
 }
@@ -551,6 +562,13 @@
     hipEvent_t staging_free = nullptr;
     bool staging_busy = false;
 
+    std::vector<char> taxon_plain;
+    uint64_t root_end_keys[2] = {0, 0};
+    int n_root_end_keys = 0;
+    iqhip::DevBuf<uint8_t> d_pair_rows;
+    std::unordered_map<uint64_t, int> pair_row_of;
+    int64_t pair_ops_removed = 0, pair_slabs_expanded = 0;
+
     std::unordered_map<uint64_t, int> key2slab;
     std::vector<iqhip::Slab> slabs;
     std::vector<int> free_slabs;
@@ -755,6 +773,9 @@
     std::vector<hipEvent_t> ev;
 };
 int slab_for_key(iqhip_engine *e, uint64_t key, bool create, int *idx);
+int expand_virtual_slabs(iqhip_engine *e);
+hipError_t launch_pair_expand(iqhip_engine *e, const Slab &s);
+hipError_t launch_pair_codes(iqhip_engine *e, const uint8_t *row_l, const uint8_t *row_r, uint8_t *out);
 bool cherry_candidate(const iqhip_engine *e);
 
 int build_plan(iqhip_engine *e, const iqhip_node_op *ops, int nops, int *last_dst,
diff --git a/iq-tree_amd/csrc/kernels_valu4.hip b/iq-tree_amd/csrc/kernels_valu4.hip
--- a/iq-tree_amd/csrc/kernels_valu4.hip
+++ b/iq-tree_amd/csrc/kernels_valu4.hip
@@ -86,7 +86,7 @@
 }
 
 template <int C, int CF>
-__device__ __forceinline__ double node_update4(bool leafL, bool holdL, bool leafR, const double *regL,
+__device__ __forceinline__ double node_update4(bool leafL, bool holdL, bool leafR, bool pairL, bool pairR, const double *regL,
                                                const double *regR, const double *s_tip,
                                                const CONST_AS double *U, const CONST_AS double *uinv,
                                                int sL, int sR, int state_unknown, const char *nx_pf,
@@ -95,12 +95,12 @@
     bool slowL = false, slowR = false;
     int rowL = 0, rowR = 0;
     if (leafL) {
-        slowL = __any((sL >= 4) && (sL != state_unknown));
-        rowL = sL < 4 ? sL : 4;
+        slowL = !pairL && __any((sL >= 4) && (sL != state_unknown));
+        rowL = pairL ? sL : (sL < 4 ? sL : 4);
     }
     if (leafR) {
-        slowR = __any((sR >= 4) && (sR != state_unknown));
-        rowR = sR < 4 ? sR : 4;
+        slowR = !pairR && __any((sR >= 4) && (sR != state_unknown));
+        rowR = pairR ? sR : (sR < 4 ? sR : 4);
     }
     double lh_max = 0.0;
 #pragma unroll
@@ -160,7 +160,7 @@
         *reinterpret_cast<double2 *>(dst + (2 * c + 1) * 1024) = make_double2(prev[c * 4 + 2], prev[c * 4 + 3]);
 #endif
     }
-    return (leafL && leafR) ? 0.0 : lh_max;
+    return (leafL && leafR && !pairL && !pairR) ? 0.0 : lh_max;
 }
 
 template <int C>
@@ -203,7 +203,8 @@
 
     __shared__ double s_model[32];
     __shared__ int s_opi[64][4];
-    __shared__ double s_opl[64][2];
+    __shared__ int s_pair[128], s_npair;
+    __shared__ double s_opl[64][6];
     __shared__ const uint8_t *s_row[kTrav4RowSlots];
     const int nst = A.state_unknown + 1;
     for (int t = threadIdx.x; t < nst * 4; t += kTravWg) s_tip[t] = A.tip[t];
@@ -269,6 +270,7 @@
         const int nslots = ops[k].chunk_slots;
         [[maybe_unused]] const unsigned long long c0 = T4_CLK();
         __syncthreads();
+        if (threadIdx.x == 0) s_npair = 0;
         for (int t = threadIdx.x; t < kn; t += kTravWg) {
             const CONST_AS DevOp &d = ops[k + t];
             const int slot_l = d.sl_slot, slot_r = d.sr_slot;
@@ -306,38 +308,86 @@
 #pragma unroll 4
             for (int o = wave; o < kn; o += WPB) {
                 const CONST_AS int *w = reinterpret_cast<const CONST_AS int *>(ops + (k + o));
-                touched ^= w[0] ^ w[16] ^ w[32] ^ w[sizeof(DevOp) / 4 - 1];
+                static_assert(sizeof(DevOp) > 192 && sizeof(DevOp) <= 256, "one read per 64 bytes of the descriptor");
+                touched ^= w[0] ^ w[16] ^ w[32] ^ w[48] ^ w[sizeof(DevOp) / 4 - 1];
             }
             asm volatile("" ::"s"(touched));
         }
         [[maybe_unused]] unsigned long long c0a = T4_CLK();
         for (int o0 = 0; o0 < kn; o0 += 64) {
             const int on = kn - o0 < 64 ? kn - o0 : 64;
-            if (o0 > 0) lds_barrier();
+            if (o0 > 0) {
+                lds_barrier();
+                if (threadIdx.x == 0) s_npair = 0;
+                lds_barrier();
+            }
             for (int t = threadIdx.x; t < on; t += kTravWg) {
                 const CONST_AS DevOp &d = ops[k + o0 + t];
                 s_opi[t][0] = d.lds_left;
                 s_opi[t][1] = d.lds_right;
-                s_opi[t][2] = d.left_kind == CHILD_LEAF;
-                s_opi[t][3] = d.right_kind == CHILD_LEAF;
+                s_opi[t][2] = d.left_kind == CHILD_LEAF ? 1 : (d.left_kind == CHILD_PAIR ? 2 : 0);
+                s_opi[t][3] = d.right_kind == CHILD_LEAF ? 1 : (d.right_kind == CHILD_PAIR ? 2 : 0);
                 s_opl[t][0] = op_child_len(d, 0);
                 s_opl[t][1] = op_child_len(d, 1);
+#pragma unroll
+                for (int q = 0; q < 4; q++) s_opl[t][2 + q] = d.pair_len[q];
+                if (d.left_kind == CHILD_PAIR) s_pair[atomicAdd(&s_npair, 1)] = 2 * t;
+                if (d.right_kind == CHILD_PAIR) s_pair[atomicAdd(&s_npair, 1)] = 2 * t + 1;
             }
             lds_barrier();
             for (int t = threadIdx.x; t < on * 2 * B; t += kTravWg) {
                 const int o = t / (2 * B), r = t - o * (2 * B), child = r / B, e = r - child * B;
                 s_reg[s_opi[o][child] + e] = exp(s_model[16 + (e & 3)] * (s_model[20 + (e >> 2)] * s_opl[o][child]));
             }
+            const int np = s_npair;
+            for (int t = threadIdx.x; t < np * 2 * B; t += kTravWg) {
+                const int pi = t / (2 * B), r = t - pi * (2 * B), w = r / B, e = r - w * B, o = s_pair[pi] >> 1, child = s_pair[pi] & 1;
+                s_reg[s_opi[o][child] + (1 + kPairRows + 6 * w) * B + e] =
+                    exp(s_model[16 + (e & 3)] * (s_model[20 + (e >> 2)] * s_opl[o][2 + 2 * child + w]));
+            }
             lds_barrier();
             c0a = T4_CLK();
-            for (int t = threadIdx.x; t < on * 2 * B; t += kTravWg) {
-                const int o = t / (2 * B), r = t - o * (2 * B), child = r / B, e = r - child * B, c = e >> 2, x = e & 3;
-                if (!s_opi[o][2 + child]) continue;
-                double *reg = s_reg + s_opi[o][child];
+            auto leaf_table = [&](double *reg, int e) {
+                const int c = e >> 2, x = e & 3;
                 const LeafE4 E = leaf_e4(s_model + x * 4, reg + c * 4);
 #pragma unroll
                 for (int row = 0; row < 4; row++) reg[B + row * B + e] = E.entry(s_tip + row * 4);
                 reg[B + 4 * B + e] = 1.0;
+            };
+            for (int t = threadIdx.x; t < on * 2 * B; t += kTravWg) {
+                const int o = t / (2 * B), r = t - o * (2 * B), child = r / B, e = r - child * B;
+                if (s_opi[o][2 + child] == 1) leaf_table(s_reg + s_opi[o][child], e);
+            }
+            if (np == 0) continue;
+            for (int t = threadIdx.x; t < np * 2 * B; t += kTravWg) {
+                const int pi = t / (2 * B), r = t - pi * (2 * B), w = r / B, e = r - w * B, o = s_pair[pi] >> 1, child = s_pair[pi] & 1;
+                leaf_table(s_reg + s_opi[o][child] + (1 + kPairRows + 6 * w) * B, e);
+            }
+            lds_barrier();
+#pragma unroll 1
+            for (int t = threadIdx.x; t < np * C * kPairRows; t += kTravWg) {
+                const int pi = t / (C * kPairRows), q = t - pi * (C * kPairRows), c = q / kPairRows, code = q - c * kPairRows;
+                const int o = s_pair[pi] >> 1, child = s_pair[pi] & 1, sa = code / 5, sb = code - 5 * sa;
+                double *reg = s_reg + s_opi[o][child];
+                const double *ta = reg + (2 + kPairRows + sa) * B + c * 4, *tb = reg + (8 + kPairRows + sb) * B + c * 4;
+                double tmp[4], l[4];
+#pragma unroll
+                for (int x = 0; x < 4; x++) tmp[x] = __dmul_rn(ta[x], tb[x]);
+#pragma unroll
+                for (int i = 0; i < 4; i++) {
+                    double v = __dmul_rn(uinv[i * 4], tmp[0]);
+                    v = fma(uinv[i * 4 + 1], tmp[1], v);
+                    v = fma(uinv[i * 4 + 2], tmp[2], v);
+                    v = fma(uinv[i * 4 + 3], tmp[3], v);
+                    l[i] = __dmul_rn(reg[c * 4 + i], v);
+                }
+#pragma unroll
+                for (int x = 0; x < 4; x++) {
+                    double v = __dmul_rn(U[x * 4], l[0]);
+                    v = fma(U[x * 4 + 1], l[1], v);
+                    v = fma(U[x * 4 + 2], l[2], v);
+                    reg[B + code * B + c * 4 + x] = fma(U[x * 4 + 3], l[3], v);
+                }
             }
         }
         [[maybe_unused]] const unsigned long long c0b = T4_CLK();
@@ -372,9 +422,12 @@
         for (int kk = 0; kk < kn; kk++, k++) {
             [[maybe_unused]] const unsigned long long c1 = T4_CLK();
             const CONST_AS DevOp *op = ops + k;
-            const bool leafL = op->left_kind == CHILD_LEAF;
+            const bool pairL = op->left_kind == CHILD_PAIR, pairR = op->right_kind == CHILD_PAIR;
+            const bool leafL = op->left_kind == CHILD_LEAF || pairL;
             const bool holdL = op->left_kind == CHILD_HOLD;
-            const bool leafR = op->right_kind == CHILD_LEAF;
+            const bool leafR = op->right_kind == CHILD_LEAF || pairR;
+            const bool tip_tip = leafL && leafR && !pairL && !pairR;
+            const int pair_row_l = op->pair_row_l, pair_row_r = op->pair_row_r;
             int16_t *const dst_sc_p = op->dst_sc;
             const int out_row = op->out_row, rule = op->no_scale, push_hold = op->push_hold;
             int sc = 0;
@@ -392,11 +445,11 @@
             if (nreal & 1) pf_sc = *reinterpret_cast<const int16_t *>(reinterpret_cast<const char *>(nx->pf_sc) + soff);
             char *dstp = reinterpret_cast<char *>(op->dst) + voff;
             [[maybe_unused]] const unsigned long long c2 = T4_CLK();
-            double lh_max = node_update4<CL, C>(leafL, holdL, leafR, s_reg + op->lds_left, s_reg + op->lds_right,
+            double lh_max = node_update4<CL, C>(leafL, holdL, leafR, pairL, pairR, s_reg + op->lds_left, s_reg + op->lds_right,
                                                 s_tip, U, uinv, sL, sR, A.state_unknown, nx_pf, dstp, coff, PF, HOLD, prev);
             if (SP == 2) lh_max = fmax(lh_max, __shfl_xor(lh_max, 32, 64));
             [[maybe_unused]] const unsigned long long c3 = T4_CLK() + (lh_max == -1.0 ? 1 : 0);
-            const ScaleChoice ch = scale_choice(rule, leafL && leafR, lh_max, invar);
+            const ScaleChoice ch = scale_choice(rule, tip_tip, lh_max, invar);
             double my_scale = 0.0;
             const unsigned long long any = __ballot(ch.scale);
             if (__builtin_expect(any != 0, 0)) {
@@ -429,6 +482,8 @@
             if (lane == 0) {
                 fold_store(&A.slab[(size_t)(2 + out_row) * A.nwaves + gw], ws);
                 if (any) fold_flag(A.fold, 2 + out_row);
+                if (pair_row_l >= 0) fold_store(&A.slab[(size_t)(2 + pair_row_l) * A.nwaves + gw], 0.0);
+                if (pair_row_r >= 0) fold_store(&A.slab[(size_t)(2 + pair_row_r) * A.nwaves + gw], 0.0);
             }
 #ifdef IQHIP_T4_TRACE
             { const unsigned long long c4 = T4_CLK(); t4_head += c2 - c1; t4_upd += c3 - c2; t4_tail += c4 - c3; t4_n++; }
@@ -798,4 +853,82 @@
     return hipGetLastError();
 }
 
-}
+__global__ __launch_bounds__(256) void k_pair_codes(const uint8_t *__restrict__ row_l, const uint8_t *__restrict__ row_r,
+                                                    uint8_t *__restrict__ out, int64_t nptn_pad) {
+    const int64_t p = (int64_t)blockIdx.x * 256 + threadIdx.x;
+    if (p >= nptn_pad) return;
+    const int a = row_l[p], b = row_r[p];
+    out[p] = (uint8_t)(5 * (a < 4 ? a : 4) + (b < 4 ? b : 4));
+}
+
+hipError_t launch_pair_codes(iqhip_engine *e, const uint8_t *row_l, const uint8_t *row_r, uint8_t *out) {
+    hipLaunchKernelGGL(k_pair_codes, dim3((unsigned)((e->nptn_pad + 255) / 256)), dim3(256), 0, e->stream, row_l, row_r, out, e->nptn_pad);
+    return hipGetLastError();
+}
+
+template <int C>
+__global__ __launch_bounds__(256) void k_pair_expand(const uint8_t *__restrict__ row_l, const uint8_t *__restrict__ row_r, double len_l,
+                                                     double len_r, const double *__restrict__ evec, const double *__restrict__ inv_evec,
+                                                     const double *__restrict__ eval, const double *__restrict__ rates,
+                                                     const double *__restrict__ tip, double *__restrict__ dst,
+                                                     int16_t *__restrict__ dst_sc, int64_t ntiles) {
+    constexpr int B = 4 * C;
+    __shared__ double s_u[16], s_ui[16], s_tip[16], s_ex[2][B], s_tab[kPairRows * B];
+    if (threadIdx.x < 16) {
+        s_u[threadIdx.x] = evec[threadIdx.x];
+        s_ui[threadIdx.x] = inv_evec[threadIdx.x];
+        s_tip[threadIdx.x] = tip[threadIdx.x];
+    }
+    if (threadIdx.x < 2 * B) {
+        const int w = threadIdx.x / B, e = threadIdx.x - w * B;
+        s_ex[w][e] = exp(eval[e & 3] * (rates[e >> 2] * (w ? len_r : len_l)));
+    }
+    __syncthreads();
+    for (int t = threadIdx.x; t < C * kPairRows; t += 256) {
+        const int c = t / kPairRows, code = t - c * kPairRows, sa = code / 5, sb = code - 5 * sa;
+        double tmp[4];
+#pragma unroll
+        for (int x = 0; x < 4; x++) {
+            const double a = sa == 4 ? 1.0 : leaf_e4(s_u + x * 4, s_ex[0] + c * 4).entry(s_tip + sa * 4);
+            const double b = sb == 4 ? 1.0 : leaf_e4(s_u + x * 4, s_ex[1] + c * 4).entry(s_tip + sb * 4);
+            tmp[x] = __dmul_rn(a, b);
+        }
+#pragma unroll
+        for (int i = 0; i < 4; i++) {
+            double v = __dmul_rn(s_ui[i * 4], tmp[0]);
+            v = fma(s_ui[i * 4 + 1], tmp[1], v);
+            v = fma(s_ui[i * 4 + 2], tmp[2], v);
+            s_tab[code * B + c * 4 + i] = fma(s_ui[i * 4 + 3], tmp[3], v);
+        }
+    }
+    __syncthreads();
+    const int lane = threadIdx.x & 63;
+    const int64_t tile = (int64_t)blockIdx.x * 4 + (threadIdx.x >> 6);
+    if (tile >= ntiles) return;
+    const int64_t ptn = tile * 64 + lane;
+    const int a = row_l[ptn], b = row_r[ptn];
+    const double *v = s_tab + (5 * (a < 4 ? a : 4) + (b < 4 ? b : 4)) * B;
+    double2 *p = reinterpret_cast<double2 *>(dst + tile * (64 * B)) + lane;
+#pragma unroll
+    for (int j = 0; j < 2 * C; j++) p[j * 64] = make_double2(v[2 * j], v[2 * j + 1]);
+    dst_sc[ptn] = 0;
+}
+
+hipError_t launch_pair_expand(iqhip_engine *e, const Slab &s) {
+    const size_t P = (size_t)e->nptn_pad;
+    const uint8_t *row_l = e->d_states.p + (size_t)s.taxon_l * P, *row_r = e->d_states.p + (size_t)s.taxon_r * P;
+    const int grid = (int)((e->ntiles + 3) / 4);
+#define IQ_PX(Cv)                                                                                                          \
+    case Cv:                                                                                                               \
+        hipLaunchKernelGGL(k_pair_expand<Cv>, dim3(grid), dim3(256), 0, e->stream, row_l, row_r, s.len_l, s.len_r, e->d_evec, \
+                           e->d_inv_evec, e->d_eval, e->d_rates, e->d_tip, s.plh.p, s.sc.p, e->ntiles);                    \
+        break;
+    switch (e->ncat) {
+        IQ_PX(1) IQ_PX(2) IQ_PX(3) IQ_PX(4) IQ_PX(5) IQ_PX(6) IQ_PX(7) IQ_PX(8)
+        default: return hipErrorInvalidValue;
+    }
+#undef IQ_PX
+    return hipGetLastError();
+}
+
+}
diff --git a/iq-tree_amd/csrc/plan.hip b/iq-tree_amd/csrc/plan.hip
--- a/iq-tree_amd/csrc/plan.hip
+++ b/iq-tree_amd/csrc/plan.hip
@@ -44,12 +44,18 @@
     d.pf_sc = d.ld_sc = e->dummy.sc.p;
     d.sl = d.sr = e->d_states.p;
     d.tabL = d.tabR = e->d_leaf_tab.p;
+    d.pair_row_l = d.pair_row_r = -1;
 }
 
 bool plan_is_cached(const iqhip_engine *e, const iqhip_node_op *ops, int nops, const std::vector<int> *explicit_segs,
                     const double *const *len_ptrs) {
     const PlanCache &c = e->plan_cache;
     const size_t in_bytes = sizeof(iqhip_node_op) * (size_t)nops;
+    for (int q = 0; q < e->n_root_end_keys; q++) {
+        const auto it = e->key2slab.find(e->root_end_keys[q]);
+        for (const Plan::Virtual &v : e->plan.virt)
+            if (it != e->key2slab.end() && it->second == v.slab) return false;
+    }
     return !len_ptrs && nops > 0 && c.version == e->keymap_version && c.ops_in.size() == in_bytes &&
            memcmp(c.ops_in.data(), ops, in_bytes) == 0 && !c.uploaded.empty() &&
            (explicit_segs ? c.segs == *explicit_segs : c.segs.empty()) &&
@@ -190,28 +196,128 @@
     return IQHIP_OK;
 }
 
+struct PairDef { int32_t taxon_l, taxon_r; double len_l, len_r; int row; const uint8_t *codes; };
+struct Kept {
+    std::vector<iqhip_node_op> ops;
+    std::vector<int> row;
+    std::unordered_map<uint64_t, PairDef> pairs;
+};
+
+uint64_t pair_key(int32_t tl, int32_t tr) { return ((uint64_t)(uint32_t)tl << 32) | (uint32_t)tr; }
+
+int pair_code_row(iqhip_engine *e, int32_t tl, int32_t tr, const uint8_t **row) {
+    const size_t P = (size_t)e->nptn_pad, nslots = e->d_pair_rows.cap / P;
+    *row = nullptr;
+    auto it = e->pair_row_of.find(pair_key(tl, tr));
+    if (it != e->pair_row_of.end()) { *row = e->d_pair_rows.p + (size_t)it->second * P; return IQHIP_OK; }
+    if (e->pair_row_of.size() >= nslots) return IQHIP_OK;
+    const int slot = (int)e->pair_row_of.size();
+    uint8_t *out = e->d_pair_rows.p + (size_t)slot * P;
+    if (!e->planner) HIPCHK(launch_pair_codes(e, e->d_states.p + (size_t)tl * P, e->d_states.p + (size_t)tr * P, out));
+    e->pair_row_of[pair_key(tl, tr)] = slot;
+    *row = out;
+    return IQHIP_OK;
+}
+
+int select_pair_children(iqhip_engine *e, const iqhip_node_op *ops, int nops, const std::vector<int> *explicit_segs,
+                         const double *const *len_ptrs, Kept &kept, bool *any) {
+    *any = false;
+    if (e->mfma || e->wide4 || e->n != 4 || e->n_user != 4 || e->embed2 || e->scalar_rule_all || explicit_segs || len_ptrs ||
+        nops < 2 || e->taxon_plain.size() != (size_t)e->ntaxa)
+        return IQHIP_OK;
+    std::unordered_map<uint64_t, int> writes, reads, first_read;
+    for (int k = 0; k < nops; k++) {
+        writes[ops[k].dst_key]++;
+        for (int side = 0; side < 2; side++) {
+            if ((side ? ops[k].right_leaf : ops[k].left_leaf) >= 0) continue;
+            const uint64_t key = side ? ops[k].right_key : ops[k].left_key;
+            if (!reads[key]++) first_read[key] = k;
+        }
+    }
+    std::vector<char> removed((size_t)nops, 0);
+    int nremoved = 0;
+    for (int k = 0; k + 1 < nops; k++) {
+        const iqhip_node_op &o = ops[k];
+        if (o.left_leaf < 0 || o.right_leaf < 0 || o.left_leaf >= e->ntaxa || o.right_leaf >= e->ntaxa) continue;
+        if (o.flags & (IQHIP_OP_NO_SCALE | IQHIP_OP_SCALAR_RULE)) continue;
+        if (!e->taxon_plain[o.left_leaf] || !e->taxon_plain[o.right_leaf]) continue;
+        if (!(o.left_len >= 0.0) || !(o.right_len >= 0.0)) continue;
+        if (writes[o.dst_key] != 1 || reads[o.dst_key] != 1 || first_read[o.dst_key] <= k) continue;
+        if (std::find(e->root_end_keys, e->root_end_keys + e->n_root_end_keys, o.dst_key) != e->root_end_keys + e->n_root_end_keys) continue;
+        removed[k] = 1;
+        nremoved++;
+    }
+    if (!nremoved) return IQHIP_OK;
+    const size_t P = (size_t)e->nptn_pad;
+    if (e->d_pair_rows.cap < (size_t)e->ntaxa * P) {
+        HIPCHK(e->d_pair_rows.ensure(e, (size_t)e->ntaxa * P));
+        e->pair_row_of.clear();
+    }
+    size_t nmissing = 0;
+    for (int k = 0; k < nops; k++)
+        nmissing += removed[k] && !e->pair_row_of.count(pair_key(ops[k].left_leaf, ops[k].right_leaf));
+    if (e->pair_row_of.size() + nmissing > e->d_pair_rows.cap / P) e->pair_row_of.clear();
+    for (int k = 0; k < nops; k++) {
+        if (removed[k]) {
+            const iqhip_node_op &o = ops[k];
+            const uint8_t *codes;
+            int rc = pair_code_row(e, o.left_leaf, o.right_leaf, &codes);
+            if (rc) return rc;
+            if (codes) {
+                int didx;
+                rc = slab_for_key(e, o.dst_key, true, &didx);
+                if (rc) return rc;
+                kept.pairs[o.dst_key] = {o.left_leaf, o.right_leaf, o.left_len, o.right_len, k, codes};
+                e->plan.virt.push_back({didx, o.left_leaf, o.right_leaf, o.left_len, o.right_len});
+                continue;
+            }
+        }
+        kept.ops.push_back(ops[k]);
+        kept.row.push_back(k);
+    }
+    *any = !kept.pairs.empty();
+    if (e->debug_plan) fprintf(stderr, "[iqhip] plan: %zu of %d ops removed as pair children\n", kept.pairs.size(), nops);
+    return IQHIP_OK;
+}
+
+void mark_virtual_slabs(iqhip_engine *e) {
+    for (const Plan::Virtual &v : e->plan.virt) {
+        Slab &s = e->slabs[v.slab];
+        s.virt = true;
+        s.taxon_l = v.taxon_l; s.taxon_r = v.taxon_r;
+        s.len_l = v.len_l; s.len_r = v.len_r;
+    }
+    e->pair_ops_removed += (int64_t)e->plan.virt.size();
+}
+
 int fill_descriptors(iqhip_engine *e, const iqhip_node_op *ops, int nops, const Units &u, const double *const *len_ptrs,
-                     int *last_dst) {
+                     int *last_dst, const Kept *kept) {
     int prev_dst = -1;
     for (int k = 0; k < nops; k++) {
         const iqhip_node_op &o = ops[u.order[k]];
         DevOp &d = e->h_ops.p[k];
         dummy_op(e, d);
-        d.out_row = u.order[k];
+        d.out_row = kept ? kept->row[u.order[k]] : u.order[k];
         d.no_scale = (o.flags & IQHIP_OP_NO_SCALE) ? 1 : (((o.flags & IQHIP_OP_SCALAR_RULE) || e->scalar_rule_all) ? 2 : 0);
         if (k > 0 && u.seg_of[k] != u.seg_of[k - 1]) prev_dst = -1;
         if (!(o.left_len >= 0.0) || !(o.right_len >= 0.0))
             return fail(IQHIP_ERR_INVALID, "negative or NaN branch length");
         const double *lp, *rp; const int16_t *lsc, *rsc;
         const uint8_t *lst, *rst; int32_t lkind, rkind;
-        int rc = resolve_child(e, o.left_key, o.left_leaf, prev_dst, &lp, &lsc, &lst, &lkind);
+        const PairDef *lpair = nullptr, *rpair = nullptr;
+        if (kept && o.left_leaf < 0 && kept->pairs.count(o.left_key)) lpair = &kept->pairs.at(o.left_key);
+        if (kept && o.right_leaf < 0 && kept->pairs.count(o.right_key)) rpair = &kept->pairs.at(o.right_key);
+        int rc = IQHIP_OK;
+        if (lpair) { lp = nullptr; lsc = nullptr; lst = lpair->codes; lkind = CHILD_PAIR; }
+        else rc = resolve_child(e, o.left_key, o.left_leaf, prev_dst, &lp, &lsc, &lst, &lkind);
         if (rc) return rc;
-        rc = resolve_child(e, o.right_key, o.right_leaf, prev_dst, &rp, &rsc, &rst, &rkind);
+        if (rpair) { rp = nullptr; rsc = nullptr; rst = rpair->codes; rkind = CHILD_PAIR; }
+        else rc = resolve_child(e, o.right_key, o.right_leaf, prev_dst, &rp, &rsc, &rst, &rkind);
         if (rc) return rc;
         int didx;
         rc = slab_for_key(e, o.dst_key, true, &didx);
         if (rc) return rc;
-        if ((lkind != CHILD_LEAF && lp == e->slabs[didx].plh.p) || (rkind != CHILD_LEAF && rp == e->slabs[didx].plh.p))
+        if ((!child_is_table(lkind) && lp == e->slabs[didx].plh.p) || (!child_is_table(rkind) && rp == e->slabs[didx].plh.p))
             return fail(IQHIP_ERR_INVALID, "node update writes onto one of its own children");
         if (lkind == CHILD_PREV && rkind == CHILD_PREV)
             return fail(IQHIP_ERR_INVALID, "node update uses the same vector for both children");
@@ -225,16 +331,18 @@
         } else {
             auto swap_children = [&]() {
                 std::swap(lp, rp); std::swap(lsc, rsc); std::swap(lst, rst);
-                std::swap(lkind, rkind); std::swap(llen, rlen); std::swap(llen_p, rlen_p);
+                std::swap(lkind, rkind); std::swap(llen, rlen); std::swap(llen_p, rlen_p); std::swap(lpair, rpair);
             };
             if (lkind == CHILD_PREV) swap_children();
-            else if (lkind == CHILD_LEAF && rkind == CHILD_LOAD) swap_children();
+            else if (child_is_table(lkind) && rkind == CHILD_LOAD) swap_children();
             if (lkind == CHILD_LOAD) lkind = CHILD_PF;
             if (rkind == CHILD_LOAD) (u.seg_of[k] ? e->plan.units_have_load : e->plan.has_load) = true;
             if (lkind == CHILD_PF) { d.pf = lp; d.pf_sc = lsc; d.real_mask |= 1; }
             if (rkind == CHILD_LOAD) { d.ld = rp; d.ld_sc = rsc; }
-            if (lkind == CHILD_LEAF) d.sl = lst;
-            if (rkind == CHILD_LEAF) d.sr = rst;
+            if (child_is_table(lkind)) d.sl = lst;
+            if (child_is_table(rkind)) d.sr = rst;
+            if (lpair) { d.pair_len[0] = lpair->len_l; d.pair_len[1] = lpair->len_r; d.pair_row_l = lpair->row; }
+            if (rpair) { d.pair_len[2] = rpair->len_l; d.pair_len[3] = rpair->len_r; d.pair_row_r = rpair->row; }
         }
         d.left_kind = lkind; d.right_kind = rkind;
         d.left_len = llen; d.right_len = rlen;
@@ -383,14 +491,15 @@
 int lay_out_lds(iqhip_engine *e, int nops, const std::vector<int> &seg_of) {
     const int B = e->block, budget = lds_budget(e);
     const bool tables_in_lds = e->mfma && e->mfma_pipelined && e->n == 20 && e->plan.nleaf_tabs > 0;
-    const int leaf_sz = (!e->mfma || e->wide4) ? 6 * B : (tables_in_lds ? (int)leaf_table_doubles(e) : B);
+    const int leaf_sz = (!e->mfma || e->wide4) ? child_region_blocks(CHILD_LEAF) * B : (tables_in_lds ? (int)leaf_table_doubles(e) : B);
+    const int pair_sz = child_region_blocks(CHILD_PAIR) * B;
     const int slot_sz = e->mfma ? 0 : trav4_lds(B).slot_doubles;
     int chunk_start = 0, used = slot_sz, regs = 0, max_used = 0, slots = 1, max_slots = 1;
     for (int k = 0; k < nops; k++) {
         DevOp &d = e->h_ops.p[k];
-        const int szl = d.left_kind == CHILD_LEAF ? leaf_sz : B;
-        const int szr = d.right_kind == CHILD_LEAF ? leaf_sz : B;
-        const int nleaf = (d.left_kind == CHILD_LEAF) + (d.right_kind == CHILD_LEAF);
+        const int szl = d.left_kind == CHILD_LEAF ? leaf_sz : (d.left_kind == CHILD_PAIR ? pair_sz : B);
+        const int szr = d.right_kind == CHILD_LEAF ? leaf_sz : (d.right_kind == CHILD_PAIR ? pair_sz : B);
+        const int nleaf = child_is_table(d.left_kind) + child_is_table(d.right_kind);
         const int need = szl + szr + nleaf * slot_sz;
         if (need > budget) return fail(IQHIP_ERR_UNSUPPORTED, "nstates*ncat too large for the LDS plan regions");
         const bool rows_full = !e->mfma && slots + nleaf > kTrav4RowSlots;
@@ -403,8 +512,8 @@
         regs += szl + szr;
         used += need;
         if (regs > max_used) max_used = regs;
-        d.sl_slot = d.left_kind == CHILD_LEAF ? slots++ : 0;
-        d.sr_slot = d.right_kind == CHILD_LEAF ? slots++ : 0;
+        d.sl_slot = child_is_table(d.left_kind) ? slots++ : 0;
+        d.sr_slot = child_is_table(d.right_kind) ? slots++ : 0;
         if (slots > max_slots) max_slots = slots;
     }
     if (nops > 0) {
@@ -432,6 +541,11 @@
         const size_t off = (size_t)(p - e->d_states.p);
         return off % (size_t)e->nptn_pad == 0 && off / (size_t)e->nptn_pad < (size_t)e->ntaxa;
     };
+    auto pair_row = [&](const uint8_t *p) {
+        if (!p || !e->d_pair_rows.p || p < e->d_pair_rows.p) return false;
+        const size_t off = (size_t)(p - e->d_pair_rows.p);
+        return off % (size_t)e->nptn_pad == 0 && off / (size_t)e->nptn_pad < e->pair_row_of.size();
+    };
     auto table = [&](const double *p) {
         if (e->plan.nleaf_tabs == 0 && !e->d_leaf_tab.p) return p == nullptr;
         if (!p || !e->d_leaf_tab.p || p < e->d_leaf_tab.p || per == 0) return false;
@@ -446,7 +560,14 @@
         if (!scs.count(d.pf_sc)) return bad(k, "pf_sc is not a counter slab / the dummy");
         if (!vecs.count(d.ld)) return bad(k, "ld (second memory child) is not a vector slab / the dummy slab");
         if (!scs.count(d.ld_sc)) return bad(k, "ld_sc is not a counter slab / the dummy");
-        if (!state_row(d.sl) || !state_row(d.sr)) return bad(k, "sl / sr is not a row of the state matrix");
+        const bool pl = k < nops && d.left_kind == CHILD_PAIR, pr = k < nops && d.right_kind == CHILD_PAIR;
+        if ((pl || pr) && (e->mfma || e->wide4)) return bad(k, "pair child in a plan of another kernel than k_traverse4");
+        if (!(pl ? pair_row(d.sl) : state_row(d.sl)) || !(pr ? pair_row(d.sr) : state_row(d.sr)))
+            return bad(k, "sl / sr is not a row of the state matrix (a pair-code row for a pair child, and only for one)");
+        if ((pl && !(d.pair_len[0] >= 0.0 && d.pair_len[1] >= 0.0)) || (pr && !(d.pair_len[2] >= 0.0 && d.pair_len[3] >= 0.0)))
+            return bad(k, "pair child with a negative or NaN pendant branch length");
+        if ((pl != (d.pair_row_l >= 0)) || (pr != (d.pair_row_r >= 0)) || d.pair_row_l >= e->plan.nrows || d.pair_row_r >= e->plan.nrows)
+            return bad(k, "pair_row is not the row of a removed op");
         if (!table(d.tabL) || !table(d.tabR)) return bad(k, "tabL / tabR is not a K2 table slot");
         if (d.cherry) {
             const size_t cper = (size_t)e->cherry_npairs * e->block;
@@ -457,16 +578,16 @@
         }
         if (k >= nops) continue;
         if (d.dst == e->dummy.plh.p || d.dst_sc == e->dummy.sc.p) return bad(k, "a real op writes the dummy slab");
-        const bool lk = d.left_kind == CHILD_LEAF || d.left_kind == CHILD_PF || d.left_kind == CHILD_HOLD ||
+        const bool lk = d.left_kind == CHILD_LEAF || d.left_kind == CHILD_PAIR || d.left_kind == CHILD_PF || d.left_kind == CHILD_HOLD ||
                         (d.left_kind == CHILD_LOAD && e->mfma && !e->mfma_pipelined);
-        const bool rk = d.right_kind == CHILD_LEAF || d.right_kind == CHILD_PREV || d.right_kind == CHILD_LOAD;
+        const bool rk = d.right_kind == CHILD_LEAF || d.right_kind == CHILD_PAIR || d.right_kind == CHILD_PREV || d.right_kind == CHILD_LOAD;
         if (!lk || !rk) return bad(k, "child kinds are not in canonical form");
         if (d.left_kind == CHILD_PF && (d.pf == e->dummy.plh.p || !(d.real_mask & 1))) return bad(k, "streamed child without a real vector");
         if (d.left_kind != CHILD_PF && !(e->mfma && !e->mfma_pipelined) && (d.real_mask & 1)) return bad(k, "real_mask set without a streamed child");
         if (d.right_kind == CHILD_LOAD && d.ld == e->dummy.plh.p) return bad(k, "second memory child without a real vector");
         if (d.dst == d.pf || d.dst == d.ld) return bad(k, "op writes one of its own children");
         if (!(d.left_len >= 0.0) || !(d.right_len >= 0.0)) return bad(k, "negative or NaN branch length");
-        if (d.out_row < 0 || d.out_row >= nops) return bad(k, "out_row outside the caller's op list");
+        if (d.out_row < 0 || d.out_row >= e->plan.nrows) return bad(k, "out_row outside the caller's op list");
         if (d.lds_left < 0 || d.lds_right < 0 || d.lds_left > e->plan.lds_doubles || d.lds_right > e->plan.lds_doubles)
             return bad(k, "LDS region outside the launch's allocation");
         if (d.sl_slot < 0 || d.sr_slot < 0 || d.sl_slot >= e->plan.state_slots || d.sr_slot >= e->plan.state_slots)
@@ -491,18 +612,18 @@
             int next = 1, regs = 0;
             for (int q = k; q < k + c.chunk_nops; q++) {
                 const DevOp &d = e->h_ops.p[q];
-                if (d.sl_slot != (d.left_kind == CHILD_LEAF ? next : 0)) return bad(q, "leaf-state slots of the chunk are not 1 .. n in op order");
-                next += d.left_kind == CHILD_LEAF;
-                if (d.sr_slot != (d.right_kind == CHILD_LEAF ? next : 0)) return bad(q, "leaf-state slots of the chunk are not 1 .. n in op order");
-                next += d.right_kind == CHILD_LEAF;
-                const int szl = (d.left_kind == CHILD_LEAF ? 6 : 1) * e->block, szr = (d.right_kind == CHILD_LEAF ? 6 : 1) * e->block;
+                if (d.sl_slot != (child_is_table(d.left_kind) ? next : 0)) return bad(q, "leaf-state slots of the chunk are not 1 .. n in op order");
+                next += child_is_table(d.left_kind);
+                if (d.sr_slot != (child_is_table(d.right_kind) ? next : 0)) return bad(q, "leaf-state slots of the chunk are not 1 .. n in op order");
+                next += child_is_table(d.right_kind);
+                const int szl = child_region_blocks(d.left_kind) * e->block, szr = child_region_blocks(d.right_kind) * e->block;
+                if (d.lds_left < d.lds_right + szr && d.lds_right < d.lds_left + szl) return bad(q, "LDS regions of the two children overlap");
                 regs = std::max(regs, std::max(d.lds_left + szl, d.lds_right + szr));
             }
             if (c.chunk_slots != next) return bad(k, "chunk_slots is not the chunk's slot count");
             if (next > kTrav4RowSlots) return bad(k, "more leaf-state slots than the kernel's row-pointer list holds");
-            if (next > e->plan.state_slots || regs > e->plan.lds_doubles ||
-                regs + next * trav4_lds(e->block).slot_doubles > lds_budget(e))
-                return bad(k, "LDS chunk outside the launch's allocation or over the budget");
+            if (next > e->plan.state_slots || regs > e->plan.lds_doubles) return bad(k, "LDS chunk outside the launch's allocation");
+            if (regs + next * trav4_lds(e->block).slot_doubles > lds_budget(e)) return bad(k, "LDS chunk over the LDS budget");
         }
         k += c.chunk_nops;
     }
@@ -538,7 +659,7 @@
     return IQHIP_OK;
 }
 
-int finish_and_upload(iqhip_engine *e, const iqhip_node_op *ops, int nops, Units &u, const std::vector<int> *explicit_segs,
+int finish_and_upload(iqhip_engine *e, int nops, const iqhip_node_op *ops_in, int nops_in, Units &u, const std::vector<int> *explicit_segs,
                       const double *const *len_ptrs, int last_dst) {
     Plan &p = e->plan;
     for (int q = 0; q < kSentinels; q++) dummy_op(e, e->h_ops.p[nops + q]);
@@ -558,7 +679,7 @@
         memcpy(e->h_ops.p + p.jobs_off, p.tab_jobs.data(), sizeof(TabJob) * p.tab_jobs.size());
     }
     PlanCache &c = e->plan_cache;
-    c.ops_in.assign((const char *)ops, (const char *)(ops + nops));
+    c.ops_in.assign((const char *)ops_in, (const char *)(ops_in + nops_in));
     c.segs = explicit_segs ? *explicit_segs : std::vector<int>();
     c.version = len_ptrs ? 0 : e->keymap_version;
     c.dst = last_dst;
@@ -569,6 +690,17 @@
         if (br == "tab") e->h_ops.p[nops - 1].tabL = nullptr;
         else if (br == "sentinel") e->h_ops.p[nops + kSentinels - 1].pf = nullptr;
         else if (br == "states") e->h_ops.p[0].sr = nullptr;
+        else if (br == "pair_row") {
+            for (int k = 0; k < nops; k++)
+                if (e->h_ops.p[k].left_kind == CHILD_LEAF && !e->pair_row_of.empty()) { e->h_ops.p[k].sl = e->d_pair_rows.p; break; }
+        } else if (br == "pair_region") {
+            for (int k = 0; k < nops; k++)
+                if (e->h_ops.p[k].left_kind == CHILD_PAIR) {
+                    e->h_ops.p[k].lds_left = lds_budget(e);
+                    e->plan.lds_doubles = lds_budget(e) + child_region_blocks(CHILD_PAIR) * e->block;
+                    break;
+                }
+        }
         else if (br == "cherry")
             for (int k = 0; k < nops; k++)
                 if (e->h_ops.p[k].cherry) { e->h_ops.p[k].cherry += 8; break; }
@@ -714,6 +846,7 @@
     if (nops + 2 > e->result_cap) return fail(IQHIP_ERR_INVALID, "too many node updates in one submission");
     if (plan_is_cached(e, ops, nops, explicit_segs, len_ptrs)) {
         *last_dst = e->plan_cache.dst;
+        mark_virtual_slabs(e);
         return IQHIP_OK;
     }
     e->plan_cache.version = 0;
@@ -723,15 +856,24 @@
     }
     e->plan = Plan();
     e->plan.cherry_model = e->model_version;
+    e->plan.nrows = nops;
+    const iqhip_node_op *const ops_in = ops;
+    const int nops_in = nops;
+    Kept kept;
+    bool removed = false;
+    int rc = select_pair_children(e, ops, nops, explicit_segs, len_ptrs, kept, &removed);
+    if (rc) return rc;
+    if (removed) { ops = kept.ops.data(); nops = (int)kept.ops.size(); }
     Units u;
-    int rc = cut_units(e, ops, nops, explicit_segs, u);
+    rc = cut_units(e, ops, nops, explicit_segs, u);
     if (!rc) rc = ensure_plan_capacity(e, nops + kSentinels + segment_table_ops(u) + devops_for(sizeof(TabJob) * (size_t)(2 * nops + 1)));
-    if (!rc) rc = fill_descriptors(e, ops, nops, u, len_ptrs, last_dst);
+    if (!rc) rc = fill_descriptors(e, ops, nops, u, len_ptrs, last_dst, removed ? &kept : nullptr);
     if (!rc) park_operands(e, nops, u.seg_of);
     if (!rc) rc = assign_leaf_tables(e, nops);
     if (!rc) rc = assign_cherry_tables(e, nops, u.seg_of);
     if (!rc) rc = lay_out_lds(e, nops, u.seg_of);
-    if (!rc) rc = finish_and_upload(e, ops, nops, u, explicit_segs, len_ptrs, *last_dst);
+    if (!rc) rc = finish_and_upload(e, nops, ops_in, nops_in, u, explicit_segs, len_ptrs, *last_dst);
+    if (!rc) mark_virtual_slabs(e);
     return rc;
 }
 
diff --git a/iq-tree_amd/csrc/trav_lds.h b/iq-tree_amd/csrc/trav_lds.h
--- a/iq-tree_amd/csrc/trav_lds.h
+++ b/iq-tree_amd/csrc/trav_lds.h
@@ -6,7 +6,7 @@
 constexpr int kTravWg = 256;
 constexpr int kTravMaxLdsBytes = 150 * 1024;
 constexpr int kTravGenericMaxLdsBytes = 160 * 1024;
-constexpr int kTrav4MaxLdsBytes = 152 * 1024;
+constexpr int kTrav4MaxLdsBytes = 150 * 1024;
 
 __host__ __device__ constexpr int tipx_doubles(int n, int nx) { return nx * n; }
 
```

Result: faster. 35250 M updates/s, median of 6 (+2.7%).
